# pedropro/UrsoNet

Hardware: AMD Instinct MI355X
Metric: images/sec fwd+bwd ResNet50 640x512 bs32/GPU (higher is better)
Workload: dtype bf16; 1 GPU; resnet50 bottleneck=32 ori_resolution=16 soft-class head + loc regression, batch 32/GPU x 512x640x3, full training step (prep+fwd+loss+bwd+clip+SGD); global_batch=32, parallelism=dp1, comm_cus=0, hipgraph=True, runner=Engine, input=uint8 frames in HBM, mean subtraction + cast in the step (molding kernel), gradient_norm_from_finalisation_blocks=True, weight_gradients_on_forked_stream=True

## Files before the change

### include/ursonet_hip.h

```cpp
#ifndef URSONET_HIP_H
#define URSONET_HIP_H

#include <stddef.h>
#include <stdint.h>

#ifdef __cplusplus
extern "C" {
#endif

#define URSO_OK            0
#define URSO_EINVAL       -1
#define URSO_ELAUNCH      -2
#define URSO_EWORKSPACE   -3

enum { URSO_F32 = 0, URSO_BF16 = 1, URSO_F16 = 2 };

#define URSO_EPI_RELU      1
#define URSO_EPI_OUT_F32   2
#define URSO_EPI_MASK_BITS 4
#define URSO_EPI_EMIT_BITS 8
#define URSO_EPI_ADD_SRCGRID 16

const char* urso_last_error(void);
int         urso_abi_version(void);

int urso_set_option(const char* name, int value);
int urso_get_option(const char* name, int* value);

typedef struct urso_conv_geom {
    int32_t B, H, W, C;
    int32_t OH, OW, N;
    int32_t KH, KW;
    int32_t SH, SW;
    int32_t PH, PW;
    int32_t DH, DW;
    int32_t FH, FW, OSH, OSW;
} urso_conv_geom;

int urso_conv_igemm(const urso_conv_geom* g, int dt, int flags,
                    const void* src_d, const void* wgt_d, const float* bias_d,
                    const void* add_d, const void* mask_d, void* dst_d, void* stream);
size_t urso_conv_igemm_ws_bytes(const urso_conv_geom* g, int dt);
int urso_conv_igemm_ws(const urso_conv_geom* g, int dt, int flags,
                       const void* src_d, const void* wgt_d, const float* bias_d,
                       const void* add_d, const void* mask_d, void* dst_d, void* ws_d, size_t ws_bytes, void* stream);
int urso_conv_igemm_bits_ok(const urso_conv_geom* g, int dt, int flags, size_t ws_bytes);
int urso_conv_igemm_ex(const urso_conv_geom* g, int dt, int flags,
                       const void* src_d, const void* wgt_d, const float* bias_d,
                       const void* add_d, const void* mask_d, void* dst_d, void* bits_out_d,
                       void* ws_d, size_t ws_bytes, void* stream);

int urso_conv_pair_ok(long long M, int dt, int c_narrow, int c_wide);
int urso_conv_pair(long long M, int c_narrow, int dt, int mode, const void* src_d, const void* w1_d, const float* bias1_d,
                   const void* add_d, void* bits_d, void* mid_d, const void* w2_d, const float* bias2_d, const void* mask2_d,
                   void* dst_d, int add_h, int add_w, void* stream);
int urso_rows_subsample2(int B, int H, int W, int row_bytes, const void* in_d, void* out_d, void* stream);
int urso_conv_pair_wgrad_splits(long long M, int dt);
int urso_conv_dgrad_wgrad_pw(long long M, int dt, const void* dz_d, const void* wd_d, const void* x_d, int mask_by_x, void* dx_d,
                             float* part_d, float* colpart_d, size_t part_stride, void* stream);
int urso_conv_pair_wgrad_entry(long long M, int dt, const void* src_d, const void* w1_d, const void* add_d, const void* bits_d,
                               const void* w2_d, const void* u_d, void* dst_d, const void* ws_d, const void* xin_d, int mask_by_xin, void* dxin_d,
                               float* part_d, float* colpart_d, float* part_s_d, float* colpart_s_d, size_t part_stride, void* stream);
int urso_conv_pair_shortcut(long long M, int dt, const void* src_d, const void* w1_d, const float* bias1_d,
                            const void* xin_d, const void* ws_d, const float* bias_s_d, void* bits_d, void* mid_d,
                            const void* w2_d, const float* bias2_d, void* dst_d, void* stream);
int urso_conv_pair_wgrad(long long M, int dt, const void* src_d, const void* w1_d, const void* add_d, const void* bits_d, void* mid_d,
                         const void* w2_d, const void* u_d, void* dst_d, int add_h, int add_w,
                         float* part_d, float* colpart_d, size_t part_stride, void* stream);
int urso_rows_expand2(int B, int H, int W, int row_bytes, const void* in_d, void* out_d, void* stream);
int urso_rows_scatter2(int B, int H, int W, int row_bytes, const void* in_d, void* out_d, void* stream);
int urso_zero_fill(void* dst_d, size_t bytes, void* stream);

int urso_conv_pointwise_sampled_ok(const urso_conv_geom* g, int dt, int flags, int has_add);
int urso_conv_pointwise_sampled(const urso_conv_geom* g, int dt, int flags, const void* src_d, const void* wgt_d, const float* bias_d,
                                const void* add_d, void* dst_d, void* bits_out_d, void* dst_sampled_d, void* stream);

int urso_conv_pointwise2_ok(int B, int OH, int OW, int C0, int C1, int N, int dt, int flags);
int urso_conv_pointwise2(int B, int OH, int OW, int C0, int C1, int N, int dt, int flags,
                         const void* src0_d, const void* wgt0_d, const void* src1_d, const void* wgt1_d,
                         const float* bias_d, const void* mask_d, void* dst_d, void* bits_out_d, void* stream);

#define URSO_DENSE_MULTI_MAX 4
typedef struct urso_dense_layer {
    const void* src0; const void* wgt0; const void* src1; const void* wgt1;
    const float* bias;
    const void* add; const void* mask;
    void* dst;
    int32_t M, N, K0, K1, flags;
} urso_dense_layer;
int urso_dense_multi(int nlayers, const urso_dense_layer* layers, int dt, void* stream);
typedef struct urso_dense_wgrad_layer {
    const void* x; const void* dz;
    float* part; float* colpart;
    int32_t M, K, N;
} urso_dense_wgrad_layer;
int urso_dense_wgrad_multi(int nlayers, const urso_dense_wgrad_layer* layers, int dt, void* stream);

int urso_conv_igemm_algorithmic(const urso_conv_geom* g, int dt, int flags, int has_add, int has_mask, double* flops_out, double* bytes_out);
int urso_conv_igemm_halo_ok(const urso_conv_geom* g, int dt, int flags, int has_add);
size_t urso_conv_igemm_halo_ws_bytes(void);
int urso_conv_igemm_halo2_shape(const urso_conv_geom* g, int dt, int flags, int has_add, int has_ws);

size_t urso_conv_winograd_ws_bytes(const urso_conv_geom* g, int dt);
int urso_conv_winograd_fwd(const urso_conv_geom* g, int dt, int flags, const void* src_d, const void* wgt_d, const float* bias_d,
                           void* dst_d, void* ws_d, size_t ws_bytes, void* stream);

#define URSO_WGRAD_PART_PAD 64
size_t urso_conv_wgrad_ws_bytes(const urso_conv_geom* g, int dt);
int urso_conv_wgrad(const urso_conv_geom* g, int dt, const void* x_d, const void* dz_d,
                    void* ws_d, size_t ws_bytes, float* dw_raw_d, float* colsum_d, void* stream);

int urso_conv_weight_prep(int KH, int KW, int C, int N, int npad, int dt,
                          const float* w_d, const float* b_d,
                          const float* gamma_d, const float* beta_d,
                          const float* mean_d, const float* var_d, float eps,
                          void* wf_d, void* wd_d, float* biasf_d, float* scale_d, void* stream);

int urso_stem_weight_pack(int N, int dt, const float* w_d, const float* b_d,
                          const float* gamma_d, const float* beta_d, const float* mean_d,
                          const float* var_d, float eps, void* wf_d, float* biasf_d,
                          float* scale_d, void* stream);
int urso_stem_wgrad_unpack(int N, const float* dw_packed_d, float* dw_raw_d, void* stream);

int urso_param_grad_finalize(int K, int N, int ldn ,
                             const float* dw_raw_d, const float* colsum_d,
                             const float* w_d, const float* b_d,
                             const float* gamma_d, const float* mean_d, const float* var_d,
                             float eps, float weight_decay, int trainable, int bn_trainable,
                             float* gw_d, float* gb_d, float* ggamma_d, float* gbeta_d,
                             float* ws_d, size_t ws_bytes, void* stream);
size_t urso_param_grad_finalize_ws_bytes(int K, int N);

typedef struct urso_param_desc {
    int32_t KH, KW, C, N, npad, K;
    int32_t splits, ks, kb;
    int32_t trainable, bn_trainable;
    int32_t bias_from;
    float eps, regc, regb;
    const float *w, *b, *gamma, *beta, *mean, *var;
    void *wf, *wd;
    float *biasf, *scale;
    const float *part, *colpart;
    float *dw_raw, *colsum, *dotpart;
    float *gw, *gb, *ggamma, *gbeta;
} urso_param_desc;
enum { URSO_PB_PREP = 0, URSO_PB_REDUCE = 1, URSO_PB_FINALIZE_MAT = 2, URSO_PB_FINALIZE_VEC = 3 };
int urso_conv_wgrad_splits(const urso_conv_geom* g, int dt);
int urso_conv_wgrad_partial(const urso_conv_geom* g, int dt, const void* x_d, const void* dz_d,
                            void* ws_d, size_t ws_bytes, void* stream);
int urso_param_desc_init(urso_param_desc* d, int KH, int KW, int C, int N, int npad, int splits, float eps, float weight_decay);
int urso_param_batch_plan(int phase, const urso_param_desc* descs_h, const int32_t* layer_ids, int n_ids,
                          int32_t* blockmap_h, int cap_blocks);
int urso_param_batch_run(int phase, int dt, const urso_param_desc* descs_d, const int32_t* blockmap_d, int nblocks, void* stream);
int urso_param_batch_run_sq(int phase, int dt, const urso_param_desc* descs_d, const int32_t* blockmap_d, int nblocks, float* sqpart_d, void* stream);
int urso_param_grad_finalize_sq_slots(int K, int N);
int urso_param_grad_finalize_sq(int K, int N, int ldn, const float* dw_raw_d, const float* colsum_d,
                                const float* w_d, const float* b_d, const float* gamma_d, const float* mean_d,
                                const float* var_d, float eps, float weight_decay, int trainable, int bn_trainable,
                                float* gw_d, float* gb_d, float* ggamma_d, float* gbeta_d,
                                float* ws_d, size_t ws_bytes, float* sqpart_d, void* stream);
int urso_sqnorm_final(int nparts, const float* parts_d, float* out_d, void* stream);

typedef struct urso_wgrad_item {
    const void* x;
    const void* dz;
    float* part;
    float* colpart;
    urso_conv_geom g;
    int32_t M, ktiles, ntiles, splits, m_per_split, mode, fill;
} urso_wgrad_item;
int urso_wgrad_group_fits(const urso_conv_geom* g, int dt);
int urso_wgrad_group_plan(int n, urso_wgrad_item* items_h, int dt, int32_t* blockmap_h, int cap_blocks);
int urso_wgrad_group_run(int dt, const urso_wgrad_item* items_d, const urso_wgrad_item* items_h, int n,
                         const int32_t* blockmap_d, int nblocks, void* stream);

int urso_conv_wgrad_pair_splits(const urso_conv_geom* g0, const urso_conv_geom* g1, int dt, int* splits0, int* splits1);
int urso_conv_wgrad_partial2(const urso_conv_geom* g0, const urso_conv_geom* g1, int dt,
                             const void* x0_d, const void* dz0_d, void* ws0_d, size_t ws0_bytes,
                             const void* x1_d, const void* dz1_d, void* ws1_d, size_t ws1_bytes, void* stream);

size_t urso_bn_ws_bytes(int M, int N);
int urso_bn_batch_stats(int M, int N, int dt, const void* z_d, void* ws_d, size_t ws_bytes, float* mean_d, float* var_d,
                        float* moving_mean_d, float* moving_var_d, float momentum, float eps, void* stream);
int urso_bn_apply(int M, int N, int dt, const void* z_d, const float* mean_d, const float* var_d, const float* gamma_d,
                  const float* beta_d, float eps, const void* res_d, int relu, void* y_d, void* stream);
int urso_bn_backward(int M, int N, int dt, const void* g_d, const void* z_d, const float* mean_d, const float* var_d,
                     const float* gamma_d, float eps, void* ws_d, size_t ws_bytes, float* dbeta_d, float* dgamma_d,
                     int bn_trainable, float* gbeta_d, float* ggamma_d, void* dz_d, void* stream);

int urso_mold_images(int B, int H, int W, int src_is_u8, const void* src_d, const float* mean3_d,
                     int dt, void* dst_d, void* stream);

int urso_stem_wgrad_pooled(const urso_conv_geom* g, int dt, const void* x_d, const void* dpool_d, const uint8_t* argmax_d,
                           void* ws_d, size_t ws_bytes, float* dw_raw_d, float* colsum_d, void* stream);
int urso_stem_conv_pool_ok(const urso_conv_geom* g, int dt);
int urso_stem_conv_pool(const urso_conv_geom* g, int dt, const void* x_d, const void* wgt_d, const float* bias_d, void* y_d,
                        uint8_t* argmax_d, void* stream);
int urso_maxpool3x3s2_fwd(int B, int H, int W, int C, int dt, const void* x_d, void* y_d,
                          uint8_t* argmax_d, void* stream);
int urso_maxpool3x3s2_bwd(int B, int H, int W, int C, int dt, const void* y_d, const void* dy_d,
                          const uint8_t* argmax_d, int relu_mask, void* dx_d, void* stream);

int urso_softmax_xent_fwd_bwd(int B, int K, const float* logits_d , const float* labels_d,
                              float weight, int relu_mask, int dt, float* loss_d, void* dz_d,
                              float* row_ws_d, void* stream);
int urso_rel_l2_fwd_bwd(int B, int D, int ld ,
                        const float* gt_d , const float* pred_d, float weight,
                        int dt, float* loss_d, void* dpred_d, float* norms_d, void* stream);
int urso_rel_l2_norms(int B, int D, int ld, const float* gt_d, const float* pred_d, float* norms_d, void* stream);
int urso_rel_l2_from_norms(int B, int D, int ld, const float* gt_d, const float* pred_d, float weight, const float* gscale_d,
                           int dt, const float* norms_d, float* loss_d, void* dpred_d, void* stream);
int urso_absdot_fwd_bwd(int B, int D, int ld , int normalize,
                        const float* gt_d , const float* x_d,
                        float weight, int dt, float* q_d , float* loss_d, void* dx_d, void* stream);
int urso_mse_fwd_bwd(int B, int D, int ld, const float* gt_d, const float* pred_d, float weight,
                     int dt, float* loss_d, void* dpred_d, void* stream);

size_t urso_sqnorm_ws_bytes(size_t n);
int urso_sqnorm(size_t n, const float* g_d, void* ws_d, size_t ws_bytes, float* out_d, void* stream);
int urso_sgd_momentum_clip(size_t n, float* w_d, const float* g_d, float* v_d,
                           const float* hyper_d, const float* normsq_d, void* stream);
int urso_adam_amsgrad_clip(size_t n, float* w_d, const float* g_d, float* m_d, float* v_d, float* vhat_d,
                           float* hyper_d, const float* normsq_d, void* stream);
int urso_scale_f32(size_t n, float* x_d, float s, void* stream);

int urso_quat_wavg_decode(int B, int K, const float* logits_d, const float* hquat_d,
                          float* q_d, float* a_d, void* stream);

int urso_quat_gmm_fit(int B, int K, const float* in_d, int in_is_pmf, const float* hquat_d, float var,
                      int nr_iterations, int nr_max_modes, float* mean_d, float* var_d, float* prior_d,
                      float* score_d, int* nmodes_d, void* stream);

enum { URSO_EVAL_LOC_REGRESS = 0, URSO_EVAL_LOC_CLASS = 1 };
enum { URSO_EVAL_ORI_QUAT = 0, URSO_EVAL_ORI_EULER = 1, URSO_EVAL_ORI_ANGLE_AXIS = 2, URSO_EVAL_ORI_SOFT = 3, URSO_EVAL_ORI_KEYPOINTS = 4 };
enum { URSO_EVAL_LOC_EST = 0, URSO_EVAL_Q_EST = 3, URSO_EVAL_LOC_ERR = 7, URSO_EVAL_ORI_ERR = 8, URSO_EVAL_ESA = 9, URSO_EVAL_DIST = 10,
       URSO_EVAL_LOC_ENC_ERR = 11, URSO_EVAL_ORI_ENC_ERR = 12, URSO_EVAL_ORI_ERR_SOFT = 13, URSO_EVAL_MODE = 14, URSO_EVAL_COLS = 16 };
typedef struct urso_pose_eval_args {
    int32_t B, n;
    int64_t row0;
    int32_t loc_mode, ori_mode;
    int32_t loc_ld, ori_ld;
    int32_t loc_bins, loc_map_rows, ori_bins, ori_map_rows, gmm_modes, pad0;
    const float* loc;
    const float* ori;
    const float* ori2;
    const double* loc_map;
    const float* ori_map;
    const float* enc_loc;
    const float* enc_ori;
    const double* loc_gt;
    const double* q_gt;
    const float* gmm_mean;
    const int32_t* gmm_nmodes;
    double* table;
} urso_pose_eval_args;
int urso_pose_eval(const urso_pose_eval_args* args, void* stream);

enum { URSO_DEC_LOC_EST = 0, URSO_DEC_Q_EST = 3, URSO_DEC_LOC_PEAK = 7, URSO_DEC_ORI_PEAK = 8, URSO_DEC_ORI_LAMBDA = 9, URSO_DEC_COLS = 12 };
typedef struct urso_pose_decode_args {
    int32_t B, n;
    int64_t row0;
    int32_t loc_mode, ori_mode;
    int32_t loc_ld, ori_ld;
    int32_t loc_bins, loc_map_rows, ori_bins, ori_map_rows;
    int32_t ori_logits_ld, pad0;
    const float* loc;
    const float* ori;
    const float* ori2;
    const double* loc_map;
    const float* ori_logits;
    const float* ori_scatter;
    double* table;
} urso_pose_decode_args;
int urso_pose_decode(const urso_pose_decode_args* args, void* stream);

int urso_warp_perspective(int B, int H, int W, int C, int interp, const uint8_t* src_d, const double* m_d, uint8_t* dst_d, void* stream);
int urso_encode_ori(int B, int K, const double* q_d, const float* hquat_d, const uint8_t* redundant_d, double var,
                    float* out_d, void* stream);

int urso_encode_loc(int B, int K, const double* loc_d, const double* hmap_d, double sig2, float* out_d, void* stream);

int urso_rgb_to_grey3(int B, int H, int W, const uint8_t* src_d, uint8_t* dst_d, void* stream);
int urso_sim2real_op(int B, int H, int W, const uint8_t* src_d, uint8_t* dst_d, const int32_t* op_d, const float* par_d,
                     const uint32_t* seed_d, const uint8_t* drop_d, int drop_stride, void* stream);
int urso_pad_images_u8(int B, int H, int W, int C, int OH, int OW, int top, int left, const uint8_t* src_d, uint8_t* dst_d, void* stream);

int urso_resize_images_u8(int B, int H, int W, int C, int NH, int NW, int OH, int OW, int top, int left,
                          const double* ky_d, int ry, const double* kx_d, int rx, const int32_t* y0_d, const double* fy_d,
                          const int32_t* x0_d, const double* fx_d, int trunc_passes, const uint8_t* src_d, uint8_t* dst_d, void* stream);

int urso_frames_grey_flags_u8(int B, int HW, const uint8_t* src_d, uint8_t* flags_d, void* stream);
int urso_frames_put_u8(int B, int HW, const uint8_t* src_d, const uint64_t* dst_addr_d, const uint8_t* kind_d, void* stream);
int urso_frames_gather_u8(int B, int HW, const uint64_t* src_addr_d, const uint8_t* kind_d, uint8_t* dst_d, void* stream);

int urso_video_prep_u8(int B, int H, int W, int top, int bottom, int left, int right, int pad, double w0, double w1, double w2,
                       const uint8_t* src_d, uint8_t* dst_d, void* stream);

// ... 48 lines not shown
```

### ursonet_amd/csrc/common.h

```cpp
#pragma once
#include <hip/hip_runtime.h>
#include <stdint.h>
#include <stdio.h>
#include "../../include/ursonet_hip.h"

typedef __attribute__((ext_vector_type(8))) __bf16 bf16x8_t;
typedef __attribute__((ext_vector_type(8))) _Float16 f16x8_t;
typedef __attribute__((ext_vector_type(4))) float f32x4_t;
typedef __attribute__((ext_vector_type(4))) int i32x4_t;
typedef __attribute__((ext_vector_type(2))) int i32x2_t;

void urso_set_error(const char* fmt, ...);
int  urso_check_launch(const char* what);

#define URSO_OPTION_TABLE(X) \
    X(pw_kernel, 3)         \
    X(pw_small, 5)          \
    X(wgrad_narrow, 1)      \
    X(wgrad_blocks, 512)    \
    X(wgrad_pipe, 1)        \
    X(wgrad_big, 1)         \
    X(wgrad_ring, 0)        \
    X(grid_cap, 0)          \
    X(hconv, 1)             \
    X(pair, 1)              \
    X(pair_single, 3)       \
    X(c3, 1)                \
    X(c3v, 1)               \
    X(stem, 1)              \
    X(stem_pool, 1)         \
    X(cus, 0)               \
    X(hconv2, 1)            \
    X(hconv2_shape, 0)      \
    X(hconv_streamk, 1)     \
    X(hconv_dbg, 0)         \
    X(hwgrad, 1)            \
    X(dense, 1)             \
    X(pwx, 1)               \
    X(pwx_dbg, 0)           \
    X(pwx_bn, 0)            \
    X(mold_scalar, 0)       \
    X(bneck, 3)
struct UrsoOptions {
#define URSO_OPT_FIELD(name, dflt) int name = dflt;
    URSO_OPTION_TABLE(URSO_OPT_FIELD)
#undef URSO_OPT_FIELD
};
extern UrsoOptions g_urso_opt;
int urso_device_cus();
int urso_usable_cus();

#define URSO_FUSE_REDUCE_MAX 16
static __host__ __device__ inline bool urso_fuse_reduce(int splits) { return splits > 1 && splits <= URSO_FUSE_REDUCE_MAX; }

#define URSO_REDUCE_COLS 256
static __host__ __device__ inline int urso_reduce_lanes(int splits) { return splits > 384 ? 16 : (splits > 192 ? 8 : (splits > 96 ? 4 : (splits > 48 ? 2 : 1))); }

void urso_prof_before(hipStream_t s, int kernel_id, double flops, double bytes);
void urso_prof_after(hipStream_t s);

void urso_prof_l2(double l2_bytes);
void urso_prof_symbol(const void* host_fn);
#define URSO_KLAUNCH(kern, grid, blk, shm, st, ...) do { urso_prof_symbol((const void*)(kern)); hipLaunchKernelGGL(kern, grid, blk, shm, st, ##__VA_ARGS__); } while (0)

struct ProfScope {
    hipStream_t s;
    ProfScope(hipStream_t st, int id, double flops, double bytes) : s(st) { urso_prof_before(s, id, flops, bytes); }
    ~ProfScope() { urso_prof_after(s); }
};

static inline size_t dt_size(int dt) { return dt == URSO_F32 ? 4 : 2; }
static __host__ __device__ inline int ceil_div(int a, int b) { return (a + b - 1) / b; }

template <typename T> struct Elem;
template <> struct Elem<float> {
    static constexpr int VE = 4;
    static __device__ __forceinline__ float to_f(float v) { return v; }
    static __device__ __forceinline__ float from_f(float v) { return v; }
};
template <> struct Elem<__bf16> {
    static constexpr int VE = 8;
    static constexpr int ONES = 0x3F803F80;
    static __device__ __forceinline__ float to_f(__bf16 v) { return (float)v; }
    static __device__ __forceinline__ __bf16 from_f(float v) { return (__bf16)v; }
};
template <> struct Elem<_Float16> {
    static constexpr int VE = 8;
    static constexpr int ONES = 0x3C003C00;
    static __device__ __forceinline__ float to_f(_Float16 v) { return (float)v; }
    static __device__ __forceinline__ _Float16 from_f(float v) { return (_Float16)v; }
};

template <typename T> struct Mma;
template <> struct Mma<__bf16> {
    static __device__ __forceinline__ void run(const i32x4_t& a, const i32x4_t& b, f32x4_t& c) {
        c = __builtin_amdgcn_mfma_f32_16x16x32_bf16(__builtin_bit_cast(bf16x8_t, a), __builtin_bit_cast(bf16x8_t, b), c, 0, 0, 0);
    }
};
template <> struct Mma<_Float16> {
    static __device__ __forceinline__ void run(const i32x4_t& a, const i32x4_t& b, f32x4_t& c) {
        c = __builtin_amdgcn_mfma_f32_16x16x32_f16(__builtin_bit_cast(f16x8_t, a), __builtin_bit_cast(f16x8_t, b), c, 0, 0, 0);
    }
};
template <> struct Mma<float> {
    static __device__ __forceinline__ void run(const i32x4_t& a, const i32x4_t& b, f32x4_t& c) {
        f32x4_t fa = __builtin_bit_cast(f32x4_t, a), fb = __builtin_bit_cast(f32x4_t, b);
        c = __builtin_amdgcn_mfma_f32_16x16x4f32(fa.x, fb.x, c, 0, 0, 0);
        c = __builtin_amdgcn_mfma_f32_16x16x4f32(fa.y, fb.y, c, 0, 0, 0);
        c = __builtin_amdgcn_mfma_f32_16x16x4f32(fa.z, fb.z, c, 0, 0, 0);
        c = __builtin_amdgcn_mfma_f32_16x16x4f32(fa.w, fb.w, c, 0, 0, 0);
    }
};

__device__ __forceinline__ int lds_swz(int row) {
    int c = (row >> 3) & 7;
    int s = (c & 4) | ((c & 1) << 1) | ((c >> 1) & 1);
    return (row & 7) ^ s;
}
__device__ __forceinline__ int lds_off(int row, int chunk) {
    return row * 128 + ((chunk ^ lds_swz(row)) << 4);
}

#define URSO_OOB_SHIFT 0x80000000u
__device__ __forceinline__ __amdgpu_buffer_rsrc_t make_rsrc(const void* p, uint32_t bytes) {
    return __builtin_amdgcn_make_buffer_rsrc(const_cast<void*>(p), 0, bytes, 0x00020000);
}
__device__ __forceinline__ i32x4_t buf_load16(__amdgpu_buffer_rsrc_t r, uint32_t byte_off) {
    return __builtin_amdgcn_raw_buffer_load_b128(r, byte_off, 0, 0);
}
__device__ __forceinline__ void buf_store16(__amdgpu_buffer_rsrc_t r, uint32_t byte_off, i32x4_t v) {
    __builtin_amdgcn_raw_buffer_store_b128(v, r, byte_off, 0, 0);
}

__device__ __forceinline__ void lds_barrier() {
    asm volatile("s_waitcnt lgkmcnt(0)" ::: "memory");
    __builtin_amdgcn_s_barrier();
    asm volatile("" ::: "memory");
}

__device__ __forceinline__ float wave_sum(float v) {
#pragma unroll
    for (int o = 32; o > 0; o >>= 1) v += __shfl_xor(v, o, 64);
    return v;
}
__device__ __forceinline__ float wave_max(float v) {
#pragma unroll
    for (int o = 32; o > 0; o >>= 1) v = fmaxf(v, __shfl_xor(v, o, 64));
    return v;
}

__device__ __forceinline__ int xcd_remap(int bid, int nblk) {
    const int NX = 8;
    if (nblk < NX) return bid;
    int xcd = bid % NX, idx = bid / NX;
    int q = nblk / NX, r = nblk % NX;
    int base = (xcd < r) ? xcd * (q + 1) : r * (q + 1) + (xcd - r) * q;
    return base + idx;
}

static inline int urso_persistent_grid(int ntiles, int blocks_per_cu, int groups = 1) {
    int bpx = ceil_div(ntiles, 8), cap = blocks_per_cu * urso_usable_cus() / (8 * groups);
    if (cap < 1) cap = 1;
    if (bpx > cap) bpx = cap;
    if (g_urso_opt.grid_cap > 0 && bpx > ceil_div(g_urso_opt.grid_cap, 8)) bpx = ceil_div(g_urso_opt.grid_cap, 8);
    return 8 * bpx;
}
struct UrsoTileStream { int tile, t_end, bpx; };
__device__ __forceinline__ UrsoTileStream urso_tile_stream(int ntiles) {
    const int xcd = blockIdx.x & 7, lb = blockIdx.x >> 3, bpx = gridDim.x >> 3;
    const int cpx = ceil_div(ntiles, 8);
    const int t_end = min((xcd + 1) * cpx, ntiles);
    return { xcd * cpx + lb, t_end, bpx };
}
```

### ursonet_amd/csrc/conv_wgrad.hip

```cpp
#include "lds_mfma.h"
#include "internal.h"
#include <stdlib.h>

struct WgradArgs {
    const void* x; const void* dz; float* part; float* colpart;
    uint32_t x_bytes, dz_bytes;
    int B, H, W, C, OH, OW, N, KH, KW, SH, SW, PH, PW;
    int M, Cc, Kc, K;
    int ktiles, ntiles, splits, m_per_split;
    int dbg;
    int pointwise;
    float rcp_ohw, rcp_ow;
    int zs, ZH, ZW, zsh, zsw;
};

template <typename T, int MODE>
__global__ __launch_bounds__(256, 2) void wgrad_kernel(const WgradArgs a) {
    constexpr int VE = Elem<T>::VE;
    constexpr int RM = 128 / (int)sizeof(T);
    constexpr int NCH = 128 / VE;
    constexpr int PIX = (sizeof(T) == 2) ? 2 : 1;
    constexpr int ITEMS = (RM / PIX) * NCH / 256;
    constexpr int PSTEP = 256 / NCH;
    __shared__ __attribute__((aligned(16))) char smem[2 * 2 * 128 * 128];
// ... 744 lines not shown
    const int dq = RM / a.OW, dr = RM - dq * a.OW;
    const uint32_t xc_off = (uint32_t)(cc * VE) * 2u, z_off0 = (uint32_t)ncol * 2u;

    auto dma = [&](int buf) {
        const uint32_t dx = lds0 + buf * BUFB + wave * 1024, dz = lds0 + buf * BUFB + RM * 256 + wave * 1024;
#pragma unroll
        for (int e = 0; e < ITEMS; ++e) {
            const int m = mcur + prow + 16 * e;
            const bool mvalid = m < m_end;
            uint32_t off; bool ok;
            if constexpr (MODE == 0) { off = (uint32_t)(m * a.C) * 2u + xc_off; ok = mvalid && kvalid; }
            else {
                int b, oy, ox;
                if constexpr (MODE == 1) {
                    b = pb[e]; oy = poy[e]; ox = pox[e];
                    int nx = ox + dr; const bool w1 = nx >= a.OW; nx -= w1 ? a.OW : 0;
                    int ny = oy + dq + (w1 ? 1 : 0); const bool w2 = ny >= a.OH; ny -= w2 ? a.OH : 0;
                    pox[e] = nx; poy[e] = ny; pb[e] = b + (w2 ? 1 : 0);
                } else { int rem; divmod(m, ohw, a.rcp_ohw, b, rem); divmod(rem, a.OW, a.rcp_ow, oy, ox); }
                const int iy = oy * a.SH - a.PH + ky, ix = ox * a.SW - a.PW + kx;
                ok = mvalid && kvalid && iy >= 0 && ix >= 0 && iy < a.H && ix < a.W;
                off = (uint32_t)(((b * a.H + iy) * a.W + ix) * a.C) * 2u + xc_off;
            }
            lds_dma16(rx, dx + e * 16 * 256, ok ? off : URSO_OOB_SHIFT);
        }
#pragma unroll
        for (int e = 0; e < 2; ++e) {
            const int mz = mcur + zrow + 32 * e;
            uint32_t zp = (uint32_t)mz;
            if (a.zs) { int b, rem, oy, ox; divmod(mz, ohw, a.rcp_ohw, b, rem); divmod(rem, a.OW, a.rcp_ow, oy, ox); zp = (uint32_t)((b * a.ZH + oy * a.zsh) * a.ZW + ox * a.zsw); }
            const uint32_t zoff = zp * (uint32_t)a.N * 2u + z_off0;
            lds_dma16(rz, dz + e * 32 * 128, (mz < m_end && nvalid) ? zoff : URSO_OOB_SHIFT);
        }
        mcur += RM;
    };

    const int fr = lane & 15, fg = lane >> 4;
    const int frow = fg * 4 + (fr >> 2), fsw = frow & 7;
    const int fbase = frow * 256 + (fr & 3) * 8;
    int offx[4], offz[2];
#pragma unroll
    for (int i = 0; i < 4; ++i) offx[i] = fbase + (((wk * 4 + i) ^ fsw) << 5);
    const int zbase = frow * 128 + (fr & 3) * 8, zsw = (frow >> 1) & 3;
#pragma unroll
    for (int j = 0; j < 2; ++j) offz[j] = zbase + (((wn * 2 + j) ^ zsw) << 5);

    f32x4_t acc[4][2], accc[2];
#pragma unroll
    for (int i = 0; i < 4; ++i)
#pragma unroll
        for (int j = 0; j < 2; ++j) acc[i][j] = f32x4_t{0.f, 0.f, 0.f, 0.f};
    accc[0] = accc[1] = f32x4_t{0.f, 0.f, 0.f, 0.f};
    const bool do_col = (kt == 0) && (wk == 0) && a.colpart;
    const i32x4_t ones = {Elem<T>::ONES, Elem<T>::ONES, Elem<T>::ONES, Elem<T>::ONES};

    const int nsteps = (m_end > m_begin) ? ceil_div(m_end - m_begin, RM) : 0;
    if (nsteps > 0) dma(0);
    asm volatile("s_waitcnt vmcnt(0)" ::: "memory");
    __syncthreads();
    for (int s = 0; s < nsteps; ++s) {
        const int cur = s & 1;
        if (s + 1 < nsteps) dma(cur ^ 1);
        const char* bx = sX(cur); const char* bz = sZ(cur);
#pragma unroll
        for (int ks = 0; ks < 2; ++ks) {
            i32x4_t fz[2], fx[4];
#pragma unroll
            for (int j = 0; j < 2; ++j) {
                const i32x2_t lo = lds_read_tr16(bz + offz[j] + ks * 32 * 128), hi = lds_read_tr16(bz + offz[j] + ks * 32 * 128 + 16 * 128);
                fz[j] = i32x4_t{lo.x, lo.y, hi.x, hi.y};
            }
#pragma unroll
            for (int i = 0; i < 4; ++i) {
                const i32x2_t lo = lds_read_tr16(bx + offx[i] + ks * 32 * 256), hi = lds_read_tr16(bx + offx[i] + ks * 32 * 256 + 16 * 256);
                fx[i] = i32x4_t{lo.x, lo.y, hi.x, hi.y};
            }
#pragma unroll
            for (int i = 0; i < 4; ++i)
#pragma unroll
                for (int j = 0; j < 2; ++j) Mma<T>::run(fz[j], fx[i], acc[i][j]);
            if (do_col) {
#pragma unroll
                for (int j = 0; j < 2; ++j) Mma<T>::run(fz[j], ones, accc[j]);
            }
        }
        asm volatile("s_waitcnt vmcnt(0)" ::: "memory");
        __syncthreads();
    }

    float* out = a.part + (size_t)sp * ((size_t)a.K * a.N + URSO_WGRAD_PART_PAD);
#pragma unroll
    for (int i = 0; i < 4; ++i) {
        const int k = kt * 128 + wk * 64 + i * 16 + fr;
        if (k >= a.K) continue;
#pragma unroll
        for (int j = 0; j < 2; ++j) {
            const int nb = n0 + wn * 32 + j * 16 + fg * 4;
            if (nb >= a.N) continue;
            *(f32x4_t*)(out + (size_t)k * a.N + nb) = acc[i][j];
        }
    }
    if (do_col && fr == 0) {
#pragma unroll
        for (int j = 0; j < 2; ++j) {
            const int nb = n0 + wn * 32 + j * 16 + fg * 4;
            if (nb < a.N) *(f32x4_t*)(a.colpart + (size_t)sp * a.N + nb) = accc[j];
        }
    }
}

__device__ __forceinline__ void reduce_partials_body(int bid, const float* __restrict__ part, float* __restrict__ out, size_t count, int splits,
                                                     size_t pstride ) {
    __shared__ f32x4_t red[256];
    const size_t nq = (count + 3) / 4;
    const bool vec = (count & 3) == 0;
    const int SL = urso_reduce_lanes(splits), cols = URSO_REDUCE_COLS / SL;
    const int col = threadIdx.x % cols, sl = threadIdx.x / cols;
    const size_t q = (size_t)bid * cols + col;
    f32x4_t t = f32x4_t{0.f, 0.f, 0.f, 0.f};
    if (vec && q < nq) {
        const size_t stride = pstride / 4;
        const f32x4_t* p = (const f32x4_t*)part + q;
        const int per = (splits + SL - 1) / SL, k1 = min(splits, (sl + 1) * per);
        int k = sl * per;
        for (; k + 16 <= k1; k += 16) {
            f32x4_t v[16];
#pragma unroll
            for (int i = 0; i < 16; ++i) v[i] = p[(size_t)(k + i) * stride];
#pragma unroll
            for (int i = 0; i < 16; ++i) t += v[i];
        }
        for (; k < k1; ++k) t += p[(size_t)k * stride];
    }
    if (SL > 1) {
        red[threadIdx.x] = t;
        __syncthreads();
        if (sl == 0) {
            t = red[col];
            for (int i = 1; i < SL; ++i) t += red[i * cols + col];
        }
    }
    if (vec && q < nq && sl == 0) *((f32x4_t*)out + q) = t;
    if (!vec && threadIdx.x == 0 && bid == 0)
        for (size_t e = 0; e < count; ++e) { float tt = 0.f; for (int i = 0; i < splits; ++i) tt += part[(size_t)i * pstride + e]; out[e] = tt; }
}

__global__ __launch_bounds__(256) void reduce_partials_kernel(const float* __restrict__ part, float* __restrict__ out, size_t count, int splits, size_t pstride) {
    reduce_partials_body(blockIdx.x, part, out, count, splits, pstride);
}

__global__ __launch_bounds__(256) void reduce_partials_batch_kernel(const urso_param_desc* __restrict__ descs, const int32_t* __restrict__ blockmap) {
    const urso_param_desc& d = descs[blockmap[2 * blockIdx.x]];
    const int local = blockmap[2 * blockIdx.x + 1];
    const size_t cnt = (size_t)d.K * d.npad;
    const int rcols = URSO_REDUCE_COLS / urso_reduce_lanes(d.splits);
    const int nb_dw = (int)(((cnt + 3) / 4 + rcols - 1) / rcols);
    if (local < nb_dw) reduce_partials_body(local, d.part, d.dw_raw, cnt, d.splits, cnt + URSO_WGRAD_PART_PAD);
    else reduce_partials_body(local - nb_dw, d.colpart, d.colsum, (size_t)d.npad, d.splits, (size_t)d.npad);
}

void urso_reduce_partials_batch_launch(const urso_param_desc* descs_d, const int32_t* blockmap_d, int nblocks, hipStream_t st) {
    URSO_KLAUNCH(reduce_partials_batch_kernel, dim3(nblocks), dim3(256), 0, st, descs_d, blockmap_d);
}

struct WgradPlan { int VE, RM, Cc, Kc, K, M, ktiles, ntiles, splits, m_per_split, narrow; size_t part_elems, col_elems; };

static int plan_wgrad(const urso_conv_geom* g, int dt, WgradPlan& p) {
    const int es = (int)dt_size(dt);
    p.VE = 16 / es; p.RM = 128 / es;
    if (g->C % p.VE || g->N % p.VE) return URSO_EINVAL;
    p.Cc = g->C / p.VE; p.Kc = g->KH * g->KW * p.Cc; p.K = p.Kc * p.VE;
    p.M = g->B * g->OH * g->OW;
    const int narrow_ok = g_urso_opt.wgrad_narrow;
#ifndef URSO_WGRAD_NARROW_MULTITAP
#define URSO_WGRAD_NARROW_MULTITAP 0
#endif
    p.narrow = (es == 2 && narrow_ok && (g->N <= 64 || (URSO_WGRAD_NARROW_MULTITAP && g->KH * g->KW > 1))) ? 1 : 0;
    p.ktiles = ceil_div(p.K, 128); p.ntiles = ceil_div(g->N, p.narrow ? 64 : 128);
    const int tiles = p.ktiles * p.ntiles;
    const int steps = ceil_div(p.M, p.RM);
    const int target = (int)((long long)g_urso_opt.wgrad_blocks * urso_usable_cus() / urso_device_cus());
#ifndef URSO_WGRAD_NARROW_PCT
#define URSO_WGRAD_NARROW_PCT 150
#endif
    int splits = (p.narrow ? target * URSO_WGRAD_NARROW_PCT / 100 : target) / tiles;
    splits = splits < 1 ? 1 : splits;
    int max_splits = steps / 8; if (max_splits < 1) max_splits = 1;
    if (splits > max_splits) splits = max_splits;
    int steps_per = ceil_div(steps, splits);
    splits = ceil_div(steps, steps_per);
    if (urso_c3g_fits(g, dt)) splits = urso_c3g_splits(g);
    else if (urso_hwg_fits(g, dt)) splits = urso_hwg_splits(g);
    p.splits = splits; p.m_per_split = steps_per * p.RM;
    p.part_elems = (size_t)splits * ((size_t)p.K * g->N + URSO_WGRAD_PART_PAD);
    p.col_elems = (size_t)splits * g->N;
    return URSO_OK;
}

extern "C" size_t urso_conv_wgrad_ws_bytes(const urso_conv_geom* g, int dt) {
    WgradPlan p;
    if (g && urso_stemw_fits(g, dt)) {
        const size_t stem = (size_t)urso_stemw_splits(g, false) * ((size_t)224 * 64 + URSO_WGRAD_PART_PAD + 64) * sizeof(float) + 256;
        const size_t gen = plan_wgrad(g, dt, p) == URSO_OK ? (p.part_elems + p.col_elems) * sizeof(float) + 256 : 0;
        return stem > gen ? stem : gen;
    }
    if (!g || plan_wgrad(g, dt, p) != URSO_OK) return 0;
    return (p.part_elems + p.col_elems) * sizeof(float) + 256;
}

extern "C" int urso_conv_wgrad_splits(const urso_conv_geom* g, int dt) {
    WgradPlan p;
    if (!g || plan_wgrad(g, dt, p) != URSO_OK) return 0;
    return p.splits;
}

static int wgrad_impl(const urso_conv_geom* g, int dt, const void* x_d, const void* dz_d,
                      void* ws_d, size_t ws_bytes, float* dw_raw_d, float* colsum_d, bool keep_partials, void* stream) {
    if (!g || !x_d || !dz_d || !ws_d || (!dw_raw_d && !keep_partials)) { urso_set_error("urso_conv_wgrad: null argument"); return URSO_EINVAL; }
    if (dt != URSO_F32 && dt != URSO_BF16 && dt != URSO_F16) { urso_set_error("urso_conv_wgrad: bad dtype"); return URSO_EINVAL; }
    if (g->DH != 1 || g->DW != 1) { urso_set_error("urso_conv_wgrad: expects the forward geometry (D=1)"); return URSO_EINVAL; }
    WgradPlan p;
    if (plan_wgrad(g, dt, p) != URSO_OK) { urso_set_error("urso_conv_wgrad: C=%d and N=%d must be multiples of %d", g->C, g->N, 16 / (int)dt_size(dt)); return URSO_EINVAL; }
    const size_t need = urso_conv_wgrad_ws_bytes(g, dt);
    if (ws_bytes < need) { urso_set_error("urso_conv_wgrad: workspace %zu < %zu", ws_bytes, need); return URSO_EWORKSPACE; }
    const size_t es = dt_size(dt);
    const bool zscat = g->FH > 0;
    if (zscat && (dt == URSO_F32 || g->FW <= 0 || g->OSH <= 0 || g->OSW <= 0 || (g->OH - 1) * g->OSH >= g->FH || (g->OW - 1) * g->OSW >= g->FW ||
                  (g->KH == 1 && g->KW == 1 && g->SH == 1 && g->SW == 1 && g->PH == 0 && g->PW == 0 && g->H == g->OH && g->W == g->OW))) {
        urso_set_error("urso_conv_wgrad: scattered dz needs a 16-bit dtype, a non-pointwise geometry and a grid that fits [FH][FW]"); return URSO_EINVAL;
    }
    const size_t x_bytes = (size_t)g->B * g->H * g->W * g->C * es,
                 dz_bytes = zscat ? (size_t)g->B * g->FH * g->FW * g->N * es : (size_t)p.M * g->N * es;
    if (x_bytes >= 0x7FFFFF00ull || dz_bytes >= 0x7FFFFF00ull) { urso_set_error("urso_conv_wgrad: tensor exceeds 2 GiB"); return URSO_EINVAL; }
    if (urso_stemw_fits(g, dt) && !keep_partials && !zscat) {
        hipStream_t st = (hipStream_t)stream;
        const int splits = urso_stemw_splits(g, false);
        const size_t cnt = (size_t)224 * 64, pstride = cnt + URSO_WGRAD_PART_PAD;
        float* part = (float*)ws_d; float* colpart = part + (size_t)splits * pstride;
        ProfScope ps(st, URSO_K_WGRAD, 2.0 * p.M * 64.0 * 147.0, (double)x_bytes + (double)p.M * 128 + (double)cnt * 4);
        int rc = urso_stemw_launch(g, dt, x_d, dz_d, nullptr, nullptr, part, colsum_d ? colpart : nullptr, pstride, st);
        if (rc != URSO_OK) return rc;
        const int rcols = URSO_REDUCE_COLS / urso_reduce_lanes(splits);
        URSO_KLAUNCH(reduce_partials_kernel, dim3((int)((cnt / 4 + rcols - 1) / rcols)), dim3(256), 0, st, part, dw_raw_d, cnt, splits, pstride);
        if (colsum_d) URSO_KLAUNCH(reduce_partials_kernel, dim3((int)((64 / 4 + rcols - 1) / rcols)), dim3(256), 0, st, colpart, colsum_d, (size_t)64, splits, (size_t)64);
        return urso_check_launch("urso_conv_wgrad(stem reduce)");
    }
    WgradArgs a;
    a.x = x_d; a.dz = dz_d; a.x_bytes = (uint32_t)x_bytes; a.dz_bytes = (uint32_t)dz_bytes;
    float* part = (float*)ws_d; float* colpart = part + p.part_elems;
    const bool direct = (p.splits == 1) && !keep_partials;
    a.part = direct ? dw_raw_d : part;
    a.colpart = keep_partials ? colpart : (colsum_d ? (direct ? colsum_d : colpart) : nullptr);
    a.B = g->B; a.H = g->H; a.W = g->W; a.C = g->C; a.OH = g->OH; a.OW = g->OW; a.N = g->N;
    a.KH = g->KH; a.KW = g->KW; a.SH = g->SH; a.SW = g->SW; a.PH = g->PH; a.PW = g->PW;
    a.dbg = 0;
    a.pointwise = (g->KH == 1 && g->KW == 1 && g->SH == 1 && g->SW == 1 && g->PH == 0 && g->PW == 0 && g->H == g->OH && g->W == g->OW) ? 1 : 0;
    a.rcp_ohw = 1.0f / (float)(g->OH * g->OW); a.rcp_ow = 1.0f / (float)g->OW;
    a.zs = zscat ? 1 : 0; a.ZH = g->FH; a.ZW = g->FW; a.zsh = g->OSH; a.zsw = g->OSW;
    if ((size_t)g->B * g->OH * g->OW >= (1u << 24)) { urso_set_error("urso_conv_wgrad: more than 2^24 output pixels"); return URSO_EINVAL; }
    a.M = p.M; a.Cc = p.Cc; a.Kc = p.Kc; a.K = p.K; a.ktiles = p.ktiles; a.ntiles = p.ntiles; a.splits = p.splits; a.m_per_split = p.m_per_split;
    hipStream_t st = (hipStream_t)stream;
    double flops = 2.0 * p.M * (double)g->N * g->KH * g->KW * g->C;
    if (g->C == 8 && g->KH == 7 && g->KW == 4 && g->SH == 2) flops *= 147.0 / 224.0;
    const double x_alg = (g->KH == 1 && g->KW == 1 && (g->SH > 1 || g->SW > 1)) ? (double)p.M * g->C * es : (double)x_bytes;
    double bytes = x_alg + (double)p.M * g->N * es + (double)p.K * g->N * 4;
    ProfScope ps(st, URSO_K_WGRAD, flops, bytes);
    dim3 grid(p.ktiles * p.ntiles, p.splits);
    const int rm = 128 / (int)dt_size(dt);
    const int mode = a.pointwise ? 0 : (g->OW >= rm ? 1 : 2);
    const int tmode = a.pointwise ? 0 : ((64 / g->OW + 1 <= g->OH) ? 1 : 2);
#define URSO_WG(KERN, TT, MD) do { if (MD == 0) URSO_KLAUNCH((KERN<TT, 0>), grid, dim3(256), 0, st, a); \
                         else if (MD == 1) URSO_KLAUNCH((KERN<TT, 1>), grid, dim3(256), 0, st, a); \
                         else URSO_KLAUNCH((KERN<TT, 2>), grid, dim3(256), 0, st, a); } while (0)
    const int pipe = g_urso_opt.wgrad_pipe;
#define URSO_WGP(TT, MD) do { if (MD == 0) URSO_KLAUNCH((wgrad_tr_kernel<TT, 0, true>), grid, dim3(256), 0, st, a); \
                         else if (MD == 1) URSO_KLAUNCH((wgrad_tr_kernel<TT, 1, true>), grid, dim3(256), 0, st, a); \
                         else URSO_KLAUNCH((wgrad_tr_kernel<TT, 2, true>), grid, dim3(256), 0, st, a); } while (0)
    if (!zscat && urso_c3g_fits(g, dt)) {
        int rc3 = urso_c3g_launch(g, dt, x_d, dz_d, a.part, a.colpart, (size_t)p.K * g->N + URSO_WGRAD_PART_PAD, st);
        if (rc3 != URSO_OK) return rc3;
    }
    else if (!zscat && urso_hwg_fits(g, dt)) {
        int rc3 = urso_hwg_launch(g, dt, x_d, dz_d, a.part, a.colpart, (size_t)p.K * g->N + URSO_WGRAD_PART_PAD, st);
        if (rc3 != URSO_OK) return rc3;
    }
    else if (dt == URSO_F32) URSO_WG(wgrad_kernel, float, mode);
    else if (p.narrow) { if (dt == URSO_BF16) URSO_WG(wgrad_tr64_kernel, __bf16, tmode); else URSO_WG(wgrad_tr64_kernel, _Float16, tmode); }
    else if (dt == URSO_BF16) { if (pipe) URSO_WGP(__bf16, tmode); else URSO_WG(wgrad_tr_kernel, __bf16, tmode); }
    else { if (pipe) URSO_WGP(_Float16, tmode); else URSO_WG(wgrad_tr_kernel, _Float16, tmode); }
#undef URSO_WGP
#undef URSO_WG
    int rc = urso_check_launch("urso_conv_wgrad");
    if (rc != URSO_OK) return rc;
    if (!direct && !keep_partials) {
        size_t cnt = (size_t)p.K * g->N;
        const int rcols = URSO_REDUCE_COLS / urso_reduce_lanes(p.splits);
        int blocks = (int)(((cnt + 3) / 4 + rcols - 1) / rcols);
        URSO_KLAUNCH(reduce_partials_kernel, dim3(blocks), dim3(256), 0, st, part, dw_raw_d, cnt, p.splits, cnt + URSO_WGRAD_PART_PAD);
        if (colsum_d) URSO_KLAUNCH(reduce_partials_kernel, dim3((int)(((size_t)g->N / 4 + rcols - 1) / rcols)), dim3(256), 0, st, colpart, colsum_d, (size_t)g->N, p.splits, (size_t)g->N);
        rc = urso_check_launch("urso_conv_wgrad(reduce)");
    }
    return rc;
}

extern "C" int urso_conv_wgrad(const urso_conv_geom* g, int dt, const void* x_d, const void* dz_d,
                               void* ws_d, size_t ws_bytes, float* dw_raw_d, float* colsum_d, void* stream) {
    return wgrad_impl(g, dt, x_d, dz_d, ws_d, ws_bytes, dw_raw_d, colsum_d, false, stream);
// ... 183 lines not shown
```

### ursonet_amd/csrc/prep.hip

```cpp
#include "common.h"
#include "internal.h"

template <typename T> __device__ __forceinline__ void store_elem(void* p, size_t i, float v) { ((T*)p)[i] = Elem<T>::from_f(v); }

__device__ __forceinline__ float bn_scale(const float* gamma, const float* var, float eps, int n) {
    return gamma ? gamma[n] * rsqrtf(var[n] + eps) : 1.0f;
}

__device__ __forceinline__ float folded_bias(const urso_param_desc& o, int n) {
    if (n >= o.N) return 0.f;
    const float s = bn_scale(o.gamma, o.var, o.eps, n);
    float bf = o.b ? o.b[n] * s : 0.f;
    if (o.gamma) bf += o.beta[n] - o.mean[n] * s;
    return bf;
}

template <typename T>
__device__ __forceinline__ void weight_prep_body(int bx, int by, int tap, int KH, int KW, int C, int N, int npad,
                                   const float* __restrict__ w, const float* __restrict__ b,
                                   const float* __restrict__ gamma, const float* __restrict__ beta,
                                   const float* __restrict__ mean, const float* __restrict__ var, float eps,
                                   void* wf, void* wd, float* biasf, float* scale, const urso_param_desc* extra = nullptr) {
    __shared__ float tile[32][33];
    const int c0 = bx * 32, n0 = by * 32;
    const int tx = threadIdx.x & 31, ty = threadIdx.x >> 5;
    const int taps = KH * KW;
    const int ftap = taps - 1 - tap;
    const int n = n0 + tx;
    const float s = (n < N) ? bn_scale(gamma, var, eps, n) : 1.0f;
    for (int cy = ty; cy < 32; cy += 8) {
        const int c = c0 + cy;
        float v = 0.f;
        if (c < C && n < N) v = w[((size_t)tap * C + c) * N + n] * s;
        tile[cy][tx] = v;
        if (wd && c < C && n < npad) store_elem<T>(wd, ((size_t)c * taps + ftap) * npad + n, v);
    }
    __syncthreads();
    for (int ny = ty; ny < 32; ny += 8) {
        const int nn = n0 + ny, c = c0 + tx;
        if (nn < npad && c < C) store_elem<T>(wf, ((size_t)nn * taps + tap) * C + c, tile[tx][ny]);
    }
    if (tap == 0 && bx == 0 && ty == 0 && n < npad) {
        float bf = 0.f, sc = 1.f;
        if (n < N) {
            sc = s;
            bf = (b ? b[n] * s : 0.f);
            if (gamma) bf += beta[n] - mean[n] * s;
            if (extra) bf += folded_bias(*extra, n);
        }
        biasf[n] = bf; scale[n] = sc;
    }
}

template <typename T>
__device__ __forceinline__ void weight_prep_body64(int bx, int by, int tap, int KH, int KW, int C, int N, int npad,
                                   const float* __restrict__ w, const float* __restrict__ b,
                                   const float* __restrict__ gamma, const float* __restrict__ beta,
                                   const float* __restrict__ mean, const float* __restrict__ var, float eps,
                                   void* wf, void* wd, float* biasf, float* scale, const urso_param_desc* extra = nullptr) {
    __shared__ float tile[64][65];
    const int c0 = bx * 64, n0 = by * 64;
    const int tq = threadIdx.x & 15, tr = threadIdx.x >> 4;
    const int taps = KH * KW, ftap = taps - 1 - tap;
    const int n = n0 + tq * 4;
    float s[4];
#pragma unroll
    for (int q = 0; q < 4; ++q) s[q] = (n + q < N) ? bn_scale(gamma, var, eps, n + q) : 1.0f;
    for (int cy = tr; cy < 64; cy += 16) {
        const int c = c0 + cy;
        f32x4_t v = {0.f, 0.f, 0.f, 0.f};
        if (c < C && n < N) { v = *(const f32x4_t*)(w + ((size_t)tap * C + c) * N + n); v.x *= s[0]; v.y *= s[1]; v.z *= s[2]; v.w *= s[3]; }
        tile[cy][tq * 4] = v.x; tile[cy][tq * 4 + 1] = v.y; tile[cy][tq * 4 + 2] = v.z; tile[cy][tq * 4 + 3] = v.w;
        if (wd && c < C && n < npad) {
            T o[4] = {Elem<T>::from_f(v.x), Elem<T>::from_f(v.y), Elem<T>::from_f(v.z), Elem<T>::from_f(v.w)};
            __builtin_memcpy((T*)wd + ((size_t)c * taps + ftap) * npad + n, o, sizeof(o));
        }
    }
    __syncthreads();
    for (int ny = tr; ny < 64; ny += 16) {
        const int nn = n0 + ny, c = c0 + tq * 4;
        if (nn < npad && c < C) {
            T o[4] = {Elem<T>::from_f(tile[tq * 4][ny]), Elem<T>::from_f(tile[tq * 4 + 1][ny]), Elem<T>::from_f(tile[tq * 4 + 2][ny]),
                      Elem<T>::from_f(tile[tq * 4 + 3][ny])};
            __builtin_memcpy((T*)wf + ((size_t)nn * taps + tap) * C + c, o, sizeof(o));
        }
    }
    if (tap == 0 && bx == 0 && tr == 0) {
#pragma unroll
        for (int q = 0; q < 4; ++q) {
            const int nq = n + q;
            if (nq < npad) {
                float bf = 0.f, sc = 1.f;
                if (nq < N) { sc = s[q]; bf = (b ? b[nq] * s[q] : 0.f); if (gamma) bf += beta[nq] - mean[nq] * s[q]; if (extra) bf += folded_bias(*extra, nq); }
                biasf[nq] = bf; scale[nq] = sc;
            }
        }
    }
}

template <typename T>
__global__ void weight_prep_kernel(int KH, int KW, int C, int N, int npad,
                                   const float* __restrict__ w, const float* __restrict__ b,
                                   const float* __restrict__ gamma, const float* __restrict__ beta,
                                   const float* __restrict__ mean, const float* __restrict__ var, float eps,
                                   void* wf, void* wd, float* biasf, float* scale) {
    weight_prep_body<T>(blockIdx.x, blockIdx.y, blockIdx.z, KH, KW, C, N, npad, w, b, gamma, beta, mean, var, eps, wf, wd, biasf, scale);
}

template <typename T>
__global__ void weight_prep_batch_kernel(const urso_param_desc* __restrict__ descs, const int32_t* __restrict__ blockmap) {
    const urso_param_desc& d = descs[blockmap[2 * blockIdx.x]];
    const int local = blockmap[2 * blockIdx.x + 1];
    const urso_param_desc* extra = d.bias_from > 0 ? &descs[d.bias_from - 1] : nullptr;
    if (((d.C | d.N | d.npad) & 3) == 0) {
        const int gx = ceil_div(d.C, 64), gy = ceil_div(d.npad, 64);
        const int bx = local % gx, by = (local / gx) % gy, tap = local / (gx * gy);
        weight_prep_body64<T>(bx, by, tap, d.KH, d.KW, d.C, d.N, d.npad, d.w, d.b, d.gamma, d.beta, d.mean, d.var, d.eps,
                              d.wf, d.wd, d.biasf, d.scale, extra);
        return;
    }
    const int gx = ceil_div(d.C, 32), gy = ceil_div(d.npad, 32);
    const int bx = local % gx, by = (local / gx) % gy, tap = local / (gx * gy);
    weight_prep_body<T>(bx, by, tap, d.KH, d.KW, d.C, d.N, d.npad, d.w, d.b, d.gamma, d.beta, d.mean, d.var, d.eps,
                        d.wf, d.wd, d.biasf, d.scale, extra);
}

extern "C" int urso_conv_weight_prep(int KH, int KW, int C, int N, int npad, int dt,
                                     const float* w_d, const float* b_d, const float* gamma_d, const float* beta_d,
                                     const float* mean_d, const float* var_d, float eps,
                                     void* wf_d, void* wd_d, float* biasf_d, float* scale_d, void* stream) {
    if (!w_d || !wf_d || !biasf_d || !scale_d || KH <= 0 || KW <= 0 || C <= 0 || N <= 0 || npad < N) {
        urso_set_error("urso_conv_weight_prep: bad argument"); return URSO_EINVAL; }
    if (gamma_d && (!beta_d || !mean_d || !var_d)) { urso_set_error("urso_conv_weight_prep: incomplete BN tensors"); return URSO_EINVAL; }
    hipStream_t st = (hipStream_t)stream;
    dim3 grid(ceil_div(C, 32), ceil_div(npad, 32), KH * KW);
    ProfScope ps(st, URSO_K_PREP, 0, (double)KH * KW * C * N * (4 + 2 * dt_size(dt)));
    if (dt == URSO_F32) URSO_KLAUNCH((weight_prep_kernel<float>), grid, dim3(256), 0, st, KH, KW, C, N, npad, w_d, b_d, gamma_d, beta_d, mean_d, var_d, eps, wf_d, wd_d, biasf_d, scale_d);
    else if (dt == URSO_BF16) URSO_KLAUNCH((weight_prep_kernel<__bf16>), grid, dim3(256), 0, st, KH, KW, C, N, npad, w_d, b_d, gamma_d, beta_d, mean_d, var_d, eps, wf_d, wd_d, biasf_d, scale_d);
    else if (dt == URSO_F16) URSO_KLAUNCH((weight_prep_kernel<_Float16>), grid, dim3(256), 0, st, KH, KW, C, N, npad, w_d, b_d, gamma_d, beta_d, mean_d, var_d, eps, wf_d, wd_d, biasf_d, scale_d);
    else { urso_set_error("urso_conv_weight_prep: bad dtype"); return URSO_EINVAL; }
    return urso_check_launch("urso_conv_weight_prep");
}

template <typename T>
__global__ void stem_pack_kernel(int N, const float* __restrict__ w, const float* __restrict__ b,
                                 const float* __restrict__ gamma, const float* __restrict__ beta,
                                 const float* __restrict__ mean, const float* __restrict__ var, float eps,
                                 void* wf, float* biasf, float* scale) {
    const int i = blockIdx.x * blockDim.x + threadIdx.x;
    const int total = N * 7 * 4 * 8;
    if (i < total) {
        const int cp = i & 7, kp = (i >> 3) & 3, ky = (i >> 5) % 7, n = i / 224;
        const int q = 2 * kp + (cp >> 2), kx = q - 1, c = cp & 3;
        float v = 0.f;
        if (kx >= 0 && c < 3) v = w[(((size_t)ky * 7 + kx) * 3 + c) * N + n] * bn_scale(gamma, var, eps, n);
        store_elem<T>(wf, i, v);
    }
    if (i < N) {
        const float s = bn_scale(gamma, var, eps, i);
        float bf = b ? b[i] * s : 0.f;
        if (gamma) bf += beta[i] - mean[i] * s;
        biasf[i] = bf; scale[i] = s;
    }
}

extern "C" int urso_stem_weight_pack(int N, int dt, const float* w_d, const float* b_d, const float* gamma_d,
                                     const float* beta_d, const float* mean_d, const float* var_d, float eps,
                                     void* wf_d, float* biasf_d, float* scale_d, void* stream) {
    if (!w_d || !wf_d || !biasf_d || !scale_d || N <= 0) { urso_set_error("urso_stem_weight_pack: bad argument"); return URSO_EINVAL; }
    hipStream_t st = (hipStream_t)stream;
    const int total = N * 224, blocks = ceil_div(total, 256);
    ProfScope ps(st, URSO_K_PREP, 0, 0);
    if (dt == URSO_F32) URSO_KLAUNCH((stem_pack_kernel<float>), dim3(blocks), dim3(256), 0, st, N, w_d, b_d, gamma_d, beta_d, mean_d, var_d, eps, wf_d, biasf_d, scale_d);
    else if (dt == URSO_BF16) URSO_KLAUNCH((stem_pack_kernel<__bf16>), dim3(blocks), dim3(256), 0, st, N, w_d, b_d, gamma_d, beta_d, mean_d, var_d, eps, wf_d, biasf_d, scale_d);
    else if (dt == URSO_F16) URSO_KLAUNCH((stem_pack_kernel<_Float16>), dim3(blocks), dim3(256), 0, st, N, w_d, b_d, gamma_d, beta_d, mean_d, var_d, eps, wf_d, biasf_d, scale_d);
    else { urso_set_error("urso_stem_weight_pack: bad dtype"); return URSO_EINVAL; }
    return urso_check_launch("urso_stem_weight_pack");
}

__global__ void stem_unpack_kernel(int N, const float* __restrict__ dwp, float* __restrict__ dw) {
    const int i = blockIdx.x * blockDim.x + threadIdx.x;
    if (i >= 7 * 7 * 3 * N) return;
    const int n = i % N, c = (i / N) % 3, kx = (i / (3 * N)) % 7, ky = i / (21 * N);
    const int q = kx + 1, kp = q >> 1, cp = (q & 1) * 4 + c;
    dw[i] = dwp[(((size_t)ky * 4 + kp) * 8 + cp) * N + n];
}

extern "C" int urso_stem_wgrad_unpack(int N, const float* dw_packed_d, float* dw_raw_d, void* stream) {
    if (!dw_packed_d || !dw_raw_d || N <= 0) { urso_set_error("urso_stem_wgrad_unpack: bad argument"); return URSO_EINVAL; }
    hipStream_t st = (hipStream_t)stream;
    ProfScope ps(st, URSO_K_FINALIZE, 0, 0);
    URSO_KLAUNCH(stem_unpack_kernel, dim3(ceil_div(147 * N, 256)), dim3(256), 0, st, N, dw_packed_d, dw_raw_d);
    return urso_check_launch("urso_stem_wgrad_unpack");
}

__device__ __forceinline__ float block_sum_f(float v, float* sh) {
    v = wave_sum(v);
    const int w = threadIdx.x >> 6, nw = (blockDim.x + 63) >> 6;
    __syncthreads();
    if ((threadIdx.x & 63) == 0) sh[w] = v;
    __syncthreads();
    float t = 0.f;
    for (int i = 0; i < nw; ++i) t += sh[i];
    return t;
}

__device__ __forceinline__ void finalize_mat_body(int bx, int by, int K, int N, int ldn, int kb, const float* __restrict__ dwr, const float* __restrict__ w,
                                    const float* __restrict__ gamma, const float* __restrict__ var, float eps,
                                    float regc, int trainable, float* __restrict__ gw, float* __restrict__ dotpart, int nsum = 1, size_t pstride = 0,
                                    float* __restrict__ sqslot = nullptr) {
    const int kbeg = by * kb, kend = min(K, kbeg + kb);
    float sq = 0.f;
    auto sq4 = [&](const f32x4_t& g) { sq += g.x * g.x + g.y * g.y + g.z * g.z + g.w * g.w; };
    auto sq_out = [&]() {
        if (!sqslot) return;
        __shared__ float shq[8];
        const float t = block_sum_f(sq, shq);
        if (threadIdx.x == 0) *sqslot = t;
    };
    if (((N | ldn) & 3) == 0) {
        __shared__ f32x4_t red4[16][17];
        const int tq = threadIdx.x & 15, tk = threadIdx.x >> 4;
        const int n = bx * 64 + tq * 4;
        f32x4_t dot = {0.f, 0.f, 0.f, 0.f};
        if (n < N) {
            f32x4_t s;
            s.x = bn_scale(gamma, var, eps, n); s.y = bn_scale(gamma, var, eps, n + 1);
            s.z = bn_scale(gamma, var, eps, n + 2); s.w = bn_scale(gamma, var, eps, n + 3);
            auto row_sum = [&](int k) -> f32x4_t {
                const float* p = dwr + (size_t)k * ldn + n;
                f32x4_t d = *(const f32x4_t*)p;
                if (nsum > 1) {
                    f32x4_t t = f32x4_t{0.f, 0.f, 0.f, 0.f};
                    t += d;
                    int q = 1;
                    for (; q + 4 <= nsum; q += 4) {
                        const f32x4_t v0 = *(const f32x4_t*)(p + (size_t)q * pstride), v1 = *(const f32x4_t*)(p + (size_t)(q + 1) * pstride);
                        const f32x4_t v2 = *(const f32x4_t*)(p + (size_t)(q + 2) * pstride), v3 = *(const f32x4_t*)(p + (size_t)(q + 3) * pstride);
                        t += v0; t += v1; t += v2; t += v3;
                    }
                    for (; q < nsum; ++q) t += *(const f32x4_t*)(p + (size_t)q * pstride);
                    d = t;
                }
                return d;
            };
            int k = kbeg + tk;
            for (; k + 16 < kend; k += 32) {
                const f32x4_t w0 = *(const f32x4_t*)(w + (size_t)k * N + n), w1 = *(const f32x4_t*)(w + (size_t)(k + 16) * N + n);
                const f32x4_t d0 = row_sum(k), d1 = row_sum(k + 16);
                dot += w0 * d0;
                dot += w1 * d1;
                f32x4_t g0 = s * d0 + w0 * regc, g1 = s * d1 + w1 * regc;
                if (!trainable) g0 = g1 = f32x4_t{0.f, 0.f, 0.f, 0.f};
                *(f32x4_t*)(gw + (size_t)k * N + n) = g0;
                *(f32x4_t*)(gw + (size_t)(k + 16) * N + n) = g1;
                sq4(g0); sq4(g1);
            }
            if (k < kend) {
                const f32x4_t ww = *(const f32x4_t*)(w + (size_t)k * N + n);
                const f32x4_t d = row_sum(k);
                dot += ww * d;
                f32x4_t g = s * d + ww * regc;
                if (!trainable) g = f32x4_t{0.f, 0.f, 0.f, 0.f};
                *(f32x4_t*)(gw + (size_t)k * N + n) = g;
                sq4(g);
            }
        }
        red4[tk][tq] = dot;
        __syncthreads();
        if (tk == 0 && n < N) {
            f32x4_t t = red4[0][tq];
#pragma unroll
            for (int i = 1; i < 16; ++i) t += red4[i][tq];
            *(f32x4_t*)(dotpart + (size_t)by * N + n) = t;
        }
        sq_out();
        return;
    }
    __shared__ float red[4][64];
    const int tn = threadIdx.x & 63, tk = threadIdx.x >> 6;
    const int n = bx * 64 + tn;
    float dot = 0.f;
    if (n < N) {
        const float s = bn_scale(gamma, var, eps, n);
        for (int k = kbeg + tk; k < kend; k += 4) {
            float d = 0.f;
            for (int q = 0; q < nsum; ++q) d += dwr[(size_t)q * pstride + (size_t)k * ldn + n];
            const float ww = w[(size_t)k * N + n];
            dot += ww * d;
            const float gv = trainable ? (s * d + regc * ww) : 0.f;
            gw[(size_t)k * N + n] = gv;
            sq += gv * gv;
        }
    }
    red[tk][tn] = dot;
    __syncthreads();
    if (tk == 0 && n < N) dotpart[(size_t)by * N + n] = red[0][tn] + red[1][tn] + red[2][tn] + red[3][tn];
    sq_out();
}

__global__ void finalize_mat_kernel(int K, int N, int ldn, int kb, const float* __restrict__ dwr, const float* __restrict__ w,
                                    const float* __restrict__ gamma, const float* __restrict__ var, float eps,
                                    float regc, int trainable, float* __restrict__ gw, float* __restrict__ dotpart, float* __restrict__ sqpart) {
    finalize_mat_body(blockIdx.x, blockIdx.y, K, N, ldn, kb, dwr, w, gamma, var, eps, regc, trainable, gw, dotpart, 1, 0,
                      sqpart ? sqpart + blockIdx.y * gridDim.x + blockIdx.x : nullptr);
}

__global__ void finalize_mat_batch_kernel(const urso_param_desc* __restrict__ descs, const int32_t* __restrict__ blockmap, float* __restrict__ sqpart) {
    const urso_param_desc& d = descs[blockmap[2 * blockIdx.x]];
    const int local = blockmap[2 * blockIdx.x + 1];
    const int gx = ceil_div(d.N, 64);
    const bool fused = urso_fuse_reduce(d.splits);
    finalize_mat_body(local % gx, local / gx, d.K, d.N, d.npad, d.kb, (d.splits == 1 || fused) ? d.part : d.dw_raw, d.w, d.gamma, d.var, d.eps,
                      d.regc, d.trainable, d.gw, d.dotpart, fused ? d.splits : 1, (size_t)d.K * d.npad + URSO_WGRAD_PART_PAD,
                      sqpart ? sqpart + blockIdx.x : nullptr);
}

__device__ __forceinline__ void finalize_vec_body(int n, int N, int ks, const float* __restrict__ dotpart, const float* __restrict__ colsum,
                                    const float* __restrict__ b, const float* __restrict__ gamma,
                                    const float* __restrict__ mean, const float* __restrict__ var, float eps,
                                    float regb, int trainable, int bn_trainable,
                                    float* __restrict__ gb, float* __restrict__ ggamma, float* __restrict__ gbeta, int nsum = 1, int cstride = 0,
                                    float* __restrict__ sqslot = nullptr) {
    float sq = 0.f;
    if (n < N) {
    float cs = 0.f;
    if (colsum) for (int q = 0; q < nsum; ++q) cs += colsum[(size_t)q * cstride + n];
    const float s = bn_scale(gamma, var, eps, n);
    if (gb) { const float v = trainable ? (s * cs + regb * (b ? b[n] : 0.f)) : 0.f; gb[n] = v; sq += v * v; }
    if (ggamma) {
        float d0 = 0.f, d1 = 0.f, d2 = 0.f, d3 = 0.f;
        int i = 0;
        for (; i + 3 < ks; i += 4) { d0 += dotpart[(size_t)i * N + n]; d1 += dotpart[(size_t)(i + 1) * N + n];
                                     d2 += dotpart[(size_t)(i + 2) * N + n]; d3 += dotpart[(size_t)(i + 3) * N + n]; }
        for (; i < ks; ++i) d0 += dotpart[(size_t)i * N + n];
        const float dot = (d0 + d1) + (d2 + d3);
        const float rstd = rsqrtf(var[n] + eps);
        const float vg = bn_trainable ? rstd * (dot + ((b ? b[n] : 0.f) - mean[n]) * cs) : 0.f, vb = bn_trainable ? cs : 0.f;
        ggamma[n] = vg;
        gbeta[n] = vb;
        sq += vg * vg + vb * vb;
    }
    }
    if (sqslot) {
        __shared__ float shq[8];
        const float t = block_sum_f(sq, shq);
        if (threadIdx.x == 0) *sqslot = t;
    }
}

__global__ void finalize_vec_kernel(int N, int ks, const float* __restrict__ dotpart, const float* __restrict__ colsum,
                                    const float* __restrict__ b, const float* __restrict__ gamma,
                                    const float* __restrict__ mean, const float* __restrict__ var, float eps,
                                    float regb, int trainable, int bn_trainable,
                                    float* __restrict__ gb, float* __restrict__ ggamma, float* __restrict__ gbeta, float* __restrict__ sqpart) {
    finalize_vec_body(blockIdx.x * blockDim.x + threadIdx.x, N, ks, dotpart, colsum, b, gamma, mean, var, eps, regb, trainable, bn_trainable, gb, ggamma, gbeta,
                      1, 0, sqpart ? sqpart + blockIdx.x : nullptr);
}

__global__ void finalize_vec_batch_kernel(const urso_param_desc* __restrict__ descs, const int32_t* __restrict__ blockmap, float* __restrict__ sqpart) {
    const urso_param_desc& d = descs[blockmap[2 * blockIdx.x]];
    const int local = blockmap[2 * blockIdx.x + 1];
    if (!d.gb && !d.ggamma) { if (sqpart && threadIdx.x == 0) sqpart[blockIdx.x] = 0.f; return; }
    const bool fused = urso_fuse_reduce(d.splits);
    finalize_vec_body(local * blockDim.x + threadIdx.x, d.N, d.ks, d.dotpart, (d.splits == 1 || fused) ? d.colpart : d.colsum, d.b, d.gamma, d.mean, d.var, d.eps,
                      d.regb, d.trainable, d.bn_trainable, d.gb, d.ggamma, d.gbeta, fused ? d.splits : 1, d.npad, sqpart ? sqpart + blockIdx.x : nullptr);
}

static int finalize_ks(int K, int N) {
    int ntiles = ceil_div(N, 64);
    int ks = ceil_div(512, ntiles);
    if (ks > 32) ks = 32;
    int maxks = K / 128; if (maxks < 1) maxks = 1;
    if (ks > maxks) ks = maxks;
    return ks;
}
extern "C" size_t urso_param_grad_finalize_ws_bytes(int K, int N) { return (size_t)finalize_ks(K, N) * N * sizeof(float) + 256; }

extern "C" int urso_param_grad_finalize_sq_slots(int K, int N) { return ceil_div(N, 64) * finalize_ks(K, N) + ceil_div(N, 256); }
static int param_grad_finalize_impl(int K, int N, int ldn, const float* dw_raw_d, const float* colsum_d,
                                        const float* w_d, const float* b_d, const float* gamma_d, const float* mean_d,
                                        const float* var_d, float eps, float weight_decay, int trainable, int bn_trainable,
                                        float* gw_d, float* gb_d, float* ggamma_d, float* gbeta_d,
                                        float* ws_d, size_t ws_bytes, float* sqpart_d, void* stream);
extern "C" int urso_param_grad_finalize(int K, int N, int ldn, const float* dw_raw_d, const float* colsum_d,
                                        const float* w_d, const float* b_d, const float* gamma_d, const float* mean_d,
                                        const float* var_d, float eps, float weight_decay, int trainable, int bn_trainable,
                                        float* gw_d, float* gb_d, float* ggamma_d, float* gbeta_d,
                                        float* ws_d, size_t ws_bytes, void* stream) {
    return param_grad_finalize_impl(K, N, ldn, dw_raw_d, colsum_d, w_d, b_d, gamma_d, mean_d, var_d, eps, weight_decay, trainable, bn_trainable,
                                    gw_d, gb_d, ggamma_d, gbeta_d, ws_d, ws_bytes, nullptr, stream);
}
extern "C" int urso_param_grad_finalize_sq(int K, int N, int ldn, const float* dw_raw_d, const float* colsum_d,
                                           const float* w_d, const float* b_d, const float* gamma_d, const float* mean_d,
                                           const float* var_d, float eps, float weight_decay, int trainable, int bn_trainable,
                                           float* gw_d, float* gb_d, float* ggamma_d, float* gbeta_d,
                                           float* ws_d, size_t ws_bytes, float* sqpart_d, void* stream) {
    if (!sqpart_d) { urso_set_error("urso_param_grad_finalize_sq: sqpart_d required"); return URSO_EINVAL; }
    return param_grad_finalize_impl(K, N, ldn, dw_raw_d, colsum_d, w_d, b_d, gamma_d, mean_d, var_d, eps, weight_decay, trainable, bn_trainable,
                                    gw_d, gb_d, ggamma_d, gbeta_d, ws_d, ws_bytes, sqpart_d, stream);
}
static int param_grad_finalize_impl(int K, int N, int ldn, const float* dw_raw_d, const float* colsum_d,
                                        const float* w_d, const float* b_d, const float* gamma_d, const float* mean_d,
                                        const float* var_d, float eps, float weight_decay, int trainable, int bn_trainable,
                                        float* gw_d, float* gb_d, float* ggamma_d, float* gbeta_d,
                                        float* ws_d, size_t ws_bytes, float* sqpart_d, void* stream) {
    if (!dw_raw_d || !w_d || !gw_d || !ws_d || K <= 0 || N <= 0 || ldn < N) { urso_set_error("urso_param_grad_finalize: bad argument"); return URSO_EINVAL; }
    if ((gb_d || ggamma_d) && !colsum_d) { urso_set_error("urso_param_grad_finalize: colsum required for bias/BN gradients"); return URSO_EINVAL; }
    if (ggamma_d && (!gamma_d || !mean_d || !var_d || !gbeta_d)) { urso_set_error("urso_param_grad_finalize: incomplete BN tensors"); return URSO_EINVAL; }
    if (ws_bytes < urso_param_grad_finalize_ws_bytes(K, N)) { urso_set_error("urso_param_grad_finalize: workspace too small"); return URSO_EWORKSPACE; }
    hipStream_t st = (hipStream_t)stream;
    const int ks = finalize_ks(K, N), kb = ceil_div(K, ks);
    const float regc = 2.0f * weight_decay / ((float)K * (float)N), regb = 2.0f * weight_decay / (float)N;
    ProfScope ps(st, URSO_K_FINALIZE, 0, (double)K * N * 12);
    URSO_KLAUNCH(finalize_mat_kernel, dim3(ceil_div(N, 64), ks), dim3(256), 0, st, K, N, ldn, kb, dw_raw_d, w_d, gamma_d, var_d, eps, regc, trainable, gw_d, ws_d, sqpart_d);
    float* sqv = sqpart_d ? sqpart_d + ceil_div(N, 64) * ks : nullptr;
    if (gb_d || ggamma_d)
        URSO_KLAUNCH(finalize_vec_kernel, dim3(ceil_div(N, 256)), dim3(256), 0, st, N, ks, (const float*)ws_d, colsum_d, b_d, gamma_d, mean_d, var_d, eps, regb, trainable, bn_trainable, gb_d, ggamma_d, gbeta_d, sqv);
    else if (sqv) hipMemsetAsync(sqv, 0, (size_t)ceil_div(N, 256) * sizeof(float), st);
    return urso_check_launch("urso_param_grad_finalize");
}


static int batch_layer_blocks(int phase, const urso_param_desc& d) {
    switch (phase) {
    case URSO_PB_PREP: return (((d.C | d.N | d.npad) & 3) == 0 ? ceil_div(d.C, 64) * ceil_div(d.npad, 64) : ceil_div(d.C, 32) * ceil_div(d.npad, 32)) * d.KH * d.KW;
    case URSO_PB_REDUCE: {
        if (d.splits <= 1 || urso_fuse_reduce(d.splits)) return 0;
        const size_t cnt = (size_t)d.K * d.npad;
        const int rcols = URSO_REDUCE_COLS / urso_reduce_lanes(d.splits);
        return (int)(((cnt + 3) / 4 + rcols - 1) / rcols) + (int)(((size_t)(d.npad + 3) / 4 + rcols - 1) / rcols);
    }
    case URSO_PB_FINALIZE_MAT: return ceil_div(d.N, 64) * d.ks;
    case URSO_PB_FINALIZE_VEC: return ceil_div(d.N, 256);
    }
    return -1;
}

extern "C" int urso_param_desc_init(urso_param_desc* d, int KH, int KW, int C, int N, int npad, int splits, float eps, float weight_decay) {
    if (!d || KH <= 0 || KW <= 0 || C <= 0 || N <= 0 || npad < N || splits < 1) { urso_set_error("urso_param_desc_init: bad argument"); return URSO_EINVAL; }
    d->KH = KH; d->KW = KW; d->C = C; d->N = N; d->npad = npad; d->K = KH * KW * C; d->splits = splits;
    d->ks = finalize_ks(d->K, N); d->kb = ceil_div(d->K, d->ks);
    d->eps = eps;
    d->regc = 2.0f * weight_decay / ((float)d->K * (float)N); d->regb = 2.0f * weight_decay / (float)N;
    return URSO_OK;
}

extern "C" int urso_param_batch_plan(int phase, const urso_param_desc* descs_h, const int32_t* layer_ids, int n_ids,
                                     int32_t* blockmap_h, int cap_blocks) {
    if (!descs_h || !layer_ids || n_ids < 0 || phase < URSO_PB_PREP || phase > URSO_PB_FINALIZE_VEC) { urso_set_error("urso_param_batch_plan: bad argument"); return URSO_EINVAL; }
    int total = 0;
    for (int i = 0; i < n_ids; ++i) {
        const urso_param_desc& d = descs_h[layer_ids[i]];
        const int nb = batch_layer_blocks(phase, d);
        if (nb < 0) return URSO_EINVAL;
        for (int l = 0; l < nb; ++l, ++total)
            if (blockmap_h && total < cap_blocks) { blockmap_h[2 * total] = layer_ids[i]; blockmap_h[2 * total + 1] = l; }
    }
    return total;
}

static int param_batch_run_impl(int phase, int dt, const urso_param_desc* descs_d, const int32_t* blockmap_d, int nblocks, float* sqpart_d, void* stream);
extern "C" int urso_param_batch_run(int phase, int dt, const urso_param_desc* descs_d, const int32_t* blockmap_d, int nblocks, void* stream) {
    return param_batch_run_impl(phase, dt, descs_d, blockmap_d, nblocks, nullptr, stream);
}
extern "C" int urso_param_batch_run_sq(int phase, int dt, const urso_param_desc* descs_d, const int32_t* blockmap_d, int nblocks, float* sqpart_d, void* stream) {
    if (!sqpart_d || (phase != URSO_PB_FINALIZE_MAT && phase != URSO_PB_FINALIZE_VEC)) { urso_set_error("urso_param_batch_run_sq: FINALIZE phases only, sqpart_d required"); return URSO_EINVAL; }
    return param_batch_run_impl(phase, dt, descs_d, blockmap_d, nblocks, sqpart_d, stream);
}
static int param_batch_run_impl(int phase, int dt, const urso_param_desc* descs_d, const int32_t* blockmap_d, int nblocks, float* sqpart_d, void* stream) {
    if (!descs_d || !blockmap_d || nblocks < 0) { urso_set_error("urso_param_batch_run: bad argument"); return URSO_EINVAL; }
    if (nblocks == 0) return URSO_OK;
    hipStream_t st = (hipStream_t)stream;
    switch (phase) {
    case URSO_PB_PREP: {
        ProfScope ps(st, URSO_K_PREP, 0, 0);
        if (dt == URSO_F32) URSO_KLAUNCH((weight_prep_batch_kernel<float>), dim3(nblocks), dim3(256), 0, st, descs_d, blockmap_d);
        else if (dt == URSO_BF16) URSO_KLAUNCH((weight_prep_batch_kernel<__bf16>), dim3(nblocks), dim3(256), 0, st, descs_d, blockmap_d);
        else if (dt == URSO_F16) URSO_KLAUNCH((weight_prep_batch_kernel<_Float16>), dim3(nblocks), dim3(256), 0, st, descs_d, blockmap_d);
        else { urso_set_error("urso_param_batch_run: bad dtype"); return URSO_EINVAL; }
        break; }
    case URSO_PB_REDUCE: { ProfScope ps(st, URSO_K_FINALIZE, 0, 0); urso_reduce_partials_batch_launch(descs_d, blockmap_d, nblocks, st); break; }
    case URSO_PB_FINALIZE_MAT: { ProfScope ps(st, URSO_K_FINALIZE, 0, 0);
        URSO_KLAUNCH(finalize_mat_batch_kernel, dim3(nblocks), dim3(256), 0, st, descs_d, blockmap_d, sqpart_d); break; }
    case URSO_PB_FINALIZE_VEC: { ProfScope ps(st, URSO_K_FINALIZE, 0, 0);
        URSO_KLAUNCH(finalize_vec_batch_kernel, dim3(nblocks), dim3(256), 0, st, descs_d, blockmap_d, sqpart_d); break; }
    default: urso_set_error("urso_param_batch_run: bad phase"); return URSO_EINVAL;
    }
    return urso_check_launch("urso_param_batch_run");
}

template <typename T>
__global__ void mold_kernel(size_t npix, int is_u8, const void* __restrict__ src, const float* __restrict__ mean, void* __restrict__ dst) {
    size_t i = (size_t)blockIdx.x * blockDim.x + threadIdx.x;
    const size_t stride = (size_t)gridDim.x * blockDim.x;
    const float m0 = mean ? mean[0] : 0.f, m1 = mean ? mean[1] : 0.f, m2 = mean ? mean[2] : 0.f;
    for (; i < npix; i += stride) {
        float a, b, c;
        if (is_u8) { const uint8_t* p = (const uint8_t*)src + i * 3; a = p[0]; b = p[1]; c = p[2]; }
        else { const float* p = (const float*)src + i * 3; a = p[0]; b = p[1]; c = p[2]; }
        T* o = (T*)dst + i * 4;
        o[0] = Elem<T>::from_f(a - m0); o[1] = Elem<T>::from_f(b - m1); o[2] = Elem<T>::from_f(c - m2); o[3] = Elem<T>::from_f(0.f);
    }
}

template <typename T>
__device__ __forceinline__ void mold8_body(size_t g, size_t ngroups, size_t stride, const uint8_t* __restrict__ src, float m0, float m1, float m2,
                                           T* __restrict__ dst) {
    for (; g < ngroups; g += stride) {
        const uint64_t* p = (const uint64_t*)(src + g * 24);
        const uint64_t q0 = p[0], q1 = p[1], q2 = p[2];
        uint8_t by[24];
        __builtin_memcpy(by, &q0, 8); __builtin_memcpy(by + 8, &q1, 8); __builtin_memcpy(by + 16, &q2, 8);
        T o[32];
#pragma unroll
        for (int k = 0; k < 8; ++k) {
            o[4 * k] = Elem<T>::from_f((float)by[3 * k] - m0); o[4 * k + 1] = Elem<T>::from_f((float)by[3 * k + 1] - m1);
            o[4 * k + 2] = Elem<T>::from_f((float)by[3 * k + 2] - m2); o[4 * k + 3] = Elem<T>::from_f(0.f);
        }
        i32x4_t v[4];
        __builtin_memcpy(v, o, 64);
        i32x4_t* d = (i32x4_t*)(dst + g * 32);
        d[0] = v[0]; d[1] = v[1]; d[2] = v[2]; d[3] = v[3];
    }
}
template <typename T>
__global__ __launch_bounds__(256) void mold8_kernel(size_t ngroups, const uint8_t* __restrict__ src, const float* __restrict__ mean, T* __restrict__ dst) {
    const float m0 = mean ? mean[0] : 0.f, m1 = mean ? mean[1] : 0.f, m2 = mean ? mean[2] : 0.f;
    mold8_body<T>((size_t)blockIdx.x * blockDim.x + threadIdx.x, ngroups, (size_t)gridDim.x * blockDim.x, src, m0, m1, m2, dst);
}

extern "C" int urso_mold_images(int B, int H, int W, int src_is_u8, const void* src_d, const float* mean3_d,
                                int dt, void* dst_d, void* stream) {
    if (!src_d || !dst_d || B <= 0 || H <= 0 || W <= 0) { urso_set_error("urso_mold_images: bad argument"); return URSO_EINVAL; }
    hipStream_t st = (hipStream_t)stream;
    const size_t npix = (size_t)B * H * W;
    if (src_is_u8 && (dt == URSO_BF16 || dt == URSO_F16) && npix % 8 == 0 && ((uintptr_t)src_d & 7) == 0 && ((uintptr_t)dst_d & 15) == 0 &&
        !g_urso_opt.mold_scalar) {
        const size_t ng = npix / 8;
        int blocks = (int)((ng + 255) / 256); if (blocks > 8192) blocks = 8192;
        ProfScope ps(st, URSO_K_MOLD, 0, (double)npix * (3 + 4 * dt_size(dt)));
        if (dt == URSO_BF16) URSO_KLAUNCH((mold8_kernel<__bf16>), dim3(blocks), dim3(256), 0, st, ng, (const uint8_t*)src_d, mean3_d, (__bf16*)dst_d);
        else URSO_KLAUNCH((mold8_kernel<_Float16>), dim3(blocks), dim3(256), 0, st, ng, (const uint8_t*)src_d, mean3_d, (_Float16*)dst_d);
        return urso_check_launch("urso_mold_images");
    }
    int blocks = (int)((npix + 255) / 256); if (blocks > 4096) blocks = 4096;
    ProfScope ps(st, URSO_K_MOLD, 0, (double)npix * ((src_is_u8 ? 3 : 12) + 4 * dt_size(dt)));
    if (dt == URSO_F32) URSO_KLAUNCH((mold_kernel<float>), dim3(blocks), dim3(256), 0, st, npix, src_is_u8, src_d, mean3_d, dst_d);
    else if (dt == URSO_BF16) URSO_KLAUNCH((mold_kernel<__bf16>), dim3(blocks), dim3(256), 0, st, npix, src_is_u8, src_d, mean3_d, dst_d);
    else if (dt == URSO_F16) URSO_KLAUNCH((mold_kernel<_Float16>), dim3(blocks), dim3(256), 0, st, npix, src_is_u8, src_d, mean3_d, dst_d);
    else { urso_set_error("urso_mold_images: bad dtype"); return URSO_EINVAL; }
    return urso_check_launch("urso_mold_images");
}
```

### ursonet_amd/engine.py

```python
import math
import os
import re
from collections import OrderedDict

import numpy as np
import torch

from . import hip
from .config import compute_dtype_name
from .graph import BN_EPS, build_graph, conv_flops
from .plan_state import _Act, _Conv, _PendingLaunches, _round_up

BN_MOMENTUM = 0.99

_DT = {"float32": hip.F32, "bfloat16": hip.BF16, "float16": hip.F16}


_SIDE_STREAMS = {}


def _side_stream(device):
    key = torch.device(device).index or 0
    if key not in _SIDE_STREAMS:
        _SIDE_STREAMS[key] = torch.cuda.Stream(device=device)
# ... 94 lines not shown

    def get_grads(self):
        out = OrderedDict()
        for (ln, wn) in self.slices:
            out.setdefault(ln, OrderedDict())[wn] = self.gview(ln, wn).detach().cpu().numpy().copy()
        return out

    def trainable_ranges(self):
        return [(o, o + n) for (ln, _), (o, n, _) in self.slices.items() if self.layer_trainable.get(ln, False)]

    def set_trainable(self, layer_regex):
        self.layer_trainable = {n: bool(re.fullmatch(layer_regex, n)) for n in self.graph.params}
        self._graphs = None
        self._build_plan()

    def _ptr_or_none(self, ln, wn):
        if ln is None or (ln, wn) not in self.slices and (ln, wn) not in self.stat_slices:
            return None
        return self.wview(ln, wn).reshape(-1)

    def _build_plan(self):
        training = self.mode == "training"
        self.plan_version += 1
        self._plan_options = self._planning_options()
        self._env_winograd = os.environ.get("URSO_WINOGRAD", "0") == "1"
        self._env_compact_grad = os.environ.get("URSO_COMPACT_GRAD", "1") != "0"
        self._env_sampled_outputs = os.environ.get("URSO_SAMPLED_OUTPUTS", "1") != "0"
        self._env_wgrad_group = int(os.environ.get("URSO_WGRAD_GROUP", "8"))
        self._env_fuse_sqnorm = os.environ.get("URSO_FUSE_SQNORM", "1") != "0"
        self._env_wgrad_stream = int(os.environ.get("URSO_WGRAD_STREAM", "0"))
        self.train_bn = training and self.config.TRAIN_BN is None
        self.acts = {}
        self.prep_ops, self.fwd_ops, self.loss_ops, self.bwd_ops, self.opt_ops = [], [], [], [], []
        self.wino_ws = None
        self.n_entry_dgrad2 = 0
        self.n_wgrad_groups = 0
        self._cleared_once = []
        self.loss_pre_ops = []
        self.labels = {"prep": [], "fwd": [], "loss": [], "bwd": [], "opt": []}
        self.convs = OrderedDict()
        self._descs = []
        self._fused_pools = {}
        self._plan_input()
        for node in self.graph.nodes:
            if node.op == "pool":
                self._plan_pool(node)
            else:
                self._plan_conv(node)
        self._fuse_pointwise_pairs()
        self._fuse_entry_shortcuts()
        self._fuse_dense_heads()
        self._plan_forward_workspaces()
        self.out_loc = self.acts[self.graph.outputs["loc"].id]
        self.out_ori = self.acts[self.graph.outputs["ori"].id] if "ori" in self.graph.outputs else None
        self._build_heads_io()
        if not training:
            for X in list(self.acts.values()):
                self._sample_block_output(X)
            return
        self._plan_stem_workspaces()
        self._build_losses()
        self._plan_relu_bitmasks()
        self._plan_backward()
        self._resolve_bucket_ops()
        self._plan_optimizer()
        self.flat_g.zero_()
        self._fork_weight_gradients()

    def _act(self, spec, numel=None):
        if spec.id not in self.acts:
            self.acts[spec.id] = _Act(self, spec, numel if numel is not None else self.B * spec.h * spec.w * spec.c, self.tdt)
        return self.acts[spec.id]

    def _plan_input(self):
        B, dt, dev = self.B, self.dt, self.device
        self.in_images = torch.zeros(B, self.H, self.W, 3, dtype=torch.float32, device=dev)
        mp = np.asarray(self.config.MEAN_PIXEL, dtype=np.float32)
        self.mean3 = torch.tensor(mp if mp.size == 3 else np.full(3, float(mp.mean()), dtype=np.float32), device=dev)
        x0 = self._act(self.graph.tensors[0], B * self.H * self.W * 4)
        self.fwd_ops.append(lambda: hip.mold_images(B, self.H, self.W, self.in_images_u8 if self.input_u8 else self.in_images,
                                                    self.mean3 if self.input_u8 else None, dt, x0.data))
        self.labels["fwd"].append("mold")

    def _plan_pool(self, node):
        if id(node) in self._fused_pools:
            return
        B, dt = self.B, self.dt
        src, dst = self._act(node.src), self._act(node.dst)
        am = torch.empty(dst.numel, dtype=torch.uint8, device=self.device)
        h, w, c = node.src.h, node.src.w, node.src.c
        self.fwd_ops.append(lambda s=src, d=dst, am=am, h=h, w=w, c=c: hip.maxpool_fwd(B, h, w, c, dt, s.data, d.data, am))
        self.labels["fwd"].append("maxpool")
        node._am = am

    def _plan_conv(self, node):
        B, dt, dev = self.B, self.dt, self.device
        training = self.mode == "training"
        c = _Conv(node)
        c.src = self._act(node.src) if not node.stem else self.acts[self.graph.tensors[0].id]
        out_elt = torch.float32 if node.out_f32 else self.tdt
        if node.dst.id not in self.acts:
            self.acts[node.dst.id] = _Act(self, node.dst, B * node.dst.h * node.dst.w * c.npad, out_elt)
        c.dst = self.acts[node.dst.id]
        c.res = self._act(node.residual) if node.residual is not None else None
        c.xin = c.src.data
        if node.stem:
            c.gf = hip.geom(B, self.H, self.W // 2, 8, node.dst.h, node.dst.w, c.npad, 7, 4, 2, 1, 3, 2)
            c.K_raw = 7 * 4 * 8
        elif node.dense:
            c.gf = hip.geom(B, 1, 1, node.cin, 1, 1, c.npad, 1, 1)
            c.gd = hip.geom(B, 1, 1, c.npad, 1, 1, node.cin, 1, 1)
            c.K_raw = node.cin
        else:
            s, (pt, pl) = node.stride, node.pad
            c.gf = hip.geom(B, node.src.h, node.src.w, node.cin, node.dst.h, node.dst.w, c.npad, node.kh, node.kw, s, s, pt, pl)
            if node.kh == 1 and node.kw == 1 and s > 1:
                c.gd = hip.geom(B, node.dst.h, node.dst.w, c.npad, node.dst.h, node.dst.w, node.cin, 1, 1,
                                FH=node.src.h, FW=node.src.w, OSH=s, OSW=s)
                c.gd_scatter = True
                c.gd_scatter_stride = s
            else:
                c.gd = hip.geom(B, node.dst.h, node.dst.w, c.npad, node.src.h, node.src.w, node.cin, node.kh, node.kw,
                                1, 1, node.kh - 1 - pt, node.kw - 1 - pl, s, s)
            c.K_raw = node.kh * node.kw * node.cin
            if (node.kh == 1 and node.kw == 1 and s == 2 and dt != hip.F32 and node.src.h % 2 == 0 and node.src.w % 2 == 0 and
                    (node.cin * 2) % 16 == 0):
                self._plan_compact_input(c)
        VE = 16 // (4 if dt == hip.F32 else 2)
        if node.cin % VE and not node.stem:
            raise ValueError("layer %s: %d input channels is not a multiple of %d" % (node.name, node.cin, VE))
        kelems = c.npad * c.K_raw
        c.wf = torch.empty(kelems, dtype=self.tdt, device=dev)
        need_dgrad = training and not node.stem
        c.wd = torch.empty(kelems, dtype=self.tdt, device=dev) if need_dgrad else None
        c.biasf = torch.empty(c.npad, dtype=torch.float32, device=dev)
        c.scale = torch.empty(c.npad, dtype=torch.float32, device=dev)
        c.w = self.wview(node.name, "kernel").reshape(-1)
        c.b = self._ptr_or_none(node.name, "bias") if node.bias else None
        c.gamma = self._ptr_or_none(node.bn, "gamma") if node.bn else None
        c.beta = self._ptr_or_none(node.bn, "beta") if node.bn else None
        c.mean = self._ptr_or_none(node.bn, "moving_mean") if node.bn else None
        c.var = self._ptr_or_none(node.bn, "moving_variance") if node.bn else None
        c.batch_bn = bool(self.train_bn and node.bn)
        if c.batch_bn:
            assert c.npad == c.N and not node.out_f32
            c.bn_gamma, c.bn_beta, c.bn_mmean, c.bn_mvar = c.gamma, c.beta, c.mean, c.var
            c.gamma = c.beta = c.mean = c.var = None
            c.Mpix = B * node.dst.h * node.dst.w
            c.z = torch.empty(c.Mpix * c.N, dtype=self.tdt, device=dev)
            c.dz = torch.empty(c.Mpix * c.N, dtype=self.tdt, device=dev)
            c.bmean, c.bvar = torch.empty(c.N, dtype=torch.float32, device=dev), torch.empty(c.N, dtype=torch.float32, device=dev)
            c.dbeta, c.dgamma = torch.empty(c.N, dtype=torch.float32, device=dev), torch.empty(c.N, dtype=torch.float32, device=dev)
        self.convs[node.name] = c
        if node.stem:
            self.prep_ops.append(lambda c=c: hip.stem_weight_pack(c.N, dt, c.w, c.b, c.gamma, c.beta, c.mean, c.var, BN_EPS,
                                                                  c.wf, c.biasf, c.scale))
            self.labels["prep"].append("prep:" + node.name)
        else:
            d = hip.ParamDesc()
            c.splits = hip.conv_wgrad_splits(c.gf, dt) if training else 1
            hip.param_desc_init(d, node.kh if not node.dense else 1, node.kw if not node.dense else 1, node.cin, c.N, c.npad,
                                max(c.splits, 1), BN_EPS, float(self.config.WEIGHT_DECAY))
            for f, t in (("w", c.w), ("b", c.b), ("gamma", c.gamma), ("beta", c.beta), ("mean", c.mean), ("var", c.var),
                         ("wf", c.wf), ("wd", c.wd), ("biasf", c.biasf), ("scale", c.scale)):
                setattr(d, f, hip.ptr(t))
            c.desc_id = len(self._descs)
            c.desc = d
            self._descs.append(d)
        self._plan_conv_forward(c)

    def _plan_compact_input(self, c):
        node, B, dt = c.node, self.B, self.dt
        X = c.src
        if X.data_compact is None:
            X.data_compact = torch.empty(X.numel // 4, dtype=self.tdt, device=self.device)
            P = [cc_ for cc_ in self.convs.values() if cc_.dst is X]
            Pc = P[0] if len(P) == 1 else None
            if (Pc is not None and not Pc.batch_bn and Pc.fwd_index is not None and hip.get_option("pair") and
                    hip.conv_pointwise_sampled_ok(Pc.gf, dt, Pc.fwd_flags | hip.EPI_EMIT_BITS, Pc.res is not None)):
                self.fwd_ops[Pc.fwd_index] = (lambda Pc=Pc, X=X: hip.conv_pointwise_sampled(
                    Pc.gf, dt, Pc.fwd_flags | (hip.EPI_EMIT_BITS if Pc.dst.bits is not None else 0), Pc.xin, Pc.wf, Pc.biasf,
                    Pc.res.data if Pc.res is not None else None, Pc.dst.data, Pc.dst.bits, X.data_compact))
                self.labels["fwd"][Pc.fwd_index] = "fwd:%s+sampled" % Pc.name
            else:
                self.fwd_ops.append(lambda X=X, hh=node.src.h, ww=node.src.w, rb=node.cin * 2:
                                    hip.rows_subsample2(B, hh, ww, rb, X.data, X.data_compact))
                self.labels["fwd"].append("subsample:T%d" % node.src.id)
        c.gf = hip.geom(B, node.dst.h, node.dst.w, node.cin, node.dst.h, node.dst.w, c.npad, 1, 1)
        c.xin = X.data_compact

    def _plan_conv_forward(self, c):
        node, dt, dev = c.node, self.dt, self.device
        training = self.mode == "training"
        flags = (hip.EPI_RELU if node.relu else 0) | (hip.EPI_OUT_F32 if node.out_f32 else 0)
        c.ws_f = hip.conv_igemm_ws_bytes(c.gf, dt)
        c.ws_d = hip.conv_igemm_ws_bytes(c.gd, dt) if (c.gd is not None and training) else 0
        c.fwd_flags = flags
        c.halo_f = (not c.batch_bn) and dt != hip.F32 and hip.conv_igemm_halo_ok(c.gf, dt, flags, c.res is not None)
        c.halo_d = bool(c.gd is not None and training and dt != hip.F32 and hip.conv_igemm_halo_ok(c.gd, dt, 0, False))
        if (c.halo_f or c.halo_d) and self.halo_ws is None:
            self.halo_ws = torch.zeros(hip.conv_igemm_halo_ws_bytes() // 4 + 16, dtype=torch.float32, device=dev)
        if c.batch_bn:
            self.fwd_ops.append(lambda c=c: hip.conv_igemm_ex(c.gf, dt, 0, c.xin, c.wf, c.biasf, None, None, c.z, None,
                                                              self.igemm_ws if c.ws_f else None))
            self.labels["fwd"].append("fwd:" + node.name)
            self.fwd_ops.append(lambda c=c: hip.bn_batch_stats(c.Mpix, c.N, dt, c.z, self.bn_ws, c.bmean, c.bvar, c.bn_mmean, c.bn_mvar,
                                                               BN_MOMENTUM, BN_EPS))
            self.labels["fwd"].append("bn_stats:" + node.name)
            self.fwd_ops.append(lambda c=c, n=node: hip.bn_apply(c.Mpix, c.N, dt, c.z, c.bmean, c.bvar, c.bn_gamma, c.bn_beta, BN_EPS,
                                                                 c.res.data if c.res is not None else None, n.relu, c.dst.data))
            self.labels["fwd"].append("bn_apply:" + node.name)
        elif (self._env_winograd and dt != hip.F32 and not node.stem and not node.dense and node.kh == 3 and node.kw == 3 and
              node.stride == 1 and tuple(node.pad) == (1, 1) and c.res is None and not (flags & ~hip.EPI_RELU) and c.npad == c.N and
              hip.conv_winograd_ws_bytes(c.gf, dt) > 0):
            need_ws = hip.conv_winograd_ws_bytes(c.gf, dt) // 4 + 64
            if self.wino_ws is None or self.wino_ws.numel() < need_ws:
                self.wino_ws = torch.empty(need_ws, dtype=torch.float32, device=dev)
            c.fwd_index = len(self.fwd_ops)
            self.fwd_ops.append(lambda c=c, f=flags: hip.conv_winograd_fwd(c.gf, dt, f, c.xin, c.wf, c.biasf, c.dst.data, self.wino_ws))
            self.labels["fwd"].append("fwd:" + node.name)
            c.winograd = True
        elif (pool := self._stem_pool_node(self.graph, node, c, dt)) is not None:
            self._fused_pools[id(pool)] = c
            pdst = self._act(pool.dst)
            pool._am = torch.empty(pdst.numel, dtype=torch.uint8, device=dev)
            c.dst.data = torch.empty(0, dtype=self.tdt, device=dev)
            c.dst.fused_pool = True
            c.fwd_index = len(self.fwd_ops)
            self.fwd_ops.append(lambda c=c, d=pdst, am=pool._am: hip.stem_conv_pool(c.gf, dt, c.xin, c.wf, c.biasf, d.data, am))
            self.labels["fwd"].append("fwd:%s+maxpool" % node.name)
        else:
            c.fwd_index = len(self.fwd_ops)
            self.fwd_ops.append(lambda c=c, f=flags: hip.conv_igemm_ex(
                c.gf, dt, f | (hip.EPI_EMIT_BITS if c.dst.bits is not None else 0), c.xin, c.wf, c.biasf,
                c.res.data if c.res is not None else None, None, c.dst.data, c.dst.bits,
                self.halo_ws if c.halo_f else (self.igemm_ws if c.ws_f else None)))
            self.labels["fwd"].append("fwd:" + node.name)

    def _plan_forward_workspaces(self):
        convs, dev = list(self.convs.values()), self.device
        max_igemm_ws = max([0] + [max(c.ws_f, c.ws_d) for c in convs])
        max_bn_ws = max([0] + [hip.bn_ws_bytes(c.Mpix, c.N) for c in convs if c.batch_bn])
        self.igemm_ws = torch.empty(max_igemm_ws // 4 + 16, dtype=torch.float32, device=dev)
        self.bn_ws = torch.empty(max_bn_ws // 8 + 32, dtype=torch.float64, device=dev) if max_bn_ws else None
        if self._descs:
            self.prep_ops.append(lambda: self.pbatch.run(hip.PB_PREP, "all", self.dt))
            self.labels["prep"].append("prep:batched[%d layers]" % len(self._descs))
        if self.mode != "training":
            self._upload_param_table()

    def _plan_stem_workspaces(self):
        stems = [c for c in self.convs.values() if c.node.stem]
        max_ws = max([0] + [hip.conv_wgrad_ws_bytes(c.gf, self.dt) for c in stems])
        max_fin_ws = max([0] + [hip.param_grad_finalize_ws_bytes(147, c.N) for c in stems])
        self.ws = torch.empty(max_ws // 4 + 64, dtype=torch.float32, device=self.device)
        self.fin_ws = torch.empty(max_fin_ws // 4 + 64, dtype=torch.float32, device=self.device)

    def _plan_buckets(self):
        from .dp import plan_buckets
        ext = {}
        for (ln, wn), (o, n, _) in self.slices.items():
            s0, e0 = ext.get(ln, (o, o))
            ext[ln] = (min(s0, o), max(e0, o + _round_up(n, 4)))
        self.buckets = plan_buckets(sorted(((ln, s0, e0) for ln, (s0, e0) in ext.items()), key=lambda t: t[1]), self.grad_bucket_bytes,
                                    tail_bytes=self.grad_tail_bytes)
        self.fused_sqnorm = (self._env_fuse_sqnorm and not self.no_fused_sqnorm and
                             len(self.buckets) == 1 and not any(c_.batch_bn for c_ in self.convs.values()))
        self._sq_slots = 0
        bucket_of = {ln: k for k, (_, _, names) in enumerate(self.buckets) for ln in names}
        groups = OrderedDict()
        for node in self._backward_order():
            if node.op == "pool" or node.stem:
                continue
            folded_bn = node.bn and not self.convs[node.name].batch_bn
            if self.layer_trainable[node.name] or (folded_bn and self.layer_trainable[node.bn]):
                groups.setdefault(bucket_of[node.name], []).append(node.name)
        self._last_of_group = {names[-1]: k for k, names in groups.items()}
        self._bucket_groups = groups

    def _plan_needed_gradients(self):
        g = self.graph
        need = {g.tensors[0].id: False}
        for node in g.nodes:
            if node.op == "pool":
                need[node.dst.id] = need.get(node.src.id, False)
            else:
                own = self.layer_trainable[node.name] or bool(node.bn and self.layer_trainable[node.bn])
                need[node.dst.id] = (own or (not node.stem and need.get(node.src.id, False)) or
                                     (node.residual is not None and need.get(node.residual.id, False)))
        self.grad_needed = need

    def _plan_backward(self):
        dt = self.dt
        q = _PendingLaunches(self, self._env_wgrad_group if dt != hip.F32 else 0)
        self._plan_buckets()
        self._plan_needed_gradients()
        need = self.grad_needed
        self._plan_compact_gradients(need)
        dense_lv = self._dense_levels() if self.dense_multi else {}
        for node in self._backward_order():
            lvl_n = dense_lv.get(node.name) if node.op != "pool" else None
            q.at_node(lvl_n)
            if not need[node.dst.id]:
                continue
            if node.op == "pool":
                self._plan_pool_backward(node)
                continue
            c = self.convs[node.name]
            assert c.dst.grad_written or c.dst.grad is not None, "no gradient reaches %s" % node.name
            G = c.dst.grad
            tr = self.layer_trainable[node.name]
            bn_tr = self.layer_trainable[node.bn] if node.bn else False
            Gsum = G
            if c.batch_bn:
                ggam, gbet = self.gview(node.bn, "gamma").reshape(-1), self.gview(node.bn, "beta").reshape(-1)
                self.bwd_ops.append((node.name, lambda c=c, G=G, bn_tr=bn_tr, ggam=ggam, gbet=gbet:
                                     hip.bn_backward(c.Mpix, c.N, dt, G, c.z, c.bmean, c.bvar, c.bn_gamma, BN_EPS, self.bn_ws, c.dbeta, c.dgamma,
                                                     bn_tr, gbet, ggam, c.dz)))
                self.labels["bwd"].append("bn_bwd:" + node.name)
                G = c.dz
                bn_tr = False
            if (tr or bn_tr) and node.stem:
                self._plan_stem_wgrad(c, G, tr, bn_tr)
            elif tr or bn_tr:
                self._plan_wgrad(c, G, tr, bn_tr, q, lvl_n)
            self._plan_residual_handover(c, Gsum)
            self._plan_dgrad(c, G, q, lvl_n)
        q.flush()

    def _plan_pool_backward(self, node):
        if not self.grad_needed[node.src.id]:
            return
        B, dt = self.B, self.dt
        src, dst = self.acts[node.src.id], self.acts[node.dst.id]
        h, w, cc = node.src.h, node.src.w, node.src.c
        assert dst.grad_written
        prod = [cc_ for cc_ in self.convs.values() if cc_.dst is src]
        if (len(prod) == 1 and prod[0].node.stem and not prod[0].batch_bn and dt != hip.F32 and hip.get_option("stem") and cc == 64 and
                h % 2 == 0 and w % 2 == 0 and (self.layer_trainable[prod[0].node.name] or bool(prod[0].node.bn and self.layer_trainable[prod[0].node.bn]))):
            prod[0].pooled_grad = (dst, node._am)
            src.grad_written = True
            return
        gsrc = src.grad_buf()
        self.bwd_ops.append((None, lambda d=dst, gs=gsrc, am=node._am, h=h, w=w, cc=cc:
                             hip.maxpool_bwd(B, h, w, cc, dt, d.data, d.grad, am, 1, gs)))
        self.labels["bwd"].append("maxpool_bwd")
        src.grad_written = True

    def _plan_stem_wgrad(self, c, G, tr, bn_tr):
        node, cfg, dt, dev = c.node, self.config, self.dt, self.device
        c.dw_raw = torch.empty(c.K_raw * c.npad, dtype=torch.float32, device=dev)
        c.colsum = torch.empty(c.npad, dtype=torch.float32, device=dev)
        if c.pooled_grad is not None:
            self.bwd_ops.append((node.name, lambda c=c, pg=c.pooled_grad: hip.stem_wgrad_pooled(c.gf, dt, c.src.data, pg[0].grad, pg[1], self.ws,
                                                                                                c.dw_raw, c.colsum)))
            self.labels["bwd"].append("wgrad:%s+maxpool_bwd" % node.name)
        else:
            self.bwd_ops.append((node.name, lambda c=c, G=G: hip.conv_wgrad(c.gf, dt, c.src.data, G, self.ws, c.dw_raw, c.colsum)))
            self.labels["bwd"].append("wgrad:" + node.name)
        c.dw_unp = torch.empty(147 * c.N, dtype=torch.float32, device=dev)
        self.bwd_ops.append((node.name, lambda c=c: hip.stem_wgrad_unpack(c.N, c.dw_raw, c.dw_unp)))
        self.labels["bwd"].append("unpack:" + node.name)
        gw = self.gview(node.name, "kernel").reshape(-1)
        gb = self.gview(node.name, "bias").reshape(-1) if node.bias else None
        gg = self.gview(node.bn, "gamma").reshape(-1) if (node.bn and not c.batch_bn) else None
        gbe = self.gview(node.bn, "beta").reshape(-1) if (node.bn and not c.batch_bn) else None
        if self.fused_sqnorm:
            s0 = self._sq_slots
            s1 = self._sq_slots = s0 + hip.param_grad_finalize_sq_slots(147, c.N)
            self.bwd_ops.append((node.name, lambda c=c, gw=gw, gb=gb, gg=gg, gbe=gbe, tr=tr, bn_tr=bn_tr, s0=s0, s1=s1:
                                 hip.param_grad_finalize_sq(147, c.N, c.N, c.dw_unp, c.colsum, c.w, c.b, c.gamma, c.mean, c.var, BN_EPS,
                                                            float(cfg.WEIGHT_DECAY), tr, bn_tr, gw, gb, gg, gbe, self.fin_ws, self.sqpart[s0:s1])))
        else:
            self.bwd_ops.append((node.name, lambda c=c, gw=gw, gb=gb, gg=gg, gbe=gbe, tr=tr, bn_tr=bn_tr:
                                 hip.param_grad_finalize(147, c.N, c.N, c.dw_unp, c.colsum, c.w, c.b, c.gamma, c.mean, c.var, BN_EPS,
                                                         float(cfg.WEIGHT_DECAY), tr, bn_tr, gw, gb, gg, gbe, self.fin_ws)))
        self.labels["bwd"].append("finalize:" + node.name)

    def _plan_wgrad(self, c, G, tr, bn_tr, q, lvl_n):
        node, d, B, dt, dev = c.node, c.desc, self.B, self.dt, self.device
        gf_w = c.gf_compact or c.gf
        Xs = c.src
        Ms = B * node.dst.h * node.dst.w
        c.solo = (hip.get_option("pair") == 1 and dt != hip.F32 and not node.dense and node.kh == 1 and node.kw == 1 and node.stride == 1 and
                  node.cin == 64 and c.npad == 256 and c.N == 256 and not c.batch_bn and self.grad_needed[Xs.spec.id] and
                  not c.wgrad_by_pair and not c.dgrad_done_by_pair and
                  c.gf_compact is None and c.dst.compact is None and Xs.compact is None and not c.gd_scatter and
                  not Xs.grad_written and Xs.pending is None and self.pair_first.get(node.name) is None and node.name not in self._last_of_group and
                  hip.conv_pair_wgrad_splits(Ms, dt) > 1)
        if c.solo:
            c.splits = c.desc.splits = hip.conv_pair_wgrad_splits(Ms, dt)
        n_part = c.splits * (c.K_raw * c.npad + hip.WGRAD_PART_PAD)
        by_pair = c.wgrad_by_pair or c.solo
        c.wg_npart = n_part
        c.wg_ws = torch.empty((n_part + c.splits * c.npad if by_pair else hip.conv_wgrad_ws_bytes(gf_w, dt) // 4) + 64,
                              dtype=torch.float32, device=dev)
        c.dw_raw = torch.empty(c.K_raw * c.npad, dtype=torch.float32, device=dev) if c.splits > 1 else None
        c.colsum = torch.empty(c.npad, dtype=torch.float32, device=dev) if c.splits > 1 else None
        c.dotpart = torch.empty(d.ks * c.N + 16, dtype=torch.float32, device=dev)
        d.part, d.colpart = c.wg_ws.data_ptr(), c.wg_ws.data_ptr() + 4 * n_part
        d.dw_raw, d.colsum, d.dotpart = hip.ptr(c.dw_raw), hip.ptr(c.colsum), hip.ptr(c.dotpart)
        d.trainable, d.bn_trainable = int(tr), int(bn_tr)
        d.gw = hip.ptr(self.gview(node.name, "kernel").reshape(-1))
        d.gb = hip.ptr(self.gview(node.name, "bias").reshape(-1)) if node.bias else None
        d.ggamma = hip.ptr(self.gview(node.bn, "gamma").reshape(-1)) if (node.bn and not c.batch_bn) else None
        d.gbeta = hip.ptr(self.gview(node.bn, "beta").reshape(-1)) if (node.bn and not c.batch_bn) else None
        if not by_pair:
            xw = c.xin if gf_w is c.gf else c.src.data
            if q.wg_max > 1 and gf_w.KH * gf_w.KW * gf_w.C == c.K_raw and gf_w.N == c.npad and hip.conv_wgrad_pair_splits(gf_w, gf_w, dt):
                q.add_wgrad_pair((c, node.name, xw, G, gf_w))
            elif q.wg_max > 1 and hip.wgrad_group_fits(gf_w, dt) and gf_w.KH * gf_w.KW * gf_w.C == c.K_raw and gf_w.N == c.npad:
                q.add_wgrad_group((c, node.name, xw, G, gf_w))
            elif lvl_n is not None and c.splits == 1 and gf_w is c.gf and self._dense_multi_ok(c):
                q.add_dense_wgrad(dict(name=node.name, x=xw, dz=G, part=c.wg_ws, colpart=c.wg_ws[c.wg_npart:], M=B, K=c.K_raw, N=c.npad))
            else:
                q.emit_wgrad(c, node.name, xw, G, gf_w)
        if node.name in self._last_of_group:
            q.flush_bucket()
            k = self._last_of_group[node.name]
            for ph, nm in ((hip.PB_REDUCE, "reduce"), (hip.PB_FINALIZE_MAT, "finalize_mat"), (hip.PB_FINALIZE_VEC, "finalize_vec")):
                self.bwd_ops.append((tuple(self._bucket_groups[k]), (ph, k)))
                self.labels["bwd"].append("%s:bucket%d" % (nm, k))

    def _plan_residual_handover(self, c, Gsum):
        if c.res is None or not self.grad_needed[c.res.spec.id]:
            return
        B, node = self.B, c.node
        R = c.res
        if R.grad_written or R.pending is not None:
            raise AssertionError("unexpected second residual consumer for %s" % node.name)
        if R.spec.relu and c.dst.compact is not None and c.dst.residual_needs_dense:
            c.dst.grad_dense = torch.zeros(c.dst.numel, dtype=self.tdt, device=self.device)
            self.bwd_ops.append((None, lambda X=c.dst: hip.rows_scatter2(B, X.compact[0], X.compact[1], X.spec.c * 2, X.grad, X.grad_dense)))
            self.labels["bwd"].append("expand:" + node.name)
            R.pending = c.dst.grad_dense
        elif R.spec.relu:
            R.pending = Gsum
            R.pending_hw = c.dst.compact
        else:
            assert c.dst.compact is None
            R.grad, R.grad_written = Gsum, True

    def _plan_dgrad(self, c, G, q, lvl_n):
        node = c.node
        if c.dgrad_done_by_pair or node.stem or not self.grad_needed[c.src.spec.id]:
            return
        B, dt = self.B, self.dt
        X = c.src
        add = X.grad if X.grad_written else X.pending
        if c.solo:
            assert add is None
            dstg = X.grad_buf()
            self.bwd_ops.append((node.name, lambda c=c, G=G, X=X, dstg=dstg, Ms=B * node.dst.h * node.dst.w:
                                 hip.conv_dgrad_wgrad_pw(Ms, dt, G, c.wd, X.data, X.spec.relu, dstg, c.wg_ws, c.wg_ws[c.wg_npart:],
                                                         c.K_raw * c.npad + hip.WGRAD_PART_PAD)))
            self.labels["bwd"].append("dgrad+wgrad:" + node.name)
            X.grad_written = True
            return
        if X.compact is not None:
            self._dgrad_compact(c, G, X)
            return
        A = self.pair_first.get(node.name)
        if (A is not None and X.spec.relu and X.bits is not None and X.pending is not None and not X.grad_written and
                self.grad_needed[A.src.spec.id] and A.src.spec.relu and A.src.bits is None and not A.src.grad_written and A.src.pending is None):
            self._dgrad_pair(c, A, G, X, add)
            return
        assert X.pending_hw is None or X.grad_written, "compact residual gradient reached a non-fused data gradient (%s)" % node.name
        dstg = X.grad_buf()
        mask = (X.bits if X.bits is not None else X.data) if X.spec.relu else None
        mflag = hip.EPI_MASK_BITS if (X.spec.relu and X.bits is not None) else 0
        if lvl_n is not None and mflag == 0 and not c.gd_scatter and self._dense_multi_ok(c):
            q.add_dense_dgrad(dict(name=node.name, level=lvl_n, src0=G, wgt0=c.wd, K0=c.npad, N=node.cin, M=B, add=add, mask=mask, dst=dstg, flags=0))
            X.grad_written, X.pending = True, None
            return
        if c.gd_scatter:
            if add is None:
                self._clear_scattered_dgrad(c, X, dstg)
            elif add is not dstg:
                raise AssertionError("scattered dgrad into %s needs an in-place accumulate" % node.name)
        self.bwd_ops.append((None, lambda c=c, G=G, add=add, mask=mask, dstg=dstg, mflag=mflag:
                             hip.conv_igemm_ex(c.gd, dt, mflag, G, c.wd, None, add, mask, dstg, None,
                                               self.halo_ws if (c.halo_d and add is None and not mflag) else (self.igemm_ws if c.ws_d else None))))
        self.labels["bwd"].append("dgrad:" + node.name)
        X.grad_written, X.pending = True, None

    def _dgrad_compact(self, c, G, X):
        B, dt, node = self.B, self.dt, c.node
        if not X.grad_written and not X.fwd_sampled:
            self.bwd_ops.append((None, lambda X=X: hip.rows_subsample2(B, X.compact[0], X.compact[1], X.spec.c // 8, X.bits, X.bits_compact)))
            self.labels["bwd"].append("bits_subsample")
        gq = c.gd_compact
        first = X._compact_first
        if (first is not None and X.grad_written and
                hip.conv_pointwise2_ok(B, gq.OH, gq.OW, first[1].npad, c.npad, node.cin, dt, hip.EPI_MASK_BITS)):
            i0, c0, G0 = first
            self.bwd_ops[i0] = (None, lambda: None)
            self.labels["bwd"][i0] = None
            self.bwd_ops.append((None, lambda c=c, c0=c0, G0=G0, G=G, X=X, gq=gq, N=node.cin:
                                 hip.conv_pointwise2(B, gq.OH, gq.OW, c0.npad, c.npad, N, dt, hip.EPI_MASK_BITS, G0, c0.wd, G, c.wd, None,
                                                     X.bits_compact, X.grad)))
            self.labels["bwd"].append("dgrad:%s+%s" % (c0.name, node.name))
            X._compact_first = None
            self.n_entry_dgrad2 += 1
            return
        if not X.grad_written:
            X._compact_first = (len(self.bwd_ops), c, G)
        else:
            X._compact_first = None
        self.bwd_ops.append((None, lambda c=c, G=G, X=X, add=(X.grad if X.grad_written else None):
                             hip.conv_igemm_ex(c.gd_compact, dt, hip.EPI_MASK_BITS, G, c.wd, None, add, X.bits_compact, X.grad, None, None)))
        self.labels["bwd"].append("dgrad:" + node.name)
        X.grad_written = True

    def _dgrad_pair(self, c, A, G, X, add):
        dt, node = self.dt, c.node
        dstg, dst2 = X.grad_buf(), A.src.grad_buf()
        a_tr = self.layer_trainable[A.name] or bool(A.node.bn and not A.batch_bn and self.layer_trainable[A.node.bn])
        wsplits = hip.conv_pair_wgrad_splits(A.Mpix, dt) if (A.node.cin == 64 and hip.get_option("pair") == 1) else 0
        if a_tr and wsplits > 1 and A.gf_compact is None:
            A.splits = A.desc.splits = wsplits
            A.wgrad_by_pair = True
            Sc = self._pair_entry_shortcut(A, X)
            if Sc is not None:
                Sc.splits = Sc.desc.splits = wsplits
                Sc.wgrad_by_pair = Sc.dgrad_done_by_pair = True
                dxin = Sc.src.grad_buf()
                Sc.src.grad_written = True
                dstg.zero_()
                dstg._urso_on_chip = True
                self.bwd_ops.append((None, lambda c=c, A=A, Sc=Sc, G=G, add=add, X=X, dst2=dst2, dxin=dxin:
                                     hip.conv_pair_wgrad_entry(A.Mpix, dt, G, c.wd, add, X.bits, A.wd, A.src.data, dst2, Sc.wd, Sc.src.data, Sc.src.spec.relu, dxin,
                                                               A.wg_ws, A.wg_ws[A.wg_npart:], Sc.wg_ws, Sc.wg_ws[Sc.wg_npart:],
                                                               A.K_raw * A.npad + hip.WGRAD_PART_PAD)))
                self.labels["bwd"].append("dgrad:%s+%s+%s+wgrad:%s+%s" % (node.name, A.name, Sc.name, A.name, Sc.name))
            else:
                self.bwd_ops.append((None, lambda c=c, A=A, G=G, add=add, X=X, dstg=dstg, dst2=dst2, hw=X.pending_hw:
                                     hip.conv_pair_wgrad(A.Mpix, dt, G, c.wd, add, X.bits, dstg, A.wd, A.src.data, dst2,
                                                         A.wg_ws, A.wg_ws[A.wg_npart:], A.K_raw * A.npad + hip.WGRAD_PART_PAD, add_hw=hw)))
                self.labels["bwd"].append("dgrad:%s+%s+wgrad:%s" % (node.name, A.name, A.name))
        else:
            self.bwd_ops.append((None, lambda c=c, A=A, G=G, add=add, X=X, dstg=dstg, dst2=dst2, hw=X.pending_hw:
                                 hip.conv_pair(A.Mpix, A.node.cin, dt, 1, G, c.wd, None, add, X.bits, dstg, A.wd, None, A.src.data, dst2,
                                               add_hw=hw)))
            self.labels["bwd"].append("dgrad:%s+%s" % (node.name, A.name))
        X.grad_written, X.pending = True, None
        A.src.grad_written = True
        A.dgrad_done_by_pair = True

    def _pair_entry_shortcut(self, A, X):
        S = [cc for cc in self.convs.values() if A.res is not None and cc.dst is A.res]
        Sc = S[0] if len(S) == 1 else None
        if Sc is None:
            return None
        sn = Sc.node
        entry = (X.pending_hw is None and not sn.stem and not sn.dense and sn.kh == 1 and sn.kw == 1 and
                 sn.stride == 1 and sn.cin == 64 and Sc.npad == 256 and Sc.N == 256 and not Sc.batch_bn and not sn.relu and
                 (self.layer_trainable[sn.name] or bool(sn.bn and self.layer_trainable[sn.bn])) and
                 self.grad_needed[Sc.src.spec.id] and Sc.src.compact is None and not Sc.gd_scatter and
                 Sc.gf_compact is None and not Sc.src.grad_written and Sc.src.pending is None and
                 sn.name not in self._last_of_group and self.pair_first.get(sn.name) is None)
        return Sc if entry else None

    def _clear_scattered_dgrad(self, c, X, dstg):
        g = self.graph
        dstg.zero_()
        writers = [cc for cc in self.convs.values() if cc.src is X and cc.gd is not None]
        once = (all(cc.gd_scatter for cc in writers) and not any(cc.res is X for cc in self.convs.values())
                and not any(n.op == "pool" and n.src.id == X.spec.id for n in g.nodes)
                and not any(t.id == X.spec.id for t in g.outputs.values()))
        if not once:
            self.bwd_ops.append((None, lambda t=dstg: hip.zero_fill(t)))
            self.labels["bwd"].append("zero:" + c.name)
        else:
            st = c.gd_scatter_stride
            self._cleared_once.append((c.name, dstg, X.spec.h, X.spec.w, X.spec.c, st, st))

    def _resolve_bucket_ops(self):
        dt = self.dt
        self._upload_param_table()
        resolved, labels = [], []
        assert len(self.bwd_ops) == len(self.labels["bwd"])
        for (tag, op), lab in zip(self.bwd_ops, self.labels["bwd"]):
            if isinstance(op, tuple):
                ph, k = op
                ids = [self.convs[nm].desc_id for nm in self._bucket_groups[k]]
                nb_ = self.pbatch.plan(ph, k, ids)
                if nb_ == 0:
                    continue
                if self.fused_sqnorm and ph in (hip.PB_FINALIZE_MAT, hip.PB_FINALIZE_VEC):
                    s0 = self._sq_slots
                    s1 = self._sq_slots = s0 + nb_
                    op = (lambda ph=ph, k=k, s0=s0, s1=s1: self.pbatch.run(ph, k, dt, sqpart=self.sqpart[s0:s1]))
                else:
                    op = (lambda ph=ph, k=k: self.pbatch.run(ph, k, dt))
            resolved.append((tag, op)); labels.append(lab)
        self.bwd_ops, self.labels["bwd"] = resolved, labels
        self.sqpart = torch.zeros(max(self._sq_slots, 1), dtype=torch.float32, device=self.device) if self.fused_sqnorm else None

    def _plan_optimizer(self):
        cfg, dev = self.config, self.device
        n = self.n_flat
        self.adam = str(getattr(cfg, "OPTIMIZER", "SGD")).upper() != "SGD"
        clip = float(cfg.GRADIENT_CLIP_NORM or 0.0)
        if self.adam:
            eps = 1e-4 if getattr(cfg, "F16", False) else 1e-7
            if self.hyper is None or self.hyper.numel() != 8:
                self.hyper = torch.tensor([float(cfg.LEARNING_RATE), 0.9, 0.999, eps, clip, 0.0, 1.0 - 0.9, 1.0 - 0.999],
                                          dtype=torch.float32, device=dev)
            if self.flat_v2 is None or self.flat_v2.numel() != self.flat_w.numel():
                self.flat_v2, self.flat_vhat = torch.zeros_like(self.flat_w), torch.zeros_like(self.flat_w)
        elif self.hyper is None or self.hyper.numel() != 3:
            self.hyper = torch.tensor([float(cfg.LEARNING_RATE), float(cfg.LEARNING_MOMENTUM), clip], dtype=torch.float32, device=dev)
        self.normsq = torch.zeros(1, dtype=torch.float32, device=dev)
        self.sq_ws = torch.empty(hip.sqnorm_ws_bytes(n) // 4, dtype=torch.float32, device=dev)
        if self.fused_sqnorm:
            self.opt_ops.append(lambda: hip.sqnorm_final(self.sqpart, self.normsq))
        else:
            self.opt_ops.append(lambda: hip.sqnorm(n, self.flat_g, self.sq_ws, self.normsq))
        if self.adam:
            self.opt_ops.append(lambda: hip.adam_amsgrad_clip(n, self.flat_w, self.flat_g, self.flat_v, self.flat_v2, self.flat_vhat,
                                                              self.hyper, self.normsq))
        else:
            self.opt_ops.append(lambda: hip.sgd_momentum_clip(n, self.flat_w, self.flat_g, self.flat_v, self.hyper, self.normsq))
        self.labels["opt"] += ["sqnorm", "adam" if self.adam else "sgd"]

    def _fork_weight_gradients(self):
        self.wgrad_stream = None
        self._single_chain_always = False
        self._graph_events = []
        if self._env_wgrad_stream != 2 or self.mode != "training" or self.no_wgrad_fork:
            return
        labs = self.labels["bwd"]
        assert len(labs) == len(self.bwd_ops)
        fin = ("reduce", "finalize_mat", "finalize_vec", "finalize", "unpack")
        if any(c.batch_bn for c in self.convs.values()):
            return
        es = 4 if self.dt == hip.F32 else 2

        def work(name, back=False):
            c = self.convs.get(name)
            g = c.gf if c is not None else None
            if g is None:
                return 0.0, 0.0
            m_out, m_in, k = g.B * g.OH * g.OW, g.B * g.H * g.W, g.KH * g.KW * g.C
            return 2.0 * m_out * k * g.N, (m_in * g.C + m_out * g.N) * es + (es if back else 4.0) * k * g.N

        def names(lab):
            return [n for part in lab.split("+wgrad:")[0:1] + lab.split("+wgrad:")[1:] for n in part.split(":", 1)[-1].split("+") if n != "maxpool_bwd"]

        def totals(lab, back=False):
            fl = by = 0.0
            for n in names(lab):
                f, b = work(n, back)
                fl += f; by += b
            return fl, by

        def est_ms(lab):
            fl, by = totals(lab, lab.startswith("dgrad"))
            return max(fl / 1.0e12, by / 4.5e9)

        def intensity(lab):
            fl, by = totals(lab)
            return fl / by if by else 1e9

        def wg(lab):
            return lab is not None and lab.startswith(("wgrad:", "wgrad_heads:")) and "dgrad" not in lab
        at = next((i for i, l in enumerate(labs) if l is not None and re.match(r"dgrad:res[23]", l)), None)
        if at is None:
            return
        EARLY, LATE = 150.0, 400.0
        room = 1.2 * sum(est_ms(l) for l in labs[at:] if l is not None and l.startswith(("dgrad:", "wgrad:")) and not (wg(l) and intensity(l) >= LATE))
        early = []
        for i in range(at - 1, -1, -1):
            if wg(labs[i]) and (labs[i].startswith("wgrad_heads:") or intensity(labs[i]) >= EARLY):
                room -= est_ms(labs[i])
                if room < 0:
                    break
                early.append(i)
        early.reverse()
        if not early or any(labs[i] is not None and labs[i].split(":")[0] in fin for i in range(early[0], at)):
            return
        moved = set(early)
        late = set(i for i in range(at, len(labs)) if wg(labs[i]) and intensity(labs[i]) >= LATE)
        side_ids = set(id(self.bwd_ops[i]) for i in moved | late)
        order = [i for i in range(at) if i not in moved] + early + list(range(at, len(labs)))
        self.bwd_ops = [self.bwd_ops[i] for i in order]
        self.labels["bwd"] = [labs[i] for i in order]
        self.wgrad_stream = _side_stream(self.device)
        self._side_open = False
        self._main_moved = True
        self._single_chain = False

        def on_side(op):
            def run():
                if self._single_chain or self._single_chain_always:
                    return op()
                main = torch.cuda.current_stream(self.device)
                if self._main_moved or not self._side_open:
                    self._stream_edge(main, self.wgrad_stream)
                    self._main_moved = False
                with torch.cuda.stream(self.wgrad_stream):
                    op()
                self._side_open = True
            return run

        def joined(op):
            def run():
                self._join_weight_gradients()
                self._main_moved = True
                return op()
            return run

        def on_main(op):
            def run():
                self._main_moved = True
                return op()
            return run
        ops = []
        for item, lab in zip(self.bwd_ops, self.labels["bwd"]):
            tag, op = item
            if id(item) in side_ids:
                op = on_side(op)
            elif lab is not None and lab.split(":")[0] in fin:
                op = joined(op)
            elif callable(op):
                op = on_main(op)
            ops.append((tag, op))
        self.bwd_ops = ops
        self.opt_ops[0] = joined(self.opt_ops[0])

    def _stream_edge(self, src, dst):
        ev = torch.cuda.Event()
        ev.record(src)
        dst.wait_event(ev)
        if torch.cuda.is_current_stream_capturing():
            self._graph_events.append(ev)

    def _join_weight_gradients(self):
        if self.wgrad_stream is not None and self._side_open:
            self._stream_edge(self.wgrad_stream, torch.cuda.current_stream(self.device))
            self._side_open = False

    def _plan_relu_bitmasks(self):
        dt = self.dt
        for X in self.acts.values():
            X.bits = None
            if not X.spec.relu or X.numel % 8:
                continue
            prod = [c for c in self.convs.values() if c.dst is X]
            cons = [c for c in self.convs.values() if c.src is X and c.gd is not None]
            if len(prod) != 1 or not cons or not prod[0].node.relu:
                continue
            P = prod[0]
            pw = lambda n: (not n.dense) and n.kh == 1 and n.kw == 1
            bn_ = lambda c: (hip.get_option("bneck") and not c.node.dense and c.node.kh == 3 and c.node.kw == 3 and c.node.stride == 2 and
                             c.npad == 32 and c.node.cin % 64 == 0 and not c.batch_bn)
            if not (pw(P.node) and P.node.stride == 1 and P.N % 32 == 0 and all(pw(c.node) or bn_(c) for c in cons)):
                continue
            if P.res is None:
                continue
            if not hip.conv_igemm_bits_ok(P.gf, dt, P.fwd_flags, P.ws_f):
                continue
            if all(hip.conv_igemm_bits_ok(c.gd, dt, 0, c.ws_d) for c in cons):
                X.bits = torch.empty(X.numel // 8, dtype=torch.uint8, device=self.device)

    def _upload_param_table(self):
        self.pbatch = hip.ParamBatch(self._descs, self.device) if self._descs else None
        if self.pbatch is not None:
            self.pbatch.plan(hip.PB_PREP, "all", list(range(len(self._descs))))

    def _build_heads_io(self):
        cfg, B, dev = self.config, self.B, self.device
        self.quat_head = bool(cfg.REGRESS_ORI and cfg.ORIENTATION_PARAM == "quaternion" and not cfg.REGRESS_KEYPOINTS)
        if self.quat_head:
            self.q_out = torch.zeros(B, 4, dtype=torch.float32, device=dev)
            if self.mode == "inference":
                x = self.out_ori
# ... 612 lines not shown
```

### ursonet_amd/hip.py

```python
import ctypes as C
import os

import torch

_HERE = os.path.dirname(os.path.abspath(__file__))
_VARIANT = os.environ.get("URSO_LIB_VARIANT", "")
LIB_PATH = os.path.join(_HERE, "lib", "liburso_hip%s.so" % (("_" + _VARIANT) if _VARIANT else ""))

F32, BF16, F16 = 0, 1, 2
EPI_RELU, EPI_OUT_F32, EPI_MASK_BITS, EPI_EMIT_BITS, EPI_ADD_SRCGRID = 1, 2, 4, 8, 16
K_IGEMM, K_WGRAD, K_PREP, K_FINALIZE, K_POOL, K_LOSS, K_OPTIM, K_DECODE, K_MOLD = range(1, 10)
KERNEL_NAMES = {K_IGEMM: "conv_igemm", K_WGRAD: "conv_wgrad", K_PREP: "weight_prep", K_FINALIZE: "param_grad_finalize",
                K_POOL: "maxpool", K_LOSS: "loss", K_OPTIM: "optimizer", K_DECODE: "quat_decode", K_MOLD: "mold"}

TORCH_DT = {F32: torch.float32, BF16: torch.bfloat16, F16: torch.float16}
DT_OF_TORCH = {v: k for k, v in TORCH_DT.items()}
DT_NAME = {F32: "f32", BF16: "bf16", F16: "f16"}


class ConvGeom(C.Structure):
    _fields_ = [(n, C.c_int32) for n in
                ("B", "H", "W", "C", "OH", "OW", "N", "KH", "KW", "SH", "SW", "PH", "PW", "DH", "DW",
                 "FH", "FW", "OSH", "OSW")]

    def __repr__(self):
        return "ConvGeom(" + ", ".join("%s=%d" % (n, getattr(self, n)) for n, _ in self._fields_) + ")"


class ProfRecord(C.Structure):
    _fields_ = [("kernel_id", C.c_int32), ("ms", C.c_float), ("flops", C.c_double), ("bytes", C.c_double)]


import threading
capture_lock = threading.RLock()


class ProfRecordEx(C.Structure):
    _fields_ = [("kernel_id", C.c_int32), ("ms", C.c_float), ("flops", C.c_double), ("bytes", C.c_double), ("n_launches", C.c_int32),
                ("symbol", C.c_char * 228), ("l2_bytes", C.c_double)]


class UrsoHipError(RuntimeError):
    pass


if not os.path.exists(LIB_PATH):
    raise ImportError("liburso_hip.so not found at %s -- build it with `python -m ursonet_amd.build` "
                      "(hipcc --offload-arch=gfx950). There is no CPU fallback." % LIB_PATH)
_lib = C.CDLL(LIB_PATH)

_vp, _fp, _i, _f, _sz = C.c_void_p, C.c_void_p, C.c_int, C.c_float, C.c_size_t
_gp = C.POINTER(ConvGeom)


class ParamDesc(C.Structure):
    _fields_ = ([(n, C.c_int32) for n in ("KH", "KW", "C", "N", "npad", "K", "splits", "ks", "kb", "trainable", "bn_trainable", "bias_from")] +
                [(n, C.c_float) for n in ("eps", "regc", "regb")] +
                [(n, C.c_void_p) for n in ("w", "b", "gamma", "beta", "mean", "var", "wf", "wd", "biasf", "scale", "part", "colpart",
                                           "dw_raw", "colsum", "dotpart", "gw", "gb", "ggamma", "gbeta")])


class DenseLayer(C.Structure):
    _fields_ = ([(n, C.c_void_p) for n in ("src0", "wgt0", "src1", "wgt1", "bias", "add", "mask", "dst")] +
                [(n, C.c_int32) for n in ("M", "N", "K0", "K1", "flags")])


class PoseEvalArgs(C.Structure):
    _fields_ = ([("B", C.c_int32), ("n", C.c_int32), ("row0", C.c_int64)] +
                [(n, C.c_int32) for n in ("loc_mode", "ori_mode", "loc_ld", "ori_ld", "loc_bins", "loc_map_rows", "ori_bins", "ori_map_rows",
                                          "gmm_modes", "pad0")] +
                [(n, C.c_void_p) for n in ("loc", "ori", "ori2", "loc_map", "ori_map", "enc_loc", "enc_ori", "loc_gt", "q_gt", "gmm_mean",
                                           "gmm_nmodes", "table")])


EVAL_LOC_REGRESS, EVAL_LOC_CLASS = 0, 1
EVAL_ORI_QUAT, EVAL_ORI_EULER, EVAL_ORI_ANGLE_AXIS, EVAL_ORI_SOFT, EVAL_ORI_KEYPOINTS = range(5)
EVAL_LOC_EST, EVAL_Q_EST, EVAL_LOC_ERR, EVAL_ORI_ERR, EVAL_ESA, EVAL_DIST = 0, 3, 7, 8, 9, 10
EVAL_LOC_ENC_ERR, EVAL_ORI_ENC_ERR, EVAL_ORI_ERR_SOFT, EVAL_MODE, EVAL_COLS = 11, 12, 13, 14, 16


class PoseDecodeArgs(C.Structure):
    _fields_ = ([("B", C.c_int32), ("n", C.c_int32), ("row0", C.c_int64)] +
                [(n, C.c_int32) for n in ("loc_mode", "ori_mode", "loc_ld", "ori_ld", "loc_bins", "loc_map_rows", "ori_bins", "ori_map_rows",
                                          "ori_logits_ld", "pad0")] +
                [(n, C.c_void_p) for n in ("loc", "ori", "ori2", "loc_map", "ori_logits", "ori_scatter", "table")])


DEC_LOC_EST, DEC_Q_EST, DEC_LOC_PEAK, DEC_ORI_PEAK, DEC_ORI_LAMBDA, DEC_COLS = 0, 3, 7, 8, 9, 12


class DenseWgradLayer(C.Structure):
    _fields_ = [(n, C.c_void_p) for n in ("x", "dz", "part", "colpart")] + [(n, C.c_int32) for n in ("M", "K", "N")]


DENSE_MULTI_MAX = 4
PB_PREP, PB_REDUCE, PB_FINALIZE_MAT, PB_FINALIZE_VEC = 0, 1, 2, 3
WGRAD_PART_PAD = 64
_dp = C.POINTER(ParamDesc)
_SIGS = {
    "urso_last_error": (C.c_char_p, []),
    "urso_abi_version": (_i, []),
    "urso_set_option": (_i, [C.c_char_p, _i]),
    "urso_get_option": (_i, [C.c_char_p, C.POINTER(C.c_int)]),
    "urso_conv_igemm": (_i, [_gp, _i, _i, _vp, _vp, _fp, _vp, _vp, _vp, _vp]),
    "urso_conv_igemm_ws_bytes": (_sz, [_gp, _i]),
    "urso_conv_igemm_ws": (_i, [_gp, _i, _i, _vp, _vp, _fp, _vp, _vp, _vp, _vp, _sz, _vp]),
    "urso_conv_igemm_bits_ok": (_i, [_gp, _i, _i, _sz]),
    "urso_conv_igemm_algorithmic": (_i, [_gp, _i, _i, _i, _i, C.POINTER(C.c_double), C.POINTER(C.c_double)]),
    "urso_conv_igemm_halo_ok": (_i, [_gp, _i, _i, _i]),
    "urso_conv_igemm_halo2_shape": (_i, [_gp, _i, _i, _i, _i]),
    "urso_conv_igemm_halo_ws_bytes": (_sz, []),
    "urso_conv_igemm_ex": (_i, [_gp, _i, _i, _vp, _vp, _fp, _vp, _vp, _vp, _vp, _vp, _sz, _vp]),
    "urso_conv_wgrad_ws_bytes": (_sz, [_gp, _i]),
    "urso_conv_wgrad": (_i, [_gp, _i, _vp, _vp, _vp, _sz, _fp, _fp, _vp]),
    "urso_conv_wgrad_splits": (_i, [_gp, _i]),
    "urso_conv_wgrad_partial": (_i, [_gp, _i, _vp, _vp, _vp, _sz, _vp]),
    "urso_param_desc_init": (_i, [_dp, _i, _i, _i, _i, _i, _i, _f, _f]),
    "urso_param_batch_plan": (_i, [_i, _dp, C.POINTER(C.c_int32), _i, C.POINTER(C.c_int32), _i]),
    "urso_wgrad_group_fits": (_i, [_gp, _i]),
    "urso_conv_wgrad_pair_splits": (_i, [_gp, _gp, _i, C.POINTER(C.c_int), C.POINTER(C.c_int)]),
    "urso_conv_wgrad_partial2": (_i, [_gp, _gp, _i, _vp, _vp, _vp, _sz, _vp, _vp, _vp, _sz, _vp]),
    "urso_wgrad_group_plan": (_i, [_i, _vp, _i, C.POINTER(C.c_int32), _i]),
    "urso_wgrad_group_run": (_i, [_i, _vp, _vp, _i, _vp, _i, _vp]),
    "urso_param_batch_run": (_i, [_i, _i, _vp, _vp, _i, _vp]),
    "urso_conv_weight_prep": (_i, [_i, _i, _i, _i, _i, _i, _fp, _fp, _fp, _fp, _fp, _fp, _f, _vp, _vp, _fp, _fp, _vp]),
    "urso_stem_weight_pack": (_i, [_i, _i, _fp, _fp, _fp, _fp, _fp, _fp, _f, _vp, _fp, _fp, _vp]),
    "urso_stem_wgrad_unpack": (_i, [_i, _fp, _fp, _vp]),
    "urso_param_grad_finalize": (_i, [_i, _i, _i, _fp, _fp, _fp, _fp, _fp, _fp, _fp, _f, _f, _i, _i,
                                      _fp, _fp, _fp, _fp, _fp, _sz, _vp]),
    "urso_param_grad_finalize_ws_bytes": (_sz, [_i, _i]),
    "urso_param_grad_finalize_sq": (_i, [_i, _i, _i, _fp, _fp, _fp, _fp, _fp, _fp, _fp, _f, _f, _i, _i,
                                         _fp, _fp, _fp, _fp, _fp, _sz, _fp, _vp]),
    "urso_param_grad_finalize_sq_slots": (_i, [_i, _i]),
    "urso_param_batch_run_sq": (_i, [_i, _i, _vp, _vp, _i, _fp, _vp]),
    "urso_sqnorm_final": (_i, [_i, _fp, _fp, _vp]),
    "urso_bn_ws_bytes": (_sz, [_i, _i]),
    "urso_bn_batch_stats": (_i, [_i, _i, _i, _vp, _vp, _sz, _fp, _fp, _fp, _fp, _f, _f, _vp]),
    "urso_bn_apply": (_i, [_i, _i, _i, _vp, _fp, _fp, _fp, _fp, _f, _vp, _i, _vp, _vp]),
    "urso_bn_backward": (_i, [_i, _i, _i, _vp, _vp, _fp, _fp, _fp, _f, _vp, _sz, _fp, _fp, _i, _fp, _fp, _vp, _vp]),
    "urso_mold_images": (_i, [_i, _i, _i, _i, _vp, _fp, _i, _vp, _vp]),
    "urso_maxpool3x3s2_fwd": (_i, [_i, _i, _i, _i, _i, _vp, _vp, _vp, _vp]),
    "urso_maxpool3x3s2_bwd": (_i, [_i, _i, _i, _i, _i, _vp, _vp, _vp, _i, _vp, _vp]),
    "urso_softmax_xent_fwd_bwd": (_i, [_i, _i, _fp, _fp, _f, _i, _i, _fp, _vp, _fp, _vp]),
    "urso_rel_l2_fwd_bwd": (_i, [_i, _i, _i, _fp, _fp, _f, _i, _fp, _vp, _fp, _vp]),
    "urso_rel_l2_norms": (_i, [_i, _i, _i, _fp, _fp, _fp, _vp]),
    "urso_rel_l2_from_norms": (_i, [_i, _i, _i, _fp, _fp, _f, _fp, _i, _fp, _fp, _vp, _vp]),
    "urso_absdot_fwd_bwd": (_i, [_i, _i, _i, _i, _fp, _fp, _f, _i, _fp, _fp, _vp, _vp]),
    "urso_mse_fwd_bwd": (_i, [_i, _i, _i, _fp, _fp, _f, _i, _fp, _vp, _vp]),
    "urso_sqnorm_ws_bytes": (_sz, [_sz]),
    "urso_sqnorm": (_i, [_sz, _fp, _vp, _sz, _fp, _vp]),
    "urso_sgd_momentum_clip": (_i, [_sz, _fp, _fp, _fp, _fp, _fp, _vp]),
    "urso_adam_amsgrad_clip": (_i, [_sz, _fp, _fp, _fp, _fp, _fp, _fp, _fp, _vp]),
    "urso_scale_f32": (_i, [_sz, _fp, _f, _vp]),
    "urso_quat_wavg_decode": (_i, [_i, _i, _fp, _fp, _fp, _fp, _vp]),
    "urso_quat_gmm_fit": (_i, [_i, _i, _fp, _i, _fp, _f, _i, _i, _fp, _fp, _fp, _fp, _vp, _vp]),
    "urso_pose_eval": (_i, [C.POINTER(PoseEvalArgs), _vp]),
    "urso_pose_decode": (_i, [C.POINTER(PoseDecodeArgs), _vp]),
    "urso_warp_perspective": (_i, [_i, _i, _i, _i, _i, _vp, _vp, _vp, _vp]),
    "urso_encode_ori": (_i, [_i, _i, _vp, _fp, _vp, C.c_double, _fp, _vp]),
    "urso_encode_loc": (_i, [_i, _i, _vp, _vp, C.c_double, _fp, _vp]),
    "urso_comm_unique_id": (_i, [_vp]),
    "urso_comm_init": (_i, [C.POINTER(_vp), _i, _i, _vp]),
    "urso_comm_allreduce_bucket": (_i, [_vp, _vp, _sz, _i, _vp]),
    "urso_comm_wait": (_i, [_vp, _vp]),
    "urso_comm_destroy": (_i, [_vp]),
    "urso_bucket_round_ef": (_i, [_sz, _fp, _fp, _vp, _vp]),
    "urso_dense_multi": (_i, [_i, C.POINTER(DenseLayer), _i, _vp]),
    "urso_dense_wgrad_multi": (_i, [_i, C.POINTER(DenseWgradLayer), _i, _vp]),
    "urso_bucket_expand_bf16": (_i, [_sz, _vp, _fp, _vp]),
    "urso_conv_pair_ok": (_i, [C.c_longlong, _i, _i, _i]),
    "urso_conv_pair": (_i, [C.c_longlong, _i, _i, _i, _vp, _vp, _fp, _vp, _vp, _vp, _vp, _fp, _vp, _vp, _i, _i, _vp]),
    "urso_conv_pair_shortcut": (_i, [C.c_longlong, _i, _vp, _vp, _fp, _vp, _vp, _fp, _vp, _vp, _vp, _fp, _vp, _vp]),
    "urso_conv_dgrad_wgrad_pw": (_i, [C.c_longlong, _i, _vp, _vp, _vp, _i, _vp, _fp, _fp, _sz, _vp]),
    "urso_conv_pair_wgrad_entry": (_i, [C.c_longlong, _i, _vp, _vp, _vp, _vp, _vp, _vp, _vp, _vp, _vp, _i, _vp, _fp, _fp, _fp, _fp, _sz, _vp]),
    "urso_stem_wgrad_pooled": (_i, [_gp, _i, _vp, _vp, _vp, _vp, _sz, _fp, _fp, _vp]),
    "urso_stem_conv_pool_ok": (_i, [_gp, _i]),
    "urso_stem_conv_pool": (_i, [_gp, _i, _vp, _vp, _fp, _vp, _vp, _vp]),
    "urso_conv_pair_wgrad_splits": (_i, [C.c_longlong, _i]),
    "urso_conv_pair_wgrad": (_i, [C.c_longlong, _i, _vp, _vp, _vp, _vp, _vp, _vp, _vp, _vp, _i, _i, _fp, _fp, _sz, _vp]),
    "urso_conv_pointwise_sampled_ok": (_i, [_gp, _i, _i, _i]),
    "urso_conv_pointwise_sampled": (_i, [_gp, _i, _i, _vp, _vp, _fp, _vp, _vp, _vp, _vp, _vp]),
    "urso_rows_subsample2": (_i, [_i, _i, _i, _i, _vp, _vp, _vp]),
    "urso_rows_expand2": (_i, [_i, _i, _i, _i, _vp, _vp, _vp]),
    "urso_rows_scatter2": (_i, [_i, _i, _i, _i, _vp, _vp, _vp]),
    "urso_zero_fill": (_i, [_vp, C.c_size_t, _vp]),
    "urso_rgb_to_grey3": (_i, [_i, _i, _i, _vp, _vp, _vp]),
    "urso_sim2real_op": (_i, [_i, _i, _i, _vp, _vp, _vp, _fp, _vp, _vp, _i, _vp]),
    "urso_pad_images_u8": (_i, [_i, _i, _i, _i, _i, _i, _i, _i, _vp, _vp, _vp]),
    "urso_resize_images_u8": (_i, [_i] * 10 + [_vp, _i, _vp, _i, _vp, _vp, _vp, _vp, _i, _vp, _vp, _vp]),
    "urso_frames_grey_flags_u8": (_i, [_i, _i, _vp, _vp, _vp]),
    "urso_frames_put_u8": (_i, [_i, _i, _vp, _vp, _vp, _vp]),
    "urso_frames_gather_u8": (_i, [_i, _i, _vp, _vp, _vp, _vp]),
    "urso_video_prep_u8": (_i, [_i] * 8 + [C.c_double] * 3 + [_vp, _vp, _vp]),
    "urso_draw_prims_u8": (_i, [_i, _i, _i, _vp, _vp, _vp, _vp, _vp, _vp]),
    "urso_pmf_sheet_u8": (_i, [_i, _i, _i, _i, _fp, _fp, _vp, _vp, _vp, _vp, _vp]),
    "urso_conv_winograd_ws_bytes": (_sz, [_gp, _i]),
    "urso_conv_winograd_fwd": (_i, [_gp, _i, _i, _vp, _vp, _fp, _vp, _vp, _sz, _vp]),
    "urso_prof_enable": (_i, [_i]),
    "urso_prof_collect": (_i, [C.POINTER(ProfRecord), _i]),
    "urso_prof_collect_ex": (_i, [C.POINTER(ProfRecordEx), _i]),
    "urso_conv_pointwise2_ok": (_i, [_i] * 8),
    "urso_conv_pointwise2": (_i, [_i] * 8 + [_vp, _vp, _vp, _vp, _fp, _vp, _vp, _vp, _vp]),
}
EXPORTED_SYMBOLS = sorted(_SIGS)
for _name, (_res, _args) in _SIGS.items():
    _fn = getattr(_lib, _name)
    _fn.restype = _res
    _fn.argtypes = _args


def last_error():
    return (_lib.urso_last_error() or b"").decode()
# ... 43 lines not shown
    if t is None:
        return None
    assert t.is_cuda and t.is_contiguous(), "expected a contiguous device tensor"
    return t.data_ptr()


def stream_ptr(stream=None):
    s = stream if stream is not None else torch.cuda.current_stream()
    return s.cuda_stream


def geom(B, H, W, Cin, OH, OW, N, KH, KW, SH=1, SW=1, PH=0, PW=0, DH=1, DW=1, FH=0, FW=0, OSH=0, OSW=0):
    return ConvGeom(B, H, W, Cin, OH, OW, N, KH, KW, SH, SW, PH, PW, DH, DW, FH, FW, OSH, OSW)


def conv_igemm(g, dt, flags, src, wgt, bias, add, mask, dst, stream=None):
    _chk(_lib.urso_conv_igemm(C.byref(g), dt, flags, ptr(src), ptr(wgt), ptr(bias), ptr(add), ptr(mask), ptr(dst),
                              stream_ptr(stream)), "urso_conv_igemm")


class DenseMulti(object):

    def __init__(self, layers, dt):
        assert 1 <= len(layers) <= DENSE_MULTI_MAX
        self.dt, self.n = dt, len(layers)
        self.host = (DenseLayer * self.n)()
        self.keep = []
        for it, L in zip(self.host, layers):
            for f in ("src0", "wgt0", "src1", "wgt1", "bias", "add", "mask", "dst"):
                t = L.get(f)
                self.keep.append(t)
                setattr(it, f, t.data_ptr() if t is not None else None)
            it.M, it.N, it.K0, it.K1, it.flags = int(L["M"]), int(L["N"]), int(L["K0"]), int(L.get("K1", 0)), int(L.get("flags", 0))

    def run(self, stream=None):
        _chk(_lib.urso_dense_multi(self.n, self.host, self.dt, stream_ptr(stream)), "urso_dense_multi")


class DenseWgradMulti(object):

    def __init__(self, layers, dt):
        assert 1 <= len(layers) <= DENSE_MULTI_MAX
        self.dt, self.n = dt, len(layers)
        self.host = (DenseWgradLayer * self.n)()
        self.keep = []
        for it, L in zip(self.host, layers):
            assert L["part"].dtype == torch.float32 and L["part"].numel() >= L["K"] * L["N"]
            for f in ("x", "dz", "part", "colpart"):
                t = L.get(f)
                self.keep.append(t)
                setattr(it, f, t.data_ptr() if t is not None else None)
            it.M, it.K, it.N = int(L["M"]), int(L["K"]), int(L["N"])

    def run(self, stream=None):
        _chk(_lib.urso_dense_wgrad_multi(self.n, self.host, self.dt, stream_ptr(stream)), "urso_dense_wgrad_multi")


def bucket_round_ef(g, resid, c, stream=None):
    assert g.dtype == torch.float32 and resid.dtype == torch.float32 and c.dtype == torch.bfloat16 and g.numel() == resid.numel() == c.numel()
    _chk(_lib.urso_bucket_round_ef(g.numel(), ptr(g), ptr(resid), ptr(c), stream_ptr(stream)), "urso_bucket_round_ef")


def bucket_expand_bf16(c, g, stream=None):
    assert g.dtype == torch.float32 and c.dtype == torch.bfloat16 and g.numel() == c.numel()
    _chk(_lib.urso_bucket_expand_bf16(g.numel(), ptr(c), ptr(g), stream_ptr(stream)), "urso_bucket_expand_bf16")


def conv_winograd_ws_bytes(g, dt):
    return int(_lib.urso_conv_winograd_ws_bytes(C.byref(g), dt))


def conv_winograd_fwd(g, dt, flags, src, wgt, bias, dst, ws, stream=None):
    _chk(_lib.urso_conv_winograd_fwd(C.byref(g), dt, flags, ptr(src), ptr(wgt), ptr(bias), ptr(dst), ptr(ws), ws.numel() * ws.element_size(),
                                     stream_ptr(stream)), "urso_conv_winograd_fwd")


def conv_igemm_ws_bytes(g, dt):
    return int(_lib.urso_conv_igemm_ws_bytes(C.byref(g), dt))


def conv_igemm_ws(g, dt, flags, src, wgt, bias, add, mask, dst, ws, stream=None):
    _chk(_lib.urso_conv_igemm_ws(C.byref(g), dt, flags, ptr(src), ptr(wgt), ptr(bias), ptr(add), ptr(mask), ptr(dst),
                                 ptr(ws), ws.numel() * ws.element_size() if ws is not None else 0, stream_ptr(stream)),
         "urso_conv_igemm_ws")


def conv_igemm_bits_ok(g, dt, flags, ws_bytes=0):
    return bool(_lib.urso_conv_igemm_bits_ok(C.byref(g), dt, flags, ws_bytes))


def conv_igemm_halo_ws_bytes():
    return int(_lib.urso_conv_igemm_halo_ws_bytes())


def conv_igemm_halo_ok(g, dt, flags, has_add=False):
    return bool(_lib.urso_conv_igemm_halo_ok(C.byref(g), dt, flags, int(bool(has_add))))


def conv_igemm_algorithmic(g, dt, flags, has_add=False, has_mask=False):
    fl, by = C.c_double(0), C.c_double(0)
    _chk(_lib.urso_conv_igemm_algorithmic(C.byref(g), dt, flags, int(bool(has_add)), int(bool(has_mask)), C.byref(fl), C.byref(by)), "urso_conv_igemm_algorithmic")
    return float(fl.value), float(by.value)


def conv_igemm_halo2_shape(g, dt, flags, has_add=False, has_ws=False):
    return int(_lib.urso_conv_igemm_halo2_shape(C.byref(g), dt, flags, int(bool(has_add)), int(bool(has_ws))))


def conv_igemm_ex(g, dt, flags, src, wgt, bias, add, mask, dst, bits_out=None, ws=None, stream=None):
    _chk(_lib.urso_conv_igemm_ex(C.byref(g), dt, flags, ptr(src), ptr(wgt), ptr(bias), ptr(add), ptr(mask), ptr(dst), ptr(bits_out),
                                 ptr(ws), (ws.numel() * ws.element_size()) if ws is not None else 0, stream_ptr(stream)), "urso_conv_igemm_ex")


def conv_pointwise2_ok(B, OH, OW, C0, C1, N, dt, flags):
    return bool(_lib.urso_conv_pointwise2_ok(B, OH, OW, C0, C1, N, dt, flags))


def conv_pointwise2(B, OH, OW, C0, C1, N, dt, flags, src0, wgt0, src1, wgt1, bias, mask, dst, bits_out=None, stream=None):
    _chk(_lib.urso_conv_pointwise2(B, OH, OW, C0, C1, N, dt, flags, ptr(src0), ptr(wgt0), ptr(src1), ptr(wgt1), ptr(bias), ptr(mask), ptr(dst),
                                   ptr(bits_out), stream_ptr(stream)), "urso_conv_pointwise2")


def conv_wgrad_ws_bytes(g, dt):
    return int(_lib.urso_conv_wgrad_ws_bytes(C.byref(g), dt))


def conv_wgrad(g, dt, x, dz, ws, dw_raw, colsum, stream=None):
    _chk(_lib.urso_conv_wgrad(C.byref(g), dt, ptr(x), ptr(dz), ptr(ws), ws.numel() * ws.element_size(), ptr(dw_raw),
                              ptr(colsum), stream_ptr(stream)), "urso_conv_wgrad")


def conv_wgrad_splits(g, dt):
    return int(_lib.urso_conv_wgrad_splits(C.byref(g), dt))


def conv_wgrad_partial(g, dt, x, dz, ws, stream=None):
    _chk(_lib.urso_conv_wgrad_partial(C.byref(g), dt, ptr(x), ptr(dz), ptr(ws), ws.numel() * ws.element_size(), stream_ptr(stream)),
         "urso_conv_wgrad_partial")


def param_desc_init(d, KH, KW, Cin, N, npad, splits, eps, weight_decay):
    _chk(_lib.urso_param_desc_init(C.byref(d), KH, KW, Cin, N, npad, splits, eps, weight_decay), "urso_param_desc_init")


class ParamBatch(object):

    def __init__(self, descs, device):
        self.n = len(descs)
        self.host = (ParamDesc * self.n)(*descs)
        raw = torch.frombuffer(bytearray(bytes(self.host)), dtype=torch.uint8)
        self.dev = raw.to(device)
        self.maps = {}

    def plan(self, phase, key, layer_ids):
        ids = (C.c_int32 * len(layer_ids))(*layer_ids)
        nb = _lib.urso_param_batch_plan(phase, self.host, ids, len(layer_ids), None, 0)
        if nb < 0:
            raise UrsoHipError("urso_param_batch_plan: " + last_error())
        buf = (C.c_int32 * (2 * max(nb, 1)))()
        _lib.urso_param_batch_plan(phase, self.host, ids, len(layer_ids), buf, nb)
        t = torch.frombuffer(bytearray(bytes(buf)), dtype=torch.int32).to(self.dev.device)
        self.maps[(phase, key)] = (t, nb)
        return nb

    def run(self, phase, key, dt, stream=None, sqpart=None):
        t, nb = self.maps[(phase, key)]
        if nb and sqpart is not None:
            assert sqpart.dtype == torch.float32 and sqpart.numel() >= nb
            _chk(_lib.urso_param_batch_run_sq(phase, dt, ptr(self.dev), ptr(t), nb, ptr(sqpart), stream_ptr(stream)), "urso_param_batch_run_sq")
        elif nb:
            _chk(_lib.urso_param_batch_run(phase, dt, ptr(self.dev), ptr(t), nb, stream_ptr(stream)), "urso_param_batch_run")

    def nblocks(self, phase, key):
        return self.maps[(phase, key)][1]


def conv_wgrad_pair_splits(g0, g1, dt):
    a, b = C.c_int(0), C.c_int(0)
    ok = _lib.urso_conv_wgrad_pair_splits(C.byref(g0), C.byref(g1), dt, C.byref(a), C.byref(b))
    return (a.value, b.value) if ok else None


def conv_wgrad_partial2(g0, g1, dt, x0, dz0, ws0, x1, dz1, ws1, stream=None):
    _chk(_lib.urso_conv_wgrad_partial2(C.byref(g0), C.byref(g1), dt, ptr(x0), ptr(dz0), ptr(ws0), ws0.numel() * ws0.element_size(),
                                       ptr(x1), ptr(dz1), ptr(ws1), ws1.numel() * ws1.element_size(), stream_ptr(stream)), "urso_conv_wgrad_partial2")


class WgradItem(C.Structure):
    _fields_ = [("x", C.c_void_p), ("dz", C.c_void_p), ("part", C.c_void_p), ("colpart", C.c_void_p), ("g", ConvGeom),
                ("M", C.c_int32), ("ktiles", C.c_int32), ("ntiles", C.c_int32), ("splits", C.c_int32), ("m_per_split", C.c_int32),
                ("mode", C.c_int32), ("fill", C.c_int32)]


def wgrad_group_fits(g, dt):
    return bool(_lib.urso_wgrad_group_fits(C.byref(g), dt))


class WgradGroup(object):

    def __init__(self, geoms, dt):
        self.n, self.dt = len(geoms), dt
        self.host = (WgradItem * self.n)()
        for it, g in zip(self.host, geoms):
            C.memmove(C.byref(it.g), C.byref(g), C.sizeof(ConvGeom))
        nb = _lib.urso_wgrad_group_plan(self.n, self.host, dt, None, 0)
        if nb < 0:
            raise UrsoHipError("urso_wgrad_group_plan: " + last_error())
        self.nblocks = nb
        self.splits = [int(it.splits) for it in self.host] if nb else []
        self.fill = self.host[0].fill / 1000.0 if nb else 0.0
        self.dev = self.map = None

    def bind(self, xs, dzs, wss, device):
        buf = (C.c_int32 * (2 * self.nblocks))()
        if _lib.urso_wgrad_group_plan(self.n, self.host, self.dt, buf, self.nblocks) != self.nblocks:
            raise UrsoHipError("urso_wgrad_group_plan: " + last_error())
        for it, x, dz, ws in zip(self.host, xs, dzs, wss):
            n_part = it.splits * (it.g.KH * it.g.KW * it.g.C * it.g.N + WGRAD_PART_PAD)
            if ws.numel() * ws.element_size() < 4 * (n_part + it.splits * it.g.N):
                raise UrsoHipError("WgradGroup.bind: workspace too small")
            it.x, it.dz, it.part, it.colpart = x.data_ptr(), dz.data_ptr(), ws.data_ptr(), ws.data_ptr() + 4 * n_part
        self.keep = (list(xs), list(dzs), list(wss))
        self.dev = torch.frombuffer(bytearray(bytes(self.host)), dtype=torch.uint8).to(device)
        self.map = torch.frombuffer(bytearray(bytes(buf)), dtype=torch.int32).to(device)

    def run(self, stream=None):
        _chk(_lib.urso_wgrad_group_run(self.dt, ptr(self.dev), C.cast(self.host, C.c_void_p), self.n, ptr(self.map), self.nblocks,
                                       stream_ptr(stream)), "urso_wgrad_group_run")


def bn_ws_bytes(M, N):
    return int(_lib.urso_bn_ws_bytes(M, N))


def bn_batch_stats(M, N, dt, z, ws, mean, var, mmean, mvar, momentum, eps, stream=None):
    _chk(_lib.urso_bn_batch_stats(M, N, dt, ptr(z), ptr(ws), ws.numel() * ws.element_size(), ptr(mean), ptr(var), ptr(mmean), ptr(mvar),
                                  momentum, eps, stream_ptr(stream)), "urso_bn_batch_stats")


def bn_apply(M, N, dt, z, mean, var, gamma, beta, eps, res, relu, y, stream=None):
    _chk(_lib.urso_bn_apply(M, N, dt, ptr(z), ptr(mean), ptr(var), ptr(gamma), ptr(beta), eps, ptr(res), int(relu), ptr(y), stream_ptr(stream)),
         "urso_bn_apply")


def bn_backward(M, N, dt, g, z, mean, var, gamma, eps, ws, dbeta, dgamma, bn_trainable, gbeta, ggamma, dz, stream=None):
    _chk(_lib.urso_bn_backward(M, N, dt, ptr(g), ptr(z), ptr(mean), ptr(var), ptr(gamma), eps, ptr(ws), ws.numel() * ws.element_size(),
                               ptr(dbeta), ptr(dgamma), int(bn_trainable), ptr(gbeta), ptr(ggamma), ptr(dz), stream_ptr(stream)), "urso_bn_backward")


def conv_weight_prep(KH, KW, Cin, N, npad, dt, w, b, gamma, beta, mean, var, eps, wf, wd, biasf, scale, stream=None):
    _chk(_lib.urso_conv_weight_prep(KH, KW, Cin, N, npad, dt, ptr(w), ptr(b), ptr(gamma), ptr(beta), ptr(mean), ptr(var),
                                    eps, ptr(wf), ptr(wd), ptr(biasf), ptr(scale), stream_ptr(stream)),
         "urso_conv_weight_prep")


def stem_weight_pack(N, dt, w, b, gamma, beta, mean, var, eps, wf, biasf, scale, stream=None):
    _chk(_lib.urso_stem_weight_pack(N, dt, ptr(w), ptr(b), ptr(gamma), ptr(beta), ptr(mean), ptr(var), eps, ptr(wf),
                                    ptr(biasf), ptr(scale), stream_ptr(stream)), "urso_stem_weight_pack")


def stem_wgrad_unpack(N, dw_packed, dw_raw, stream=None):
    _chk(_lib.urso_stem_wgrad_unpack(N, ptr(dw_packed), ptr(dw_raw), stream_ptr(stream)), "urso_stem_wgrad_unpack")


def param_grad_finalize_ws_bytes(K, N):
    return int(_lib.urso_param_grad_finalize_ws_bytes(K, N))


def param_grad_finalize(K, N, ldn, dw_raw, colsum, w, b, gamma, mean, var, eps, wd, trainable, bn_trainable,
                        gw, gb, ggamma, gbeta, ws, stream=None):
    _chk(_lib.urso_param_grad_finalize(K, N, ldn, ptr(dw_raw), ptr(colsum), ptr(w), ptr(b), ptr(gamma), ptr(mean),
                                       ptr(var), eps, wd, int(trainable), int(bn_trainable), ptr(gw), ptr(gb),
                                       ptr(ggamma), ptr(gbeta), ptr(ws), ws.numel() * ws.element_size(),
                                       stream_ptr(stream)), "urso_param_grad_finalize")


def param_grad_finalize_sq_slots(K, N):
    return int(_lib.urso_param_grad_finalize_sq_slots(K, N))


def param_grad_finalize_sq(K, N, ldn, dw_raw, colsum, w, b, gamma, mean, var, eps, wd, trainable, bn_trainable,
                           gw, gb, ggamma, gbeta, ws, sqpart, stream=None):
    assert sqpart.dtype == torch.float32 and sqpart.numel() >= param_grad_finalize_sq_slots(K, N)
    _chk(_lib.urso_param_grad_finalize_sq(K, N, ldn, ptr(dw_raw), ptr(colsum), ptr(w), ptr(b), ptr(gamma), ptr(mean),
                                          ptr(var), eps, wd, int(trainable), int(bn_trainable), ptr(gw), ptr(gb),
                                          ptr(ggamma), ptr(gbeta), ptr(ws), ws.numel() * ws.element_size(), ptr(sqpart),
                                          stream_ptr(stream)), "urso_param_grad_finalize_sq")


def sqnorm_final(parts, out, stream=None):
    assert parts.dtype == torch.float32 and out.dtype == torch.float32
    _chk(_lib.urso_sqnorm_final(parts.numel(), ptr(parts), ptr(out), stream_ptr(stream)), "urso_sqnorm_final")


def mold_images(B, H, W, src, mean3, dt, dst, stream=None):
    is_u8 = 1 if src.dtype == torch.uint8 else 0
    assert is_u8 or src.dtype == torch.float32
    _chk(_lib.urso_mold_images(B, H, W, is_u8, ptr(src), ptr(mean3), dt, ptr(dst), stream_ptr(stream)), "urso_mold_images")


def maxpool_fwd(B, H, W, Cc, dt, x, y, argmax, stream=None):
    _chk(_lib.urso_maxpool3x3s2_fwd(B, H, W, Cc, dt, ptr(x), ptr(y), ptr(argmax), stream_ptr(stream)), "urso_maxpool3x3s2_fwd")


def maxpool_bwd(B, H, W, Cc, dt, y, dy, argmax, relu_mask, dx, stream=None):
    _chk(_lib.urso_maxpool3x3s2_bwd(B, H, W, Cc, dt, ptr(y), ptr(dy), ptr(argmax), int(relu_mask), ptr(dx),
                                    stream_ptr(stream)), "urso_maxpool3x3s2_bwd")


def softmax_xent(B, K, logits, labels, weight, relu_mask, dt, loss, dz, row_ws, stream=None):
    _chk(_lib.urso_softmax_xent_fwd_bwd(B, K, ptr(logits), ptr(labels), weight, int(relu_mask), dt, ptr(loss), ptr(dz),
                                        ptr(row_ws), stream_ptr(stream)), "urso_softmax_xent_fwd_bwd")


def rel_l2_norms(B, D, ld, gt, pred, norms, stream=None):
    _chk(_lib.urso_rel_l2_norms(B, D, ld, ptr(gt), ptr(pred), ptr(norms), stream_ptr(stream)), "urso_rel_l2_norms")


def rel_l2_from_norms(B, D, ld, gt, pred, weight, gscale, dt, norms, loss, dpred, stream=None):
    _chk(_lib.urso_rel_l2_from_norms(B, D, ld, ptr(gt), ptr(pred), weight, ptr(gscale), dt, ptr(norms), ptr(loss), ptr(dpred),
                                     stream_ptr(stream)), "urso_rel_l2_from_norms")
# ... 320 lines not shown
```

### ursonet_amd/plan_state.py

```python
import torch

from . import hip


def _round_up(v, m):
    return (v + m - 1) // m * m


class _Act(object):

    def __init__(self, eng, spec, numel, dtype):
        self.spec, self.numel = spec, numel
        self.fused_pool = False
        self.data = torch.empty(numel, dtype=dtype, device=eng.device)
        self.grad = None
        self.grad_written = False
        self.pending = None
        self.bits = None
        self.compact = None
        self.pending_hw = None
        self.grad_dense, self.residual_needs_dense = None, False
        self.data_compact = self.bits_compact = None
        self.fwd_sampled = False
        self._compact_first = None
        self.eng = eng

    @property
    def data(self):
        if self.fused_pool:
            raise RuntimeError("T%d is conv1's output inside the fused conv1 + ReLU + max-pool kernel: it is never stored (option stem_pool = 0 keeps it)" % self.spec.id)
        return self._data

    @data.setter
    def data(self, t):
        self._data = t

    def grad_buf(self):
        if self.grad is None:
            self.grad = torch.empty(self.numel, dtype=self.data.dtype, device=self.eng.device)
        return self.grad


class _Conv(object):

    def __init__(self, node):
        self.node, self.name, self.bn = node, node.name, node.bn
        self.N, self.npad = node.cout, _round_up(node.cout, 8)
        self.src = self.dst = self.res = None
        self.xin = None
        self.gf = self.gd = self.gf_compact = self.gd_compact = None
        self.gd_scatter, self.gd_scatter_stride = False, 0
        self.K_raw, self.fwd_flags, self.fwd_index, self.winograd = 0, 0, None, False
        self.w = self.b = self.gamma = self.beta = self.mean = self.var = self.wf = self.wd = self.biasf = self.scale = None
        self.batch_bn, self.Mpix = False, None
        self.bn_gamma = self.bn_beta = self.bn_mmean = self.bn_mvar = self.z = self.dz = self.bmean = self.bvar = self.dbeta = self.dgamma = None
        self.splits, self.desc, self.desc_id = 0, None, None
        self.ws_f = self.ws_d = 0
        self.halo_f = self.halo_d = False
        self.pooled_grad = None
        self.solo = self.wgrad_by_pair = self.dgrad_done_by_pair = False
        self.wg_ws, self.wg_npart = None, 0
        self.dw_raw = self.colsum = self.dotpart = self.dw_unp = None


class _PendingLaunches(object):

    WGRAD_GROUP_FILL = 0.7

    def __init__(self, eng, wg_max):
        self.eng, self.dt = eng, eng.dt
        self.wg_max = wg_max
        self.wg, self.hw, self.dd, self.dwg = [], [], [], []

    def _emit(self, tag, op, label):
        self.eng.bwd_ops.append((tag, op))
        self.eng.labels["bwd"].append(label)

    def emit_wgrad(self, c, name, xw, G, gf_w):
        dt = self.dt
        self._emit(name, lambda: hip.conv_wgrad_partial(gf_w, dt, xw, G, c.wg_ws), "wgrad:" + name)

    def at_node(self, level):
        if self.dd and level != self.dd[0]["level"]:
            self.flush_dense_dgrads()
        if self.dwg and level is None:
            self.flush_dense_wgrads()

    def add_wgrad_pair(self, item):
        self.hw.append(item)
        if len(self.hw) == 2:
            self.flush_hw_pair()

    def add_wgrad_group(self, item):
        cand = self.wg + [item]
        wide = lambda g: g.KH * g.KW * g.C >= 256 and g.N >= 256
        if len(cand) > 1 and (wide(cand[-1][4]) != wide(cand[0][4]) or
                              hip.WgradGroup([t[4] for t in cand], self.dt).fill < self.WGRAD_GROUP_FILL):
            self.flush_wgrads()
        self.wg.append(item)
        if len(self.wg) >= self.wg_max:
            self.flush_wgrads()

    def add_dense_dgrad(self, L):
        prev = [P for P in self.dd if P["dst"] is L["dst"]]
        if prev and L["add"] is L["dst"] and prev[-1].get("src1") is None:
            prev[-1].update(src1=L["src0"], wgt1=L["wgt0"], K1=L["K0"], name=prev[-1]["name"] + "+" + L["name"])
            return
        if prev:
            self.flush_dense_dgrads()
        self.dd.append(L)

    def add_dense_wgrad(self, L):
        self.dwg.append(L)

    def flush_bucket(self):
        if self.dwg and any(L["dz"] is P["dst"] for L in self.dwg for P in self.dd):
            self.flush_dense_dgrads()
        self.flush_dense_wgrads()
        self.flush_wgrads()
        self.flush_hw_pair()

    def flush(self):
        self.flush_dense_dgrads()
        self.flush_bucket()

    def flush_hw_pair(self):
        items, self.hw = self.hw, []
        sp = hip.conv_wgrad_pair_splits(items[0][4], items[1][4], self.dt) if len(items) == 2 else None
        if sp is None:
            for t in items:
                self.emit_wgrad(*t)
            return
        for (c, _, _, _, _), s_ in zip(items, sp):
            assert s_ <= c.splits
            c.splits = c.desc.splits = s_
            c.wg_npart = s_ * (c.K_raw * c.npad + hip.WGRAD_PART_PAD)
            c.desc.part, c.desc.colpart = c.wg_ws.data_ptr(), c.wg_ws.data_ptr() + 4 * c.wg_npart
        (c0, n0, x0, G0, g0), (c1, n1, x1, G1, g1) = items
        dt = self.dt
        self._emit((n0, n1), lambda: hip.conv_wgrad_partial2(g0, g1, dt, x0, G0, c0.wg_ws, x1, G1, c1.wg_ws), "wgrad:%s+%s" % (n0, n1))
        self.eng.n_wgrad_groups += 1

    def flush_wgrads(self):
        items, self.wg = self.wg, []
        dev = self.eng.device
        while items:
            take = items
            grp = None
            while len(take) > 1:
                grp = hip.WgradGroup([t[4] for t in take], self.dt)
                if grp.nblocks:
                    break
                take, grp = take[:len(take) - 1], None
            items = items[len(take):]
            if grp is None:
                self.emit_wgrad(*take[0])
                continue
            for (c, _, _, _, _), s in zip(take, grp.splits):
                need_f = s * (c.K_raw * c.npad + hip.WGRAD_PART_PAD) + s * c.npad + 64
                if c.wg_ws.numel() < need_f:
                    c.wg_ws = torch.empty(need_f, dtype=torch.float32, device=dev)
                if s > 1 and c.dw_raw is None:
                    c.dw_raw = torch.empty(c.K_raw * c.npad, dtype=torch.float32, device=dev)
                    c.colsum = torch.empty(c.npad, dtype=torch.float32, device=dev)
                    c.desc.dw_raw, c.desc.colsum = hip.ptr(c.dw_raw), hip.ptr(c.colsum)
                c.splits = c.desc.splits = s
                c.wg_npart = s * (c.K_raw * c.npad + hip.WGRAD_PART_PAD)
                c.desc.part, c.desc.colpart = c.wg_ws.data_ptr(), c.wg_ws.data_ptr() + 4 * c.wg_npart
            grp.bind([t[2] for t in take], [t[3] for t in take], [t[0].wg_ws for t in take], dev)
            names = tuple(t[1] for t in take)
            self._emit(names, lambda grp=grp: grp.run(), "wgrad:" + "+".join(names))
            self.eng.n_wgrad_groups += 1

    def flush_dense_dgrads(self):
        layers, self.dd = self.dd, []
        for i in range(0, len(layers), hip.DENSE_MULTI_MAX):
            part = layers[i:i + hip.DENSE_MULTI_MAX]
            self._emit(None, hip.DenseMulti(part, self.dt).run, "dgrad_heads:" + "+".join(L["name"] for L in part))

    def flush_dense_wgrads(self):
        layers, self.dwg = self.dwg, []
        for i in range(0, len(layers), hip.DENSE_MULTI_MAX):
            part = layers[i:i + hip.DENSE_MULTI_MAX]
            self._emit(tuple(L["name"] for L in part), hip.DenseWgradMulti(part, self.dt).run, "wgrad_heads:" + "+".join(L["name"] for L in part))
```

Before: 4699 images/sec.

## Fold stem weight prep/finalize into batched param kernels and fuse final norm reduction

The stem conv now gets a param descriptor. Its weight packing runs inside the batched weight-prep kernel, and its gradient finalize reads packed rows directly, which removes the separate stem prep, unpack and finalize launches. The last finalize_vec block also uses an atomic ticket to do the global squared-norm reduction, dropping the separate sqnorm_final launch before SGD. The cost is extra descriptor fields, per-layer sq slot bookkeeping, and a last-block-done pattern that depends on correct fences and resetting the ticket each step.

```diff
diff --git a/include/ursonet_hip.h b/include/ursonet_hip.h
--- a/include/ursonet_hip.h
+++ b/include/ursonet_hip.h
@@ -143,6 +143,12 @@
     const float *part, *colpart;
     float *dw_raw, *colsum, *dotpart;
     float *gw, *gb, *ggamma, *gbeta;
+    int32_t stem;
+    int32_t norm_nparts;
+    float *sqslots;
+    const float *norm_parts;
+    float *norm_out;
+    uint32_t *norm_ticket;
 } urso_param_desc;
 enum { URSO_PB_PREP = 0, URSO_PB_REDUCE = 1, URSO_PB_FINALIZE_MAT = 2, URSO_PB_FINALIZE_VEC = 3 };
 int urso_conv_wgrad_splits(const urso_conv_geom* g, int dt);
diff --git a/ursonet_amd/csrc/common.h b/ursonet_amd/csrc/common.h
--- a/ursonet_amd/csrc/common.h
+++ b/ursonet_amd/csrc/common.h
@@ -52,6 +52,8 @@
 
 #define URSO_FUSE_REDUCE_MAX 16
 static __host__ __device__ inline bool urso_fuse_reduce(int splits) { return splits > 1 && splits <= URSO_FUSE_REDUCE_MAX; }
+
+static __host__ __device__ inline int urso_desc_dw_rows(const urso_param_desc& d) { return d.stem ? 224 : d.K; }
 
 #define URSO_REDUCE_COLS 256
 static __host__ __device__ inline int urso_reduce_lanes(int splits) { return splits > 384 ? 16 : (splits > 192 ? 8 : (splits > 96 ? 4 : (splits > 48 ? 2 : 1))); }
diff --git a/ursonet_amd/csrc/conv_wgrad.hip b/ursonet_amd/csrc/conv_wgrad.hip
--- a/ursonet_amd/csrc/conv_wgrad.hip
+++ b/ursonet_amd/csrc/conv_wgrad.hip
@@ -920,7 +920,7 @@
 __global__ __launch_bounds__(256) void reduce_partials_batch_kernel(const urso_param_desc* __restrict__ descs, const int32_t* __restrict__ blockmap) {
     const urso_param_desc& d = descs[blockmap[2 * blockIdx.x]];
     const int local = blockmap[2 * blockIdx.x + 1];
-    const size_t cnt = (size_t)d.K * d.npad;
+    const size_t cnt = (size_t)urso_desc_dw_rows(d) * d.npad;
     const int rcols = URSO_REDUCE_COLS / urso_reduce_lanes(d.splits);
     const int nb_dw = (int)(((cnt + 3) / 4 + rcols - 1) / rcols);
     if (local < nb_dw) reduce_partials_body(local, d.part, d.dw_raw, cnt, d.splits, cnt + URSO_WGRAD_PART_PAD);
diff --git a/ursonet_amd/csrc/prep.hip b/ursonet_amd/csrc/prep.hip
--- a/ursonet_amd/csrc/prep.hip
+++ b/ursonet_amd/csrc/prep.hip
@@ -107,24 +107,6 @@
     weight_prep_body<T>(blockIdx.x, blockIdx.y, blockIdx.z, KH, KW, C, N, npad, w, b, gamma, beta, mean, var, eps, wf, wd, biasf, scale);
 }
 
-template <typename T>
-__global__ void weight_prep_batch_kernel(const urso_param_desc* __restrict__ descs, const int32_t* __restrict__ blockmap) {
-    const urso_param_desc& d = descs[blockmap[2 * blockIdx.x]];
-    const int local = blockmap[2 * blockIdx.x + 1];
-    const urso_param_desc* extra = d.bias_from > 0 ? &descs[d.bias_from - 1] : nullptr;
-    if (((d.C | d.N | d.npad) & 3) == 0) {
-        const int gx = ceil_div(d.C, 64), gy = ceil_div(d.npad, 64);
-        const int bx = local % gx, by = (local / gx) % gy, tap = local / (gx * gy);
-        weight_prep_body64<T>(bx, by, tap, d.KH, d.KW, d.C, d.N, d.npad, d.w, d.b, d.gamma, d.beta, d.mean, d.var, d.eps,
-                              d.wf, d.wd, d.biasf, d.scale, extra);
-        return;
-    }
-    const int gx = ceil_div(d.C, 32), gy = ceil_div(d.npad, 32);
-    const int bx = local % gx, by = (local / gx) % gy, tap = local / (gx * gy);
-    weight_prep_body<T>(bx, by, tap, d.KH, d.KW, d.C, d.N, d.npad, d.w, d.b, d.gamma, d.beta, d.mean, d.var, d.eps,
-                        d.wf, d.wd, d.biasf, d.scale, extra);
-}
-
 extern "C" int urso_conv_weight_prep(int KH, int KW, int C, int N, int npad, int dt,
                                      const float* w_d, const float* b_d, const float* gamma_d, const float* beta_d,
                                      const float* mean_d, const float* var_d, float eps,
@@ -143,11 +125,10 @@
 }
 
 template <typename T>
-__global__ void stem_pack_kernel(int N, const float* __restrict__ w, const float* __restrict__ b,
-                                 const float* __restrict__ gamma, const float* __restrict__ beta,
-                                 const float* __restrict__ mean, const float* __restrict__ var, float eps,
-                                 void* wf, float* biasf, float* scale) {
-    const int i = blockIdx.x * blockDim.x + threadIdx.x;
+__device__ __forceinline__ void stem_pack_body(int i, int N, const float* __restrict__ w, const float* __restrict__ b,
+                                               const float* __restrict__ gamma, const float* __restrict__ beta,
+                                               const float* __restrict__ mean, const float* __restrict__ var, float eps,
+                                               void* wf, float* biasf, float* scale) {
     const int total = N * 7 * 4 * 8;
     if (i < total) {
         const int cp = i & 7, kp = (i >> 3) & 3, ky = (i >> 5) % 7, n = i / 224;
@@ -162,6 +143,13 @@
         if (gamma) bf += beta[i] - mean[i] * s;
         biasf[i] = bf; scale[i] = s;
     }
+}
+template <typename T>
+__global__ void stem_pack_kernel(int N, const float* __restrict__ w, const float* __restrict__ b,
+                                 const float* __restrict__ gamma, const float* __restrict__ beta,
+                                 const float* __restrict__ mean, const float* __restrict__ var, float eps,
+                                 void* wf, float* biasf, float* scale) {
+    stem_pack_body<T>(blockIdx.x * blockDim.x + threadIdx.x, N, w, b, gamma, beta, mean, var, eps, wf, biasf, scale);
 }
 
 extern "C" int urso_stem_weight_pack(int N, int dt, const float* w_d, const float* b_d, const float* gamma_d,
@@ -178,6 +166,34 @@
     return urso_check_launch("urso_stem_weight_pack");
 }
 
+template <typename T>
+__global__ void weight_prep_batch_kernel(const urso_param_desc* __restrict__ descs, const int32_t* __restrict__ blockmap) {
+    const urso_param_desc& d = descs[blockmap[2 * blockIdx.x]];
+    const int local = blockmap[2 * blockIdx.x + 1];
+    if (d.stem) {
+        stem_pack_body<T>(local * (int)blockDim.x + (int)threadIdx.x, d.N, d.w, d.b, d.gamma, d.beta, d.mean, d.var, d.eps, d.wf, d.biasf, d.scale);
+        return;
+    }
+    const urso_param_desc* extra = d.bias_from > 0 ? &descs[d.bias_from - 1] : nullptr;
+    if (((d.C | d.N | d.npad) & 3) == 0) {
+        const int gx = ceil_div(d.C, 64), gy = ceil_div(d.npad, 64);
+        const int bx = local % gx, by = (local / gx) % gy, tap = local / (gx * gy);
+        weight_prep_body64<T>(bx, by, tap, d.KH, d.KW, d.C, d.N, d.npad, d.w, d.b, d.gamma, d.beta, d.mean, d.var, d.eps,
+                              d.wf, d.wd, d.biasf, d.scale, extra);
+        return;
+    }
+    const int gx = ceil_div(d.C, 32), gy = ceil_div(d.npad, 32);
+    const int bx = local % gx, by = (local / gx) % gy, tap = local / (gx * gy);
+    weight_prep_body<T>(bx, by, tap, d.KH, d.KW, d.C, d.N, d.npad, d.w, d.b, d.gamma, d.beta, d.mean, d.var, d.eps,
+                        d.wf, d.wd, d.biasf, d.scale, extra);
+}
+
+__device__ __forceinline__ int stem_packed_row(int i) {
+    const int c = i % 3, kx = (i / 3) % 7, ky = i / 21;
+    const int q = kx + 1, kp = q >> 1, cp = (q & 1) * 4 + c;
+    return (ky * 4 + kp) * 8 + cp;
+}
+
 __global__ void stem_unpack_kernel(int N, const float* __restrict__ dwp, float* __restrict__ dw) {
     const int i = blockIdx.x * blockDim.x + threadIdx.x;
     if (i >= 7 * 7 * 3 * N) return;
@@ -208,7 +224,7 @@
 __device__ __forceinline__ void finalize_mat_body(int bx, int by, int K, int N, int ldn, int kb, const float* __restrict__ dwr, const float* __restrict__ w,
                                     const float* __restrict__ gamma, const float* __restrict__ var, float eps,
                                     float regc, int trainable, float* __restrict__ gw, float* __restrict__ dotpart, int nsum = 1, size_t pstride = 0,
-                                    float* __restrict__ sqslot = nullptr) {
+                                    float* __restrict__ sqslot = nullptr, bool stem = false) {
     const int kbeg = by * kb, kend = min(K, kbeg + kb);
     float sq = 0.f;
     auto sq4 = [&](const f32x4_t& g) { sq += g.x * g.x + g.y * g.y + g.z * g.z + g.w * g.w; };
@@ -228,7 +244,7 @@
             s.x = bn_scale(gamma, var, eps, n); s.y = bn_scale(gamma, var, eps, n + 1);
             s.z = bn_scale(gamma, var, eps, n + 2); s.w = bn_scale(gamma, var, eps, n + 3);
             auto row_sum = [&](int k) -> f32x4_t {
-                const float* p = dwr + (size_t)k * ldn + n;
+                const float* p = dwr + (size_t)(stem ? stem_packed_row(k) : k) * ldn + n;
                 f32x4_t d = *(const f32x4_t*)p;
                 if (nsum > 1) {
                     f32x4_t t = f32x4_t{0.f, 0.f, 0.f, 0.f};
@@ -285,7 +301,8 @@
         const float s = bn_scale(gamma, var, eps, n);
         for (int k = kbeg + tk; k < kend; k += 4) {
             float d = 0.f;
-            for (int q = 0; q < nsum; ++q) d += dwr[(size_t)q * pstride + (size_t)k * ldn + n];
+            const size_t row = (size_t)(stem ? stem_packed_row(k) : k);
+            for (int q = 0; q < nsum; ++q) d += dwr[(size_t)q * pstride + row * ldn + n];
             const float ww = w[(size_t)k * N + n];
             dot += ww * d;
             const float gv = trainable ? (s * d + regc * ww) : 0.f;
@@ -312,8 +329,8 @@
     const int gx = ceil_div(d.N, 64);
     const bool fused = urso_fuse_reduce(d.splits);
     finalize_mat_body(local % gx, local / gx, d.K, d.N, d.npad, d.kb, (d.splits == 1 || fused) ? d.part : d.dw_raw, d.w, d.gamma, d.var, d.eps,
-                      d.regc, d.trainable, d.gw, d.dotpart, fused ? d.splits : 1, (size_t)d.K * d.npad + URSO_WGRAD_PART_PAD,
-                      sqpart ? sqpart + blockIdx.x : nullptr);
+                      d.regc, d.trainable, d.gw, d.dotpart, fused ? d.splits : 1, (size_t)urso_desc_dw_rows(d) * d.npad + URSO_WGRAD_PART_PAD,
+                      sqpart ? (d.sqslots ? d.sqslots + local : sqpart + blockIdx.x) : nullptr, d.stem != 0);
 }
 
 __device__ __forceinline__ void finalize_vec_body(int n, int N, int ks, const float* __restrict__ dotpart, const float* __restrict__ colsum,
@@ -361,10 +378,31 @@
 __global__ void finalize_vec_batch_kernel(const urso_param_desc* __restrict__ descs, const int32_t* __restrict__ blockmap, float* __restrict__ sqpart) {
     const urso_param_desc& d = descs[blockmap[2 * blockIdx.x]];
     const int local = blockmap[2 * blockIdx.x + 1];
-    if (!d.gb && !d.ggamma) { if (sqpart && threadIdx.x == 0) sqpart[blockIdx.x] = 0.f; return; }
-    const bool fused = urso_fuse_reduce(d.splits);
-    finalize_vec_body(local * blockDim.x + threadIdx.x, d.N, d.ks, d.dotpart, (d.splits == 1 || fused) ? d.colpart : d.colsum, d.b, d.gamma, d.mean, d.var, d.eps,
-                      d.regb, d.trainable, d.bn_trainable, d.gb, d.ggamma, d.gbeta, fused ? d.splits : 1, d.npad, sqpart ? sqpart + blockIdx.x : nullptr);
+    float* sqslot = sqpart ? (d.sqslots ? d.sqslots + ceil_div(d.N, 64) * d.ks + local : sqpart + blockIdx.x) : nullptr;
+    if (!d.gb && !d.ggamma) { if (sqslot && threadIdx.x == 0) *sqslot = 0.f; }
+    else {
+        const bool fused = urso_fuse_reduce(d.splits);
+        finalize_vec_body(local * blockDim.x + threadIdx.x, d.N, d.ks, d.dotpart, (d.splits == 1 || fused) ? d.colpart : d.colsum, d.b, d.gamma, d.mean, d.var, d.eps,
+                          d.regb, d.trainable, d.bn_trainable, d.gb, d.ggamma, d.gbeta, fused ? d.splits : 1, d.npad, sqslot);
+    }
+    const urso_param_desc& dl = descs[blockmap[2 * (gridDim.x - 1)]];
+    if (!sqpart || !dl.norm_out) return;
+    __shared__ int last;
+    __shared__ float shn[8];
+    if (threadIdx.x == 0) {
+        __threadfence();
+        last = atomicAdd(dl.norm_ticket, 1u) == gridDim.x - 1;
+    }
+    __syncthreads();
+    if (!last) return;
+    __threadfence();
+    float s = 0.f;
+    for (int i = threadIdx.x; i < dl.norm_nparts; i += blockDim.x) s += __hip_atomic_load(dl.norm_parts + i, __ATOMIC_RELAXED, __HIP_MEMORY_SCOPE_AGENT);
+    s = block_sum_f(s, shn);
+    if (threadIdx.x == 0) {
+        dl.norm_out[0] = s;
+        __hip_atomic_store(dl.norm_ticket, 0u, __ATOMIC_RELAXED, __HIP_MEMORY_SCOPE_AGENT);
+    }
 }
 
 static int finalize_ks(int K, int N) {
@@ -424,10 +462,11 @@
 
 static int batch_layer_blocks(int phase, const urso_param_desc& d) {
     switch (phase) {
-    case URSO_PB_PREP: return (((d.C | d.N | d.npad) & 3) == 0 ? ceil_div(d.C, 64) * ceil_div(d.npad, 64) : ceil_div(d.C, 32) * ceil_div(d.npad, 32)) * d.KH * d.KW;
+    case URSO_PB_PREP: if (d.stem) return ceil_div(d.N * 224, 256);
+        return (((d.C | d.N | d.npad) & 3) == 0 ? ceil_div(d.C, 64) * ceil_div(d.npad, 64) : ceil_div(d.C, 32) * ceil_div(d.npad, 32)) * d.KH * d.KW;
     case URSO_PB_REDUCE: {
         if (d.splits <= 1 || urso_fuse_reduce(d.splits)) return 0;
-        const size_t cnt = (size_t)d.K * d.npad;
+        const size_t cnt = (size_t)urso_desc_dw_rows(d) * d.npad;
         const int rcols = URSO_REDUCE_COLS / urso_reduce_lanes(d.splits);
         return (int)(((cnt + 3) / 4 + rcols - 1) / rcols) + (int)(((size_t)(d.npad + 3) / 4 + rcols - 1) / rcols);
     }
@@ -442,6 +481,7 @@
     d->KH = KH; d->KW = KW; d->C = C; d->N = N; d->npad = npad; d->K = KH * KW * C; d->splits = splits;
     d->ks = finalize_ks(d->K, N); d->kb = ceil_div(d->K, d->ks);
     d->eps = eps;
+    d->stem = 0; d->norm_nparts = 0; d->sqslots = nullptr; d->norm_parts = nullptr; d->norm_out = nullptr; d->norm_ticket = nullptr;
     d->regc = 2.0f * weight_decay / ((float)d->K * (float)N); d->regb = 2.0f * weight_decay / (float)N;
     return URSO_OK;
 }
diff --git a/ursonet_amd/engine.py b/ursonet_amd/engine.py
--- a/ursonet_amd/engine.py
+++ b/ursonet_amd/engine.py
@@ -270,21 +270,22 @@
             c.bmean, c.bvar = torch.empty(c.N, dtype=torch.float32, device=dev), torch.empty(c.N, dtype=torch.float32, device=dev)
             c.dbeta, c.dgamma = torch.empty(c.N, dtype=torch.float32, device=dev), torch.empty(c.N, dtype=torch.float32, device=dev)
         self.convs[node.name] = c
+        d = hip.ParamDesc()
         if node.stem:
-            self.prep_ops.append(lambda c=c: hip.stem_weight_pack(c.N, dt, c.w, c.b, c.gamma, c.beta, c.mean, c.var, BN_EPS,
-                                                                  c.wf, c.biasf, c.scale))
-            self.labels["prep"].append("prep:" + node.name)
+            assert c.npad == c.N
+            c.splits = 1
+            hip.param_desc_init(d, 7, 7, 3, c.N, c.npad, 1, BN_EPS, float(self.config.WEIGHT_DECAY))
+            d.stem = 1
         else:
-            d = hip.ParamDesc()
             c.splits = hip.conv_wgrad_splits(c.gf, dt) if training else 1
             hip.param_desc_init(d, node.kh if not node.dense else 1, node.kw if not node.dense else 1, node.cin, c.N, c.npad,
                                 max(c.splits, 1), BN_EPS, float(self.config.WEIGHT_DECAY))
-            for f, t in (("w", c.w), ("b", c.b), ("gamma", c.gamma), ("beta", c.beta), ("mean", c.mean), ("var", c.var),
-                         ("wf", c.wf), ("wd", c.wd), ("biasf", c.biasf), ("scale", c.scale)):
-                setattr(d, f, hip.ptr(t))
-            c.desc_id = len(self._descs)
-            c.desc = d
-            self._descs.append(d)
+        for f, t in (("w", c.w), ("b", c.b), ("gamma", c.gamma), ("beta", c.beta), ("mean", c.mean), ("var", c.var),
+                     ("wf", c.wf), ("wd", c.wd), ("biasf", c.biasf), ("scale", c.scale)):
+            setattr(d, f, hip.ptr(t))
+        c.desc_id = len(self._descs)
+        c.desc = d
+        self._descs.append(d)
         self._plan_conv_forward(c)
 
     def _plan_compact_input(self, c):
@@ -370,9 +371,7 @@
     def _plan_stem_workspaces(self):
         stems = [c for c in self.convs.values() if c.node.stem]
         max_ws = max([0] + [hip.conv_wgrad_ws_bytes(c.gf, self.dt) for c in stems])
-        max_fin_ws = max([0] + [hip.param_grad_finalize_ws_bytes(147, c.N) for c in stems])
         self.ws = torch.empty(max_ws // 4 + 64, dtype=torch.float32, device=self.device)
-        self.fin_ws = torch.empty(max_fin_ws // 4 + 64, dtype=torch.float32, device=self.device)
 
     def _plan_buckets(self):
         from .dp import plan_buckets
@@ -388,7 +387,7 @@
         bucket_of = {ln: k for k, (_, _, names) in enumerate(self.buckets) for ln in names}
         groups = OrderedDict()
         for node in self._backward_order():
-            if node.op == "pool" or node.stem:
+            if node.op == "pool":
                 continue
             folded_bn = node.bn and not self.convs[node.name].batch_bn
             if self.layer_trainable[node.name] or (folded_bn and self.layer_trainable[node.bn]):
@@ -439,7 +438,7 @@
                 G = c.dz
                 bn_tr = False
             if (tr or bn_tr) and node.stem:
-                self._plan_stem_wgrad(c, G, tr, bn_tr)
+                self._plan_stem_wgrad(c, G, tr, bn_tr, q)
             elif tr or bn_tr:
                 self._plan_wgrad(c, G, tr, bn_tr, q, lvl_n)
             self._plan_residual_handover(c, Gsum)
@@ -465,8 +464,8 @@
         self.labels["bwd"].append("maxpool_bwd")
         src.grad_written = True
 
-    def _plan_stem_wgrad(self, c, G, tr, bn_tr):
-        node, cfg, dt, dev = c.node, self.config, self.dt, self.device
+    def _plan_stem_wgrad(self, c, G, tr, bn_tr, q):
+        node, d, dt, dev = c.node, c.desc, self.dt, self.device
         c.dw_raw = torch.empty(c.K_raw * c.npad, dtype=torch.float32, device=dev)
         c.colsum = torch.empty(c.npad, dtype=torch.float32, device=dev)
         if c.pooled_grad is not None:
@@ -476,24 +475,27 @@
         else:
             self.bwd_ops.append((node.name, lambda c=c, G=G: hip.conv_wgrad(c.gf, dt, c.src.data, G, self.ws, c.dw_raw, c.colsum)))
             self.labels["bwd"].append("wgrad:" + node.name)
-        c.dw_unp = torch.empty(147 * c.N, dtype=torch.float32, device=dev)
-        self.bwd_ops.append((node.name, lambda c=c: hip.stem_wgrad_unpack(c.N, c.dw_raw, c.dw_unp)))
-        self.labels["bwd"].append("unpack:" + node.name)
-        gw = self.gview(node.name, "kernel").reshape(-1)
-        gb = self.gview(node.name, "bias").reshape(-1) if node.bias else None
-        gg = self.gview(node.bn, "gamma").reshape(-1) if (node.bn and not c.batch_bn) else None
-        gbe = self.gview(node.bn, "beta").reshape(-1) if (node.bn and not c.batch_bn) else None
+        c.dotpart = torch.empty(d.ks * c.N + 16, dtype=torch.float32, device=dev)
+        d.part, d.colpart, d.dotpart = hip.ptr(c.dw_raw), hip.ptr(c.colsum), hip.ptr(c.dotpart)
+        d.trainable, d.bn_trainable = int(tr), int(bn_tr)
+        d.gw = hip.ptr(self.gview(node.name, "kernel").reshape(-1))
+        d.gb = hip.ptr(self.gview(node.name, "bias").reshape(-1)) if node.bias else None
+        d.ggamma = hip.ptr(self.gview(node.bn, "gamma").reshape(-1)) if (node.bn and not c.batch_bn) else None
+        d.gbeta = hip.ptr(self.gview(node.bn, "beta").reshape(-1)) if (node.bn and not c.batch_bn) else None
         if self.fused_sqnorm:
             s0 = self._sq_slots
-            s1 = self._sq_slots = s0 + hip.param_grad_finalize_sq_slots(147, c.N)
-            self.bwd_ops.append((node.name, lambda c=c, gw=gw, gb=gb, gg=gg, gbe=gbe, tr=tr, bn_tr=bn_tr, s0=s0, s1=s1:
-                                 hip.param_grad_finalize_sq(147, c.N, c.N, c.dw_unp, c.colsum, c.w, c.b, c.gamma, c.mean, c.var, BN_EPS,
-                                                            float(cfg.WEIGHT_DECAY), tr, bn_tr, gw, gb, gg, gbe, self.fin_ws, self.sqpart[s0:s1])))
-        else:
-            self.bwd_ops.append((node.name, lambda c=c, gw=gw, gb=gb, gg=gg, gbe=gbe, tr=tr, bn_tr=bn_tr:
-                                 hip.param_grad_finalize(147, c.N, c.N, c.dw_unp, c.colsum, c.w, c.b, c.gamma, c.mean, c.var, BN_EPS,
-                                                         float(cfg.WEIGHT_DECAY), tr, bn_tr, gw, gb, gg, gbe, self.fin_ws)))
-        self.labels["bwd"].append("finalize:" + node.name)
+            self._sq_slots = s0 + hip.param_grad_finalize_sq_slots(147, c.N)
+            c.sq_own = (s0, self._sq_slots)
+        self._close_bucket(node.name, q)
+
+    def _close_bucket(self, name, q):
+        if name not in self._last_of_group:
+            return
+        q.flush_bucket()
+        k = self._last_of_group[name]
+        for ph, nm in ((hip.PB_REDUCE, "reduce"), (hip.PB_FINALIZE_MAT, "finalize_mat"), (hip.PB_FINALIZE_VEC, "finalize_vec")):
+            self.bwd_ops.append((tuple(self._bucket_groups[k]), (ph, k)))
+            self.labels["bwd"].append("%s:bucket%d" % (nm, k))
 
     def _plan_wgrad(self, c, G, tr, bn_tr, q, lvl_n):
         node, d, B, dt, dev = c.node, c.desc, self.B, self.dt, self.device
@@ -533,12 +535,7 @@
                 q.add_dense_wgrad(dict(name=node.name, x=xw, dz=G, part=c.wg_ws, colpart=c.wg_ws[c.wg_npart:], M=B, K=c.K_raw, N=c.npad))
             else:
                 q.emit_wgrad(c, node.name, xw, G, gf_w)
-        if node.name in self._last_of_group:
-            q.flush_bucket()
-            k = self._last_of_group[node.name]
-            for ph, nm in ((hip.PB_REDUCE, "reduce"), (hip.PB_FINALIZE_MAT, "finalize_mat"), (hip.PB_FINALIZE_VEC, "finalize_vec")):
-                self.bwd_ops.append((tuple(self._bucket_groups[k]), (ph, k)))
-                self.labels["bwd"].append("%s:bucket%d" % (nm, k))
+        self._close_bucket(node.name, q)
 
     def _plan_residual_handover(self, c, Gsum):
         if c.res is None or not self.grad_needed[c.res.spec.id]:
@@ -698,22 +695,49 @@
         self._upload_param_table()
         resolved, labels = [], []
         assert len(self.bwd_ops) == len(self.labels["bwd"])
+        self._norm_by = None
+        n_vec = 0
         for (tag, op), lab in zip(self.bwd_ops, self.labels["bwd"]):
             if isinstance(op, tuple):
                 ph, k = op
-                ids = [self.convs[nm].desc_id for nm in self._bucket_groups[k]]
+                group = self._bucket_groups[k]
+                ids = [self.convs[nm].desc_id for nm in group]
                 nb_ = self.pbatch.plan(ph, k, ids)
                 if nb_ == 0:
                     continue
                 if self.fused_sqnorm and ph in (hip.PB_FINALIZE_MAT, hip.PB_FINALIZE_VEC):
+                    own = 0
+                    for nm in group:
+                        cc = self.convs[nm]
+                        if cc.sq_own is not None:
+                            assert nm == group[-1]
+                            nvec = -(-cc.N // 256)
+                            own = nvec if ph == hip.PB_FINALIZE_VEC else cc.sq_own[1] - cc.sq_own[0] - nvec
                     s0 = self._sq_slots
-                    s1 = self._sq_slots = s0 + nb_
-                    op = (lambda ph=ph, k=k, s0=s0, s1=s1: self.pbatch.run(ph, k, dt, sqpart=self.sqpart[s0:s1]))
+                    s1 = self._sq_slots = s0 + nb_ - own
+                    op = (lambda ph=ph, k=k, s0=s0, s1=s1, own=own: self.pbatch.run(ph, k, dt, sqpart=self.sqpart[s0:s1], own_slots=own))
+                    if ph == hip.PB_FINALIZE_VEC:
+                        n_vec += 1
+                        self._norm_by = group[-1]
                 else:
                     op = (lambda ph=ph, k=k: self.pbatch.run(ph, k, dt))
             resolved.append((tag, op)); labels.append(lab)
         self.bwd_ops, self.labels["bwd"] = resolved, labels
         self.sqpart = torch.zeros(max(self._sq_slots, 1), dtype=torch.float32, device=self.device) if self.fused_sqnorm else None
+        if not self.fused_sqnorm:
+            return
+        if n_vec != 1:
+            self._norm_by = None
+        self.normsq = torch.zeros(1, dtype=torch.float32, device=self.device)
+        self.norm_ticket = torch.zeros(1, dtype=torch.int32, device=self.device)
+        for cc in self.convs.values():
+            if cc.sq_own is not None:
+                cc.desc.sqslots = self.sqpart[cc.sq_own[0]:].data_ptr()
+        if self._norm_by is not None:
+            d = self.convs[self._norm_by].desc
+            d.norm_parts, d.norm_nparts = self.sqpart.data_ptr(), self.sqpart.numel()
+            d.norm_out, d.norm_ticket = self.normsq.data_ptr(), self.norm_ticket.data_ptr()
+        self.pbatch.upload(self._descs)
 
     def _plan_optimizer(self):
         cfg, dev = self.config, self.device
@@ -729,9 +753,12 @@
                 self.flat_v2, self.flat_vhat = torch.zeros_like(self.flat_w), torch.zeros_like(self.flat_w)
         elif self.hyper is None or self.hyper.numel() != 3:
             self.hyper = torch.tensor([float(cfg.LEARNING_RATE), float(cfg.LEARNING_MOMENTUM), clip], dtype=torch.float32, device=dev)
-        self.normsq = torch.zeros(1, dtype=torch.float32, device=dev)
+        if not (self.fused_sqnorm and self._norm_by is not None):
+            self.normsq = torch.zeros(1, dtype=torch.float32, device=dev)
         self.sq_ws = torch.empty(hip.sqnorm_ws_bytes(n) // 4, dtype=torch.float32, device=dev)
-        if self.fused_sqnorm:
+        if self.fused_sqnorm and self._norm_by is not None:
+            pass
+        elif self.fused_sqnorm:
             self.opt_ops.append(lambda: hip.sqnorm_final(self.sqpart, self.normsq))
         else:
             self.opt_ops.append(lambda: hip.sqnorm(n, self.flat_g, self.sq_ws, self.normsq))
@@ -740,7 +767,7 @@
                                                               self.hyper, self.normsq))
         else:
             self.opt_ops.append(lambda: hip.sgd_momentum_clip(n, self.flat_w, self.flat_g, self.flat_v, self.hyper, self.normsq))
-        self.labels["opt"] += ["sqnorm", "adam" if self.adam else "sgd"]
+        self.labels["opt"] += ["sqnorm"] * (len(self.opt_ops) - 1) + ["adam" if self.adam else "sgd"]
 
     def _fork_weight_gradients(self):
         self.wgrad_stream = None
diff --git a/ursonet_amd/hip.py b/ursonet_amd/hip.py
--- a/ursonet_amd/hip.py
+++ b/ursonet_amd/hip.py
@@ -57,7 +57,9 @@
     _fields_ = ([(n, C.c_int32) for n in ("KH", "KW", "C", "N", "npad", "K", "splits", "ks", "kb", "trainable", "bn_trainable", "bias_from")] +
                 [(n, C.c_float) for n in ("eps", "regc", "regb")] +
                 [(n, C.c_void_p) for n in ("w", "b", "gamma", "beta", "mean", "var", "wf", "wd", "biasf", "scale", "part", "colpart",
-                                           "dw_raw", "colsum", "dotpart", "gw", "gb", "ggamma", "gbeta")])
+                                           "dw_raw", "colsum", "dotpart", "gw", "gb", "ggamma", "gbeta")] +
+                [(n, C.c_int32) for n in ("stem", "norm_nparts")] +
+                [(n, C.c_void_p) for n in ("sqslots", "norm_parts", "norm_out", "norm_ticket")])
 
 
 class DenseLayer(C.Structure):
@@ -407,6 +409,11 @@
         self.dev = raw.to(device)
         self.maps = {}
 
+    def upload(self, descs):
+        assert len(descs) == self.n
+        self.host = (ParamDesc * self.n)(*descs)
+        self.dev.copy_(torch.frombuffer(bytearray(bytes(self.host)), dtype=torch.uint8))
+
     def plan(self, phase, key, layer_ids):
         ids = (C.c_int32 * len(layer_ids))(*layer_ids)
         nb = _lib.urso_param_batch_plan(phase, self.host, ids, len(layer_ids), None, 0)
@@ -418,10 +425,10 @@
         self.maps[(phase, key)] = (t, nb)
         return nb
 
-    def run(self, phase, key, dt, stream=None, sqpart=None):
+    def run(self, phase, key, dt, stream=None, sqpart=None, own_slots=0):
         t, nb = self.maps[(phase, key)]
         if nb and sqpart is not None:
-            assert sqpart.dtype == torch.float32 and sqpart.numel() >= nb
+            assert sqpart.dtype == torch.float32 and sqpart.numel() >= nb - own_slots
             _chk(_lib.urso_param_batch_run_sq(phase, dt, ptr(self.dev), ptr(t), nb, ptr(sqpart), stream_ptr(stream)), "urso_param_batch_run_sq")
         elif nb:
             _chk(_lib.urso_param_batch_run(phase, dt, ptr(self.dev), ptr(t), nb, stream_ptr(stream)), "urso_param_batch_run")
diff --git a/ursonet_amd/plan_state.py b/ursonet_amd/plan_state.py
--- a/ursonet_amd/plan_state.py
+++ b/ursonet_amd/plan_state.py
@@ -55,12 +55,13 @@
         self.batch_bn, self.Mpix = False, None
         self.bn_gamma = self.bn_beta = self.bn_mmean = self.bn_mvar = self.z = self.dz = self.bmean = self.bvar = self.dbeta = self.dgamma = None
         self.splits, self.desc, self.desc_id = 0, None, None
+        self.sq_own = None
         self.ws_f = self.ws_d = 0
         self.halo_f = self.halo_d = False
         self.pooled_grad = None
         self.solo = self.wgrad_by_pair = self.dgrad_done_by_pair = False
         self.wg_ws, self.wg_npart = None, 0
-        self.dw_raw = self.colsum = self.dotpart = self.dw_unp = None
+        self.dw_raw = self.colsum = self.dotpart = None
 
 
 class _PendingLaunches(object):
```

New measurement: 4724 images/sec, median of 6. No clear change (+0.5%).
